# SHI-Labs/Prompt-Free-Diffusion

Hardware: AMD Instinct MI355X
Metric: images/sec @512x512 50-step DDIM, SD-v1.5+SeeCoder (higher is better)
Workload: dtype f16; 1 GPU; [c2] SD-v1.5 UNet + seecoder-v1-0, 512x512, 50-step DDIM (50 real steps), CFG 2.0, fp16, batch=4/GPU, 1 SeeCoder encode(s) + VAE decode per batch; global_batch=4, parallelism=dp1, world_size_reported_by_backend=1, collectives_forced_at_world_1=False

## Files before the change

### include/pfd_hip.h

```cpp
#ifndef PFD_HIP_H
#define PFD_HIP_H

#include <stddef.h>
#include <stdint.h>

#ifdef __cplusplus
extern "C" {
#endif

#define PFD_OK 0
#define PFD_EINVAL (-1)
#define PFD_ESHAPE (-2)
#define PFD_ELAUNCH (-3)

#define PFD_ABI_VERSION 10

typedef void* pfd_stream_t;

#define PFD_ACT_NONE 0
#define PFD_ACT_GELU 1
#define PFD_ACT_RELU 2
#define PFD_ACT_SILU 3
#define PFD_ACT_GEGLU 4

int pfd_abi_version(void);
const char* pfd_last_error(void);

typedef struct PfdGemmDesc {
  const void* A;
  const void* W;
  const void* bias;
  const void* rowvec;
  const void* R;
  void* C;
  int64_t lda, ldw, ldr, ldc, ldrv;
  int32_t M, N, K;
  int32_t rows_per_rv;
  int32_t act;
  int32_t bias_per_row;
  int32_t ksize, stride, pad, ups;
  int32_t B, H, Wd, Cin;
  int32_t Ho, Wo;
  void* ws;
  size_t ws_bytes;
  void* Ct;
  int64_t ldct;
  int32_t n_split;
  int32_t w_tiled;
  const void* gn_table;
  const void* A2;
  int64_t lda2;
  int32_t gn_c1;
  int32_t gn_act;
  const void* ln_stats;
  const void* ln_colsum;
  int32_t ln_parts;
  float ln_eps;
  void* ln_out;
  int32_t k_split;
  int32_t zero_rows;
  void* gn_out;
  const void* gnf_gamma;
  const void* gnf_beta;
  void* gnf_y;
  int64_t gnf_ldy;
  float gnf_eps;
  int32_t gnf_act;
  int32_t gnf_rows;
  int32_t gnf_skip_raw;
  int32_t res_rows;
} PfdGemmDesc;
int pfd_gemm_f16(const PfdGemmDesc* d, pfd_stream_t stream);
int pfd_gemm_f16_ex(const PfdGemmDesc* d, int32_t tile, pfd_stream_t stream);

int32_t pfd_gemm_geglu_group(int32_t N);

typedef struct PfdAttnDesc {
  const void* Q;
  const void* K;
  const void* Vt;
  void* O;
  int64_t ldq, ldk, ldvt, ldo;
  int64_t q_bs, k_bs, vt_bs, o_bs;
  int32_t B, H, Nq, Nk, D;
  float scale;
} PfdAttnDesc;
int pfd_attention_f16(const PfdAttnDesc* d, pfd_stream_t stream);

typedef struct PfdSwinAttnDesc {
  const void* qkv;
  const void* qkv_bias;
  const void* rpb;
  void* out;
  int32_t B, H, W, C, nH, ws, shift;
  float scale;
} PfdSwinAttnDesc;
int pfd_swin_window_attention_f16(const PfdSwinAttnDesc* d, pfd_stream_t stream);

size_t pfd_groupnorm_ws_bytes(int32_t B, int32_t C, int32_t HW);
int32_t pfd_groupnorm_takes_pstats(int32_t B, int32_t C1, int32_t C2, int32_t HW, int32_t G);
int pfd_groupnorm_pstats_f16(const void* x1, int32_t C1, int64_t ldx1, const void* st1, const void* x2, int32_t C2,
                             int64_t ldx2, const void* st2, const void* gamma, const void* beta, void* y, int64_t ldy,
                             int32_t B, int32_t HW, int32_t G, float eps, int32_t act, pfd_stream_t stream);

int pfd_groupnorm_table_f16(const void* x1, int32_t C1, int64_t ldx1, const void* x2, int32_t C2, int64_t ldx2,
                            const void* gamma, const void* beta, void* table, int32_t B, int32_t HW, int32_t G,
                            float eps, void* ws, size_t ws_bytes, pfd_stream_t stream);
int pfd_groupnorm_f16(const void* x1, int32_t C1, int64_t ldx1, const void* x2, int32_t C2,
                      int64_t ldx2, const void* gamma, const void* beta, void* y, int64_t ldy,
                      int32_t B, int32_t HW, int32_t G, float eps, int32_t act ,
                      void* ws, size_t ws_bytes, pfd_stream_t stream);

int pfd_layernorm_f16(const void* x, int64_t ldx, const void* gamma, const void* beta, void* y,
                      int64_t ldy, int32_t M, int32_t C, float eps, int32_t gather4, int32_t B,
                      int32_t H, int32_t W, pfd_stream_t stream);

int pfd_ln_rowstats_f16(const void* x, int64_t ldx, int32_t M, int32_t C, void* out, pfd_stream_t stream);

int pfd_softmax_rows_f16(const void* x, int64_t ldx, void* y, int64_t ldy, int32_t R, int32_t N,
                         float scale, pfd_stream_t stream);

int pfd_nchw_to_nhwc_f16(const void* x, int32_t src_f32, void* y, int32_t B, int32_t C, int32_t H,
                         int32_t W, float mul, float add, int32_t rep, pfd_stream_t stream);
int pfd_nhwc_to_nchw(const void* x, void* y, int32_t dst_f32, int32_t B, int32_t C, int32_t H,
                     int32_t W, float mul, float add, float lo, float hi, pfd_stream_t stream);
int pfd_im2col_f16(const void* x, int64_t ldx, void* col, int32_t B, int32_t H, int32_t W,
                   int32_t Cin, int32_t ksize, int32_t stride, int32_t pad, int32_t Ho, int32_t Wo,
                   int32_t Kpad, pfd_stream_t stream);
int pfd_timestep_embedding_f16(const int64_t* t, void* out, int32_t B, int32_t dim,
                               float max_period, pfd_stream_t stream);
int pfd_cfg_ddim_step(const void* eps, int32_t nb, const float* x, const float* noise,
                      const float* coef, float* x_prev, float* pred_x0, void* xin_next, int32_t rep,
                      int32_t B, int32_t C, int32_t h, int32_t w, pfd_stream_t stream);
int pfd_philox_normal_f32(const int64_t* key, int32_t step, float* out, int32_t B, int64_t n_per_sample,
                          pfd_stream_t stream);
int pfd_cfg_ddim_step_rng(const void* eps, int32_t nb, const float* x, const int64_t* key, int32_t step,
                          float noise_mul, const float* coef, float* x_prev, float* pred_x0, void* xin_next,
                          int32_t rep, int32_t B, int32_t C, int32_t h, int32_t w, pfd_stream_t stream);
int pfd_add_f16(const void* a, const void* b, void* y, int64_t n, pfd_stream_t stream);
int pfd_axpby_f16(const void* a, float alpha, const void* b, float beta, void* y, int64_t n,
                  pfd_stream_t stream);
int pfd_add_rowvec_f16(const void* x, int64_t ldx, const void* v, void* y, int64_t ldy, int32_t R,
                       int32_t C, pfd_stream_t stream);

int pfd_add_rowvec_lnstats_f16(const void* x, int64_t ldx, const void* v, void* y, int64_t ldy, int32_t R, int32_t C,
                               void* stats, pfd_stream_t stream);

int pfd_image_u8_f16(const void* x, void* y, int64_t n, float mul, float add, int32_t f16_image,
                     pfd_stream_t stream);

#define PFD_IMG_PRECISION_BITS 22
#define PFD_IMG_U8 0
#define PFD_IMG_NCHW_F16 1
#define PFD_IMG_NCHW_F32 2
#define PFD_IMG_NHWC_F16 3

int pfd_image_resample_check(int32_t B, int32_t Hin, int32_t Win, int32_t Hout, int32_t Wout, int32_t C);

int pfd_image_resample_h_u8(const void* src, void* dst, int32_t B, int32_t H, int32_t Win, int32_t Wout, int32_t C,
                            const int32_t* kk, const int32_t* xmin, const int32_t* klen, int32_t ktaps,
                            pfd_stream_t stream);

int pfd_image_resample_v_u8(const void* src, void* dst, int32_t out_kind, int32_t B, int32_t Hin, int32_t Hout,
                            int32_t W, int32_t C, const int32_t* kk, const int32_t* ymin, const int32_t* klen,
                            int32_t ktaps, pfd_stream_t stream);

int pfd_act_f16(const void* x, void* y, int64_t n, int32_t act, pfd_stream_t stream);

int pfd_prof_enable(int32_t on);
int pfd_prof_read(int32_t bucket, double* ms, int64_t* launches, double* flops, double* bytes);
const char* pfd_prof_bucket_name(int32_t bucket);
int pfd_prof_num_buckets(void);

#ifdef __cplusplus
}
#endif
#endif
```

### prompt-free-diffusion_amd/csrc/gemm_conv.hip

```cpp
#include "pfd_common.h"

namespace {

__device__ __attribute__((aligned(16))) half_t g_zero_halves[8];
__device__ __forceinline__ const half_t* pfd_zero_halves() { return g_zero_halves; }

constexpr int BK = 64;
constexpr int LDS_LD = BK + 8;

struct GemmParams {
  const half_t* A;
  const half_t* W;
  const half_t* bias;
  const half_t* rowvec;
  const half_t* R;
  half_t* C;
  long lda, ldw, ldr, ldc, ldrv;
  int M, N, K;
  int rows_per_rv, act, bias_per_row;
  int ksize, stride, pad, ups;
  int B, H, Wd, Cin, Ho, Wo;
  int tiles_m, tiles_n;
};

// ... 327 lines not shown
    if (cb + 1 < ncb) store_patch((cb + 1) & 1);
  }
  const int x = x0 + wave * 16 + l15, n0 = 4 * kg;
  if (x < p.Wd && n0 < p.N) {
    const long m = ((long)b * p.H + y) * p.Wd + x;
    const half_t* bsrc = p.bias ? p.bias : pfd_zero_halves();
    half_t bv[4], o[4];
#pragma unroll
    for (int r = 0; r < 4; ++r) bv[r] = bsrc[p.bias ? min(n0 + r, p.N - 1) : r];
#pragma unroll
    for (int r = 0; r < 4; ++r) o[r] = (half_t)(acc[r] + (float)bv[r]);
    half_t* cp = p.C + m * p.ldc + n0;
    if (n0 + 4 <= p.N && (p.ldc & 3) == 0 && (reinterpret_cast<uintptr_t>(p.C) & 7) == 0) {
      Pack8 q;
#pragma unroll
      for (int r = 0; r < 4; ++r) q.e[r] = o[r];
      *reinterpret_cast<uint2*>(cp) = q.u;
    } else {
#pragma unroll
      for (int r = 0; r < 4; ++r)
        if (n0 + r < p.N) cp[r] = o[r];
    }
  }
}

static bool narrow_conv_takes(const GemmParams& p) {
  return p.ksize == 3 && p.stride == 1 && p.pad == 1 && !p.ups && p.Ho == p.H && p.Wo == p.Wd && p.N <= 16 && p.Cin % BK == 0 &&
         !p.rowvec && !p.R && p.act == PFD_ACT_NONE && !p.bias_per_row;
}

static int launch_narrow_conv(const GemmParams& p, hipStream_t s) {
  const bool prof = pfd_prof_on();
  if (prof)
    pfd_prof_begin(20, 2.0 * p.M * p.N * p.K, 2.0 * p.B * p.H * p.Wd * p.Cin + 2.0 * p.N * p.K + 2.0 * p.M * p.N, s);
  const int segs = (p.Wd + NRW_PX - 1) / NRW_PX;
  hipLaunchKernelGGL(conv3x3_narrow_kernel, dim3(segs * p.H * p.B), dim3(256), 0, s, p);
  if (prof) pfd_prof_end(s);
  return pfd_check_launch("pfd_gemm_f16(conv3x3 narrow)");
}

}

int pfd_gemm160_try(const PfdGemmDesc* d, int variant, int splits, hipStream_t s);

extern "C" int32_t pfd_gemm_geglu_group(int32_t N) { return N % 160 == 0 ? 2 : 32; }

extern "C" int pfd_gemm_f16_ex(const PfdGemmDesc* d, int32_t tile, pfd_stream_t stream) {
  if (!d || !d->A || !d->W || !d->C) return PFD_EINVAL;
  if (d->M <= 0 || d->N <= 0 || d->K <= 0) return PFD_EINVAL;
  if ((d->lda & 7) || (d->ldw & 7)) return PFD_EINVAL;
  if ((reinterpret_cast<uintptr_t>(d->A) & 15) || (reinterpret_cast<uintptr_t>(d->W) & 15)) return PFD_EINVAL;
  if (d->K % BK) return PFD_ESHAPE;
  if (d->rowvec && d->rows_per_rv < 1) return PFD_EINVAL;
  if (d->act < PFD_ACT_NONE || d->act > PFD_ACT_GEGLU) return PFD_EINVAL;
  if (d->ksize > 0) {
    if (d->Cin <= 0 || d->K != (d->ups == 2 ? 4 : d->ksize * d->ksize) * d->Cin) return PFD_EINVAL;
    if ((long)d->B * d->Ho * d->Wo != d->M) return PFD_EINVAL;
    if (d->stride < 1) return PFD_EINVAL;
  }
  if (d->Ct && (d->act != PFD_ACT_NONE || d->rowvec || d->R || d->bias_per_row || (tile != 0 && tile < 1000)))
    return PFD_EINVAL;
  if (tile == 0 || tile >= 1000) {
    const int enc = tile >= 1000 ? tile - 1000 : 0;
    const int rc = pfd_gemm160_try(d, enc / 100, enc % 100, (hipStream_t)stream);
    if (rc <= 0) return rc;
    if (tile >= 1000 || d->Ct) return PFD_ESHAPE;
  }
  if (d->ksize > 0 && d->ups == 2) {
    pfd_set_error("pfd_gemm_f16: the phase-folded upsample convolution is served by the 256-row loader-wave kernel only (see PfdGemmDesc.ups)");
    return PFD_ESHAPE;
  }
  if (d->gn_table) {
    pfd_set_error("pfd_gemm_f16: the GroupNorm prologue is served by the 3x3 patch kernel only (see PfdGemmDesc.gn_table)");
    return PFD_ESHAPE;
  }
  if (d->gn_out) {
    pfd_set_error("pfd_gemm_f16: GroupNorm statistics of the output are emitted by the wide-tile kernels only (see PfdGemmDesc.gn_out)");
    return PFD_ESHAPE;
  }
  if (d->res_rows > 0 && d->res_rows != d->M) {
    pfd_set_error("pfd_gemm_f16: a residual stored once for a doubled batch is read by the wide-tile kernels only (see PfdGemmDesc.res_rows)");
    return PFD_ESHAPE;
  }
  if (d->gnf_y) {
    pfd_set_error("pfd_gemm_f16: the fused GroupNorm lives in the split-K reduction of the wide-tile kernels only (see PfdGemmDesc.gnf_y)");
    return PFD_ESHAPE;
  }
  if (d->k_split > 0 || d->zero_rows > 0) {
    pfd_set_error("pfd_gemm_f16: k_split / zero_rows are served by the wide-tile linear kernels only (see PfdGemmDesc.k_split)");
    return PFD_ESHAPE;
  }
  if (d->w_tiled) {
    pfd_set_error("pfd_gemm_f16: K-tile-contiguous weights are read by the wide-tile kernels only (see PfdGemmDesc.w_tiled)");
    return PFD_ESHAPE;
  }
  if (d->ln_stats || d->ln_out) {
    pfd_set_error("pfd_gemm_f16: the LayerNorm fold is served by the wide-tile linear kernels only (see PfdGemmDesc.ln_stats)");
    return PFD_ESHAPE;
  }
  GemmParams p;
  p.A = (const half_t*)d->A;
  p.W = (const half_t*)d->W;
  p.bias = (const half_t*)d->bias;
  p.rowvec = (const half_t*)d->rowvec;
  p.R = (const half_t*)d->R;
  p.C = (half_t*)d->C;
  p.lda = d->lda; p.ldw = d->ldw; p.ldr = d->ldr; p.ldc = d->ldc; p.ldrv = d->ldrv;
  p.M = d->M; p.N = d->N; p.K = d->K;
  p.rows_per_rv = d->rows_per_rv > 0 ? d->rows_per_rv : 1;
  p.act = d->act; p.bias_per_row = d->bias_per_row;
  p.ksize = d->ksize; p.stride = d->stride; p.pad = d->pad; p.ups = d->ups;
  p.B = d->B; p.H = d->H; p.Wd = d->Wd; p.Cin = d->Cin; p.Ho = d->Ho; p.Wo = d->Wo;
  p.tiles_m = p.tiles_n = 0;
  if (p.ksize > 0) {
    if (p.Cin % BK) return PFD_ESHAPE;
    if (p.K != p.ksize * p.ksize * p.Cin) return PFD_EINVAL;
    if ((long)p.B * p.Ho * p.Wo != p.M) return PFD_EINVAL;
    if (p.stride < 1) return PFD_EINVAL;
  }
  if (p.act < PFD_ACT_NONE || p.act > PFD_ACT_GEGLU) return PFD_EINVAL;
  hipStream_t s = (hipStream_t)stream;
  if (tile == 0 && narrow_conv_takes(p)) return launch_narrow_conv(p, s);
  if (p.act == PFD_ACT_GEGLU) {
    if (p.N % 128 || pfd_gemm_geglu_group(p.N) != 32) return PFD_ESHAPE;
    return launch<2, 2>(p, s);
  }
  switch (tile) {
    case 0: break;
    case 22: return launch<2, 2>(p, s);
    case 21: return launch<2, 1>(p, s);
    case 12: return launch<1, 2>(p, s);
    case 11: return launch<1, 1>(p, s);
    default: return PFD_EINVAL;
  }
  auto blocks = [&](int bm, int bn) { return (long)((p.M + bm - 1) / bm) * ((p.N + bn - 1) / bn); };
  auto waste = [&](int bn) { return (double)(((p.N + bn - 1) / bn) * bn) / p.N; };
  if (blocks(128, 128) >= 512 && waste(128) <= 1.13) return launch<2, 2>(p, s);
  if (blocks(128, 64) >= 384 && p.M >= 128) return launch<2, 1>(p, s);
  if (p.N > 64 && blocks(64, 128) >= 384 && waste(128) <= 1.13) return launch<1, 2>(p, s);
  return launch<1, 1>(p, s);
}

extern "C" int pfd_gemm_f16(const PfdGemmDesc* d, pfd_stream_t stream) { return pfd_gemm_f16_ex(d, 0, stream); }
```

### prompt-free-diffusion_amd/csrc/gemm_glds.hip

```cpp
#include <type_traits>

#include <stdlib.h>

#include "pfd_common.h"

int pfd_ln_rowstats_launch(const half_t* x, long ldx, int M, int C, float* out, hipStream_t s, bool prof);

namespace {

constexpr int BK = 64;
constexpr int BN = 160;
constexpr int ROWB = BK * 2;

__device__ __attribute__((aligned(256))) half_t g_zero_page[128];

struct G160Params {
  const half_t* A;
  const half_t* W;
  const half_t* bias;
  const half_t* rowvec;
  const half_t* R;
  half_t* C;
  float* ws;
  half_t* Ct;
  long ldct;
  int n_split;
  long lda, ldw, ldr, ldc, ldrv;
  int M, N, K;
  int rows_per_rv, act;
  int ksize, stride, pad, ups;
  int B, H, Wd, Cin, Ho, Wo;
  int tiles_m, tiles_n, splits, kt_per_split;
  int nmajor;
  int krot;
  int pt_w, pt_sh;
  int w_tu;
  long w_kstep;
  const float2* ln_in;
  const float* ln_cs;
  float2* ln_out;
  int ln_P;
  float ln_eps;
  const float* gn_table;
  const half_t* A2;
  long lda2;
  int gn_c1, gn_act;
  float2* gn_out;
  int k_split;
  int zero_rows;
  int r_wrap;
};

__device__ __forceinline__ long res_row(const G160Params& p, int m) {
  const int mc = min(m, p.M - 1);
  return mc >= p.r_wrap ? mc - p.r_wrap : mc;
}

__device__ __forceinline__ void glds16(const void* src, void* lds_dst) {
  __builtin_amdgcn_global_load_lds((const __attribute__((address_space(1))) void*)src,
                                   (__attribute__((address_space(3))) void*)lds_dst, 16, 0, 0);
}

__device__ __forceinline__ const half_t* w_row_ptr(const G160Params& p, int n, int c8) {
  if (p.w_tu == 0) return p.W + (long)n * p.ldw + c8;
  const int tn = n / p.w_tu;
  return p.W + ((long)tn * (p.K / BK) * p.w_tu + (n - tn * p.w_tu)) * BK + c8;
}

#if !defined(PFD_CPU_EMU)
#define PFD_ARG_BATCH_LIN(p)                                                                                              \
  asm volatile("" ::"s"((p).tiles_m), "s"((p).tiles_n), "s"((p).nmajor), "s"((p).kt_per_split), "s"((p).K), "s"((p).M),      \
               "s"((p).zero_rows), "s"((p).k_split), "s"((p).krot), "s"((p).w_tu), "s"((p).A), "s"((p).A2), "s"((p).W),      \
               "s"((p).lda), "s"((p).lda2), "s"((p).ldw), "s"((p).w_kstep))
#define PFD_ARG_BATCH_CONV(p)                                                                                             \
  asm volatile("" ::"s"((p).tiles_m), "s"((p).tiles_n), "s"((p).nmajor), "s"((p).kt_per_split), "s"((p).K), "s"((p).M),      \
               "s"((p).krot), "s"((p).w_tu), "s"((p).A), "s"((p).W), "s"((p).lda), "s"((p).ldw), "s"((p).w_kstep),           \
               "s"((p).Cin), "s"((p).H), "s"((p).Wd), "s"((p).Ho), "s"((p).Wo), "s"((p).stride), "s"((p).pad), "s"((p).ups), \
               "s"((p).ksize))
#else
#define PFD_ARG_BATCH_LIN(p) ((void)0)
#define PFD_ARG_BATCH_CONV(p) ((void)0)
#endif
template <int BN_>
__device__ __forceinline__ const half_t* w_row_ptr_tile(const G160Params& p, int tile_n, int r, int c8) {
  if (p.w_tu == 0) return p.W + (long)(tile_n * BN_ + r) * p.ldw + c8;
  const int sub = (BN_ > 160 && r >= p.w_tu) ? 1 : 0;
  const int tn = tile_n * (BN_ > 160 ? 2 : 1) + sub;
  return p.W + ((long)tn * (p.K / BK) * p.w_tu + (r - sub * p.w_tu)) * BK + c8;
}
#define PFD_W_ROW_PTR(BN_, p, tile_n, n0, r, c8) w_row_ptr_tile<BN_>(p, tile_n, r, c8)

__device__ __forceinline__ G160Params reload_params() {
  typedef __attribute__((address_space(4))) const unsigned* KArgPtr;
  KArgPtr k = (KArgPtr)__builtin_amdgcn_kernarg_segment_ptr();
  asm volatile("" : "+s"(k)::"memory");
  static_assert(sizeof(G160Params) % 4 == 0, "argument block read as dwords");
  unsigned w[sizeof(G160Params) / 4];
#pragma unroll
  for (unsigned i = 0; i < sizeof(G160Params) / 4; ++i) w[i] = k[i];
  G160Params q;
  __builtin_memcpy(&q, w, sizeof(q));
  return q;
}

template <int BYTES> struct GRaw;
template <> struct GRaw<2>  { typedef unsigned short type; };
template <> struct GRaw<8>  { typedef unsigned int type __attribute__((ext_vector_type(2))); };
template <> struct GRaw<16> { typedef unsigned int type __attribute__((ext_vector_type(4))); };
template <class T>
__device__ __forceinline__ T gld(const void* ptr) {
  typedef typename GRaw<sizeof(T)>::type V;
  const V v = *reinterpret_cast<const __attribute__((address_space(1))) V*>((unsigned long)ptr);
  T out;
  __builtin_memcpy(&out, &v, sizeof(T));
  return out;
}
template <class T>
__device__ __forceinline__ void gst(void* ptr, T val) {
  typedef typename GRaw<sizeof(T)>::type V;
  V v;
  __builtin_memcpy(&v, &val, sizeof(T));
  *reinterpret_cast<__attribute__((address_space(1))) V*>((unsigned long)ptr) = v;
}

template <int PT>
__device__ __forceinline__ int tile_row_m(const G160Params& p, int m0, int row) {
  if constexpr (PT == 2) {
    const int hw = p.H * p.Wd;
    const int bp = m0 / hw;
    const int q = m0 - bp * hw + row;
    const int y = q / p.Wd, x = q - y * p.Wd;
    return ((bp >> 2) * 2 * p.H + 2 * y + ((bp >> 1) & 1)) * (2 * p.Wd) + 2 * x + (bp & 1);
  } else if constexpr (PT == 1) return p.pt_w ? m0 + (row >> p.pt_sh) * p.Wd + (row & (p.pt_w - 1)) : m0 + row;
  else return m0 + row;
}

__device__ __forceinline__ int k_rotation(int krot, int tile_m, int tiles_m, int nsteps) {
  if (!krot || nsteps < 2) return 0;
  const int stride = max(1, nsteps / max(1, tiles_m));
  return (tile_m * stride) % nsteps;
}

__device__ __forceinline__ void lds_store16_opaque(void* lds_dst, uint4 v) {
  typedef unsigned u32x4 __attribute__((ext_vector_type(4)));
  const unsigned addr = (unsigned)(uintptr_t)(__attribute__((address_space(3))) char*)lds_dst;
  const u32x4 d = {v.x, v.y, v.z, v.w};
  asm volatile("ds_write_b128 %0, %1" ::"v"(addr), "v"(d) : "memory");
}

constexpr int stage_row_bytes(int cols) { return cols * 2 + 16; }

template <int WMB, int NT, bool PT = false>
__device__ __forceinline__ bool epilogue_stage(float4_t (&acc)[WMB][NT], const G160Params& p, int lane, int m0,
                                               int n0, int wm, int wn, int split, char* smem,
                                               const float2* lnstat = nullptr) {
  constexpr int BN = 32 * NT;
  const int l15 = lane & 15, g = lane >> 4;
  const int lr0 = wm * WMB * 16 + l15;
  auto mrow = [&](int lr) __attribute__((always_inline)) { return tile_row_m<PT>(p, m0, lr); };
  const int nw = n0 + wn * (16 * NT) + 4 * g;
  constexpr bool GEGLU_ONLY = NT == 10;
  if (lnstat && p.splits == 1) {
    float2 abv[WMB];
#pragma unroll
    for (int i = 0; i < WMB; ++i) abv[i] = lnstat[wm * WMB * 16 + i * 16 + l15];
    asm volatile("s_waitcnt lgkmcnt(0)" ::: "memory");
    __builtin_amdgcn_sched_barrier(0);
    float4_t cs[NT];
#pragma unroll
    for (int j = 0; j < NT; ++j) cs[j] = *reinterpret_cast<const float4_t*>(p.ln_cs + nw + j * 16);
#pragma unroll
    for (int i = 0; i < WMB; ++i) {
      const float2 ab = abv[i];
#pragma unroll
      for (int j = 0; j < NT; ++j)
#pragma unroll
        for (int r = 0; r < 4; ++r) acc[i][j][r] = fmaf(acc[i][j][r], ab.x, ab.y * cs[j][r]);
    }
  }

  const bool slab = !GEGLU_ONLY && p.splits > 1;

  if (!GEGLU_ONLY && !slab && p.Ct && n0 >= p.n_split) {
    float bv[NT][4];
    const half_t* bp = p.bias ? p.bias + nw : g_zero_page;
    const int bstep = p.bias ? 16 : 0;
#pragma unroll
    for (int j = 0; j < NT; ++j) {
      Pack8 b;
      b.u = gld<uint2>(bp + j * bstep);
#pragma unroll
      for (int r = 0; r < 4; ++r) bv[j][r] = (float)b.e[r];
    }
#pragma unroll
    for (int i = 0; i < WMB; ++i) {
      const int m = mrow(lr0 + i * 16);
      if (m >= p.M) continue;
#pragma unroll
      for (int j = 0; j < NT; ++j)
#pragma unroll
        for (int r = 0; r < 4; ++r)
          gst<half_t>(p.Ct + (long)(nw + j * 16 + r - p.n_split) * p.ldct + m, (half_t)(acc[i][j][r] + bv[j][r]));
    }
    return false;
  }

  const bool geglu = GEGLU_ONLY || p.act == PFD_ACT_GEGLU;
  const int lrow = wm * WMB * 16 + l15;
  const bool has_bias = p.bias && !slab;
  const half_t* bp = has_bias ? p.bias + nw : g_zero_page;
  const int bstep = has_bias ? 16 : 0;
  Pack8 bq[NT];
#pragma unroll
  for (int j = 0; j < NT; ++j) bq[j].u = gld<uint2>(bp + j * bstep);
  if (geglu) {
    constexpr int RS = stage_row_bytes(BN / 2);
#pragma unroll
    for (int i = 0; i < WMB; ++i) {
      char* sp = smem + (lrow + i * 16) * RS + (wn * (8 * NT) + 2 * g) * 2;
#pragma unroll
      for (int j = 0; j < NT; ++j) {
        half2_t o;
        o[0] = (half_t)((acc[i][j][0] + (float)bq[j].e[0]) * pfd_gelu(acc[i][j][2] + (float)bq[j].e[2]));
        o[1] = (half_t)((acc[i][j][1] + (float)bq[j].e[1]) * pfd_gelu(acc[i][j][3] + (float)bq[j].e[3]));
        *reinterpret_cast<half2_t*>(sp + j * 16) = o;
      }
    }
  } else if constexpr (!GEGLU_ONLY) {
    constexpr int RS = stage_row_bytes(BN);
    char* sp0 = smem + lrow * RS + (wn * (16 * NT) + 4 * g) * 2;
    auto put_row = [&](auto act, auto itag, const Pack8(&rv)[NT]) __attribute__((always_inline)) {
      constexpr int ACT = decltype(act)::value;
      constexpr int i = decltype(itag)::value;
      char* sp = sp0 + i * 16 * RS;
#pragma unroll
      for (int j = 0; j < NT; ++j) {
        Pack8 o;
#pragma unroll
        for (int r = 0; r < 4; ++r) {
          float v = acc[i][j][r] + (float)bq[j].e[r] + (float)rv[j].e[r];
          if constexpr (ACT == PFD_ACT_GELU) v = pfd_gelu(v);
          else if constexpr (ACT == PFD_ACT_RELU) v = fmaxf(v, 0.f);
          else if constexpr (ACT == PFD_ACT_SILU) v = pfd_silu(v);
          o.e[r] = (half_t)v;
        }
        *reinterpret_cast<uint2*>(sp + j * 32) = o.u;
      }
    };
    auto load_rv = [&](Pack8(&rv)[NT], int m) __attribute__((always_inline)) {
      const half_t* rvp = p.rowvec + (long)(min(m, p.M - 1) / p.rows_per_rv) * p.ldrv + nw;
#pragma unroll
      for (int j = 0; j < NT; ++j) rv[j].u = gld<uint2>(rvp + j * 16);
    };
    auto for_rows = [&](auto&& f) __attribute__((always_inline)) {
      f(std::integral_constant<int, 0>{});
      if constexpr (WMB > 1) f(std::integral_constant<int, 1>{});
      if constexpr (WMB > 2) f(std::integral_constant<int, 2>{});
      if constexpr (WMB > 3) f(std::integral_constant<int, 3>{});
      static_assert(WMB <= 4, "row tiles per wave");
    };
    auto run = [&](auto act) __attribute__((always_inline)) {
      Pack8 cur[NT];
      const int first = mrow(wm * WMB * 16), last = mrow(wm * WMB * 16 + WMB * 16 - 1);
      if (!p.rowvec || slab) {
#pragma unroll
        for (int j = 0; j < NT; ++j) cur[j].u = make_uint2(0, 0);
        for_rows([&](auto it) __attribute__((always_inline)) { put_row(act, it, cur); });
      } else if (PT || min(first, p.M - 1) / p.rows_per_rv == min(last, p.M - 1) / p.rows_per_rv) {
        load_rv(cur, first);
        for_rows([&](auto it) __attribute__((always_inline)) { put_row(act, it, cur); });
      } else if constexpr (!PT) {
        Pack8 nxt[NT];
        load_rv(cur, mrow(lr0));
        for_rows([&](auto it) __attribute__((always_inline)) {
          constexpr int i = decltype(it)::value;
          if constexpr (i + 1 < WMB) load_rv(nxt, mrow(lr0 + (i + 1) * 16));
          put_row(act, it, cur);
          if constexpr (i + 1 < WMB) {
#pragma unroll
            for (int j = 0; j < NT; ++j) cur[j].u = nxt[j].u;
          }
        });
      }
    };
    switch (slab ? PFD_ACT_NONE : p.act) {
      case PFD_ACT_GELU: run(std::integral_constant<int, PFD_ACT_GELU>{}); break;
      case PFD_ACT_RELU: run(std::integral_constant<int, PFD_ACT_RELU>{}); break;
      case PFD_ACT_SILU: run(std::integral_constant<int, PFD_ACT_SILU>{}); break;
      default: run(std::integral_constant<int, PFD_ACT_NONE>{}); break;
    }
// ... 191 lines not shown
    }
  };
  if (geglu) store_pass(std::integral_constant<int, BN / 2>{});
  else if constexpr (!GEGLU_ONLY) store_pass(std::integral_constant<int, BN>{});
}

template <int WMB, int NT, int NTHREADS, bool LNOUT = false, bool PT = false>
__device__ __forceinline__ void epilogue160(float4_t (&acc)[WMB][NT], const G160Params& p, int lane, int m0,
                                            int n0, int wm, int wn, int split, char* smem, int tid,
                                            const float2* lnstat = nullptr, int slab0 = 0) {
  epilogue_stage<WMB, NT, PT>(acc, p, lane, m0, n0, wm, wn, split, smem, lnstat);
  __syncthreads();
  epilogue_store<(NTHREADS / 128) * WMB * 16, NT, NTHREADS, LNOUT, PT>(p, m0, n0, smem, tid, slab0);
}

template <int WAVES_M, int WMB, bool CONV, int NBUF, int NT>
__global__ __launch_bounds__(WAVES_M * 128) void gemm160_kernel(const G160Params p) {
  constexpr int BN = 32 * NT;
  constexpr int NW = WAVES_M * 2;
  constexpr int BM = WAVES_M * WMB * 16;
  constexpr int A_INSTR = BM / 8;
  constexpr int B_INSTR = BN / 8;
  constexpr int A_PER_WAVE = A_INSTR / NW;
  constexpr int B_PER_WAVE = (B_INSTR + NW - 1) / NW;
  constexpr int STAGE = (BM + BN) * ROWB;
  constexpr int MAIN_BYTES = NBUF * STAGE;
  constexpr int DEPTH = NBUF - 1;
  constexpr bool B_DUP = NBUF > 2 && B_INSTR % NW != 0;
  static_assert(MAIN_BYTES <= 160 * 1024, "operand ring exceeds the 160 KiB LDS");
  static_assert(BM * stage_row_bytes(NT == 10 ? BN / 2 : BN) <= MAIN_BYTES, "the epilogue's staging image reuses the operand ring");
  constexpr int SMEM = MAIN_BYTES;
  static_assert(A_INSTR % NW == 0, "A tile must split evenly over the waves");
  static_assert(WAVES_M * 128 >= BM, "one thread per row forms the LayerNorm statistics");
  __shared__ __attribute__((aligned(1024))) char smem[SMEM + (CONV ? 0 : BM * 8)];
  float2* const lnstat = reinterpret_cast<float2*>(smem + SMEM);
  if constexpr (CONV) PFD_ARG_BATCH_CONV(p);
  else PFD_ARG_BATCH_LIN(p);

  const int tid = threadIdx.x;
  const int lane = tid & 63;
  const int wave = __builtin_amdgcn_readfirstlane(tid >> 6);
  const int wm = wave >> 1, wn = wave & 1;
  const int l15 = lane & 15, g = lane >> 4;

  const int nblk = p.tiles_m * p.tiles_n;
  const int t = xcd_remap(blockIdx.x, nblk);
  const int tile_m = p.nmajor ? t % p.tiles_m : t / p.tiles_n;
  const int tile_n = p.nmajor ? t / p.tiles_m : t - tile_m * p.tiles_n;
  const int m0 = tile_m * BM;
  const int n0 = tile_n * BN;
  const int split = blockIdx.z;
  const int kt_begin = split * p.kt_per_split;
  const int nk_total = p.K / BK;
  const int kt_end = min(nk_total, kt_begin + p.kt_per_split);

  const int srow = lane >> 3;
  const int cpos = lane & 7;
  const half_t* a_ptr[A_PER_WAVE];
  const half_t* a2_ptr[A_PER_WAVE];
  int a_oy[A_PER_WAVE], a_ox[A_PER_WAVE];
  long a_img[A_PER_WAVE];
  bool a_ok[A_PER_WAVE];
  int a_chunk[A_PER_WAVE];
#pragma unroll
  for (int j = 0; j < A_PER_WAVE; ++j) {
    const int r = (wave + NW * j) * 8 + srow;
    const int c = cpos ^ ((r >> 1) & 7);
    a_chunk[j] = c * 8;
    const int m = m0 + r;
    a_ok[j] = m < p.M;
    if (CONV) {
      const int hw = p.Ho * p.Wo;
      const int b = m / hw;
      const int rem = m - b * hw;
      const int oy = rem / p.Wo;
      a_oy[j] = oy * p.stride - p.pad;
      a_ox[j] = (rem - oy * p.Wo) * p.stride - p.pad;
      a_img[j] = (long)b * p.H * p.Wd * p.lda;
      a_ptr[j] = a2_ptr[j] = p.A;
    } else {
      const int mz = m - p.zero_rows;
      a_ok[j] = a_ok[j] && mz >= 0;
      a_ptr[j] = a_ok[j] ? p.A + (long)mz * p.lda + c * 8 : g_zero_page;
      a2_ptr[j] = a_ok[j] ? p.A2 + (long)mz * p.lda2 + c * 8 : g_zero_page;
      a_oy[j] = a_ox[j] = 0;
      a_img[j] = 0;
    }
  }
  const half_t* b_ptr[B_PER_WAVE];
#pragma unroll
  for (int j = 0; j < B_PER_WAVE; ++j) {
    int q = wave + NW * j;
    if (q >= B_INSTR) q = B_DUP ? q - NW : 0;
    const int r = q * 8 + srow;
    const int c = cpos ^ ((r >> 1) & 7);
    b_ptr[j] = PFD_W_ROW_PTR(BN, p, tile_n, n0, r, c * 8);
  }
  const int Hin = p.ups ? 2 * p.H : p.H;
  const int Win = p.ups ? 2 * p.Wd : p.Wd;

  const int nsteps = (!CONV && m0 + BM <= p.zero_rows) ? 0 : kt_end - kt_begin;
  int kt_issue = kt_begin + k_rotation(p.krot, tile_m, p.tiles_m, nsteps);
  int tap_ky = 0, tap_kx = 0, ci0 = 0;
  const half_t* a_tap[A_PER_WAVE];
  auto set_tap = [&]() {
#pragma unroll
    for (int j = 0; j < A_PER_WAVE; ++j) {
      int iy = a_oy[j] + tap_ky, ix = a_ox[j] + tap_kx;
      const bool ok = a_ok[j] && iy >= 0 && iy < Hin && ix >= 0 && ix < Win;
      if (p.ups) {
        iy >>= 1;
        ix >>= 1;
      }
      a_tap[j] = ok ? p.A + a_img[j] + ((long)iy * p.Wd + ix) * p.lda + a_chunk[j] : nullptr;
    }
  };
  auto seek = [&](int kt) {
    const int k0 = kt * BK;
    const int tap = k0 / p.Cin;
    ci0 = k0 - tap * p.Cin;
    tap_ky = tap / p.ksize;
    tap_kx = tap - tap_ky * p.ksize;
    set_tap();
  };
  if (CONV) seek(kt_issue);

  auto issue = [&](int stage) {
    char* As = smem + stage * STAGE;
    char* Bs = As + BM * ROWB;
    const int k0 = kt_issue * BK;
    const long kw = kt_issue * p.w_kstep;
    if (CONV) {
#pragma unroll
      for (int j = 0; j < A_PER_WAVE; ++j) {
        const half_t* src = a_tap[j] ? a_tap[j] + ci0 : g_zero_page;
        glds16(src, As + (wave + NW * j) * 1024);
      }
    } else {
      const bool first = k0 < p.k_split;
#pragma unroll
      for (int j = 0; j < A_PER_WAVE; ++j) {
        const half_t* src = first ? a_ptr[j] + k0 : a2_ptr[j] + (k0 - p.k_split);
        glds16(a_ok[j] ? src : a_ptr[j], As + (wave + NW * j) * 1024);
      }
    }
#pragma unroll
    for (int j = 0; j < B_PER_WAVE; ++j) {
      const int q = wave + NW * j;
      if (q < B_INSTR) glds16(b_ptr[j] + kw, Bs + q * 1024);
      else if (B_DUP) glds16(b_ptr[j] + kw, Bs + (q - NW) * 1024);
    }
    if (++kt_issue == kt_end) {
      kt_issue = kt_begin;
      if (CONV) seek(kt_begin);
    } else if (CONV) {
      ci0 += BK;
      if (ci0 >= p.Cin) {
        ci0 = 0;
        if (++tap_kx == p.ksize) {
          tap_kx = 0;
          ++tap_ky;
        }
        set_tap();
      }
    }
  };

// ... 732 lines not shown
                for (int j = 0; j < 5; ++j)
                  acc[i][j] = __builtin_amdgcn_mfma_f32_16x16x32_f16(bf[j], af[i], acc[i][j], 0, 0, 0);
            }
            if constexpr (NWS == 2) stage ^= 1;
            else if (++stage == NWS) stage = 0;
            toff += 1;
          }
          toff += PW - 3;
        }
      }
      block_barrier();
    }
    {
      const G160Params pe = reload_params();
      epilogue_stage<WMB, 5, true>(acc, pe, lane, m0, n0, wm, wn, split, smem);
    }
    asm volatile("s_waitcnt lgkmcnt(0)" ::: "memory");
    block_barrier();
  }
  const G160Params pe = reload_params();
  epilogue_store<256, 5, 768, false, true>(pe, m0, n0, smem, tid, tile_m * (256 / GN_SLAB));
}


__global__ __launch_bounds__(256) void splitk_reduce_kernel(const G160Params p) {
  const int nv = p.N / 8;
  const long nvec = (long)p.M * nv;
  for (long i = (long)blockIdx.x * 256 + threadIdx.x; i < nvec; i += (long)gridDim.x * 256) {
    const int m = (int)(i / nv);
    const int n = (int)(i - (long)m * nv) * 8;
    Pack16 bb, rv, rr;
    bb.u = *reinterpret_cast<const uint4*>(p.bias ? p.bias + n : g_zero_page);
    rv.u = *reinterpret_cast<const uint4*>(p.rowvec ? p.rowvec + (long)(m / p.rows_per_rv) * p.ldrv + n : g_zero_page);
    rr.u = *reinterpret_cast<const uint4*>(p.R ? p.R + res_row(p, m) * p.ldr + n : g_zero_page);
    float v[8] = {0, 0, 0, 0, 0, 0, 0, 0};
    for (int s0 = 0; s0 < p.splits; s0 += 4) {
      Pack16 a[4];
#pragma unroll
      for (int u = 0; u < 4; ++u)
        a[u].u = *reinterpret_cast<const uint4*>(reinterpret_cast<const half_t*>(p.ws) +
                                                 ((long)min(s0 + u, p.splits - 1) * p.M + m) * p.N + n);
#pragma unroll
      for (int u = 0; u < 4; ++u) {
        const float w = s0 + u < p.splits ? 1.f : 0.f;
#pragma unroll
        for (int e = 0; e < 8; ++e) v[e] += (float)a[u].e[e] * w;
      }
    }
    if (p.ln_in) {
      const float2* src = p.ln_in + (long)m * p.ln_P;
      float sum = 0.f, sq = 0.f;
#pragma unroll
      for (int j = 0; j < 8; ++j) {
        const float2 t = src[min(j, p.ln_P - 1)];
        const float w = j < p.ln_P ? 1.f : 0.f;
        sum = fmaf(t.x, w, sum);
        sq = fmaf(t.y, w, sq);
      }
      const float inv_k = 1.0f / (float)p.K;
      const float mean = sum * inv_k;
      const float rstd = rsqrtf(fmaxf(fmaf(-mean, mean, sq * inv_k), 0.f) + p.ln_eps);
      const float4_t c0 = *reinterpret_cast<const float4_t*>(p.ln_cs + n);
      const float4_t c1 = *reinterpret_cast<const float4_t*>(p.ln_cs + n + 4);
#pragma unroll
      for (int e = 0; e < 4; ++e) {
        v[e] = fmaf(v[e], rstd, -rstd * mean * c0[e]);
        v[4 + e] = fmaf(v[4 + e], rstd, -rstd * mean * c1[e]);
      }
    }
    Pack16 o;
#pragma unroll
    for (int e = 0; e < 8; ++e) {
      float x = v[e] + (float)bb.e[e];
      x += (float)rv.e[e];
      if (p.act == PFD_ACT_GELU) x = pfd_gelu(x);
      else if (p.act == PFD_ACT_RELU) x = fmaxf(x, 0.f);
      else if (p.act == PFD_ACT_SILU) x = pfd_silu(x);
      o.e[e] = (half_t)(x + (float)rr.e[e]);
    }
    *reinterpret_cast<uint4*>(p.C + (long)m * p.ldc + n) = o.u;
  }
}

constexpr int RGN_T = 256;
__global__ __launch_bounds__(RGN_T) void splitk_reduce_gn_kernel(const G160Params p) {
  constexpr int RW = RGN_T / 64, ROWS_SW = 3 * RW;
  __shared__ __attribute__((aligned(16))) float red[(RW + 1) * 320];
  const int tid = threadIdx.x, lane = tid & 63, w = tid >> 6;
  const int tiles_n = p.N / 160;
  const int slab = blockIdx.x / tiles_n, tile_n = blockIdx.x - slab * tiles_n;
  const int n = tile_n * 160 + (lane % 20) * 8;
  const bool active = lane < 60;
  const int rsub = lane / 20;
  float cs[8], cq[8];
#pragma unroll
  for (int e = 0; e < 8; ++e) cs[e] = cq[e] = 0.f;
  Pack16 bb;
  bb.u = *reinterpret_cast<const uint4*>(p.bias ? p.bias + n : g_zero_page);
  constexpr int SWEEPS = (GN_SLAB + ROWS_SW - 1) / ROWS_SW, U = SWEEPS < 3 ? SWEEPS : 3;
  static_assert(SWEEPS % U == 0, "sweeps in groups of U");
  for (int it0 = 0; it0 < SWEEPS; it0 += U) {
    int m[U];
    bool ok[U];
    Pack16 rv[U], rr[U];
    float v[U][8];
#pragma unroll
    for (int u = 0; u < U; ++u) {
      const int row_u = w * 3 + rsub + (it0 + u) * ROWS_SW;
      m[u] = min(slab * GN_SLAB + min(row_u, GN_SLAB - 1), p.M - 1);
      ok[u] = active && row_u < GN_SLAB && slab * GN_SLAB + row_u < p.M;
      rv[u].u = *reinterpret_cast<const uint4*>(p.rowvec ? p.rowvec + (long)(m[u] / p.rows_per_rv) * p.ldrv + n : g_zero_page);
      rr[u].u = *reinterpret_cast<const uint4*>(p.R ? p.R + res_row(p, m[u]) * p.ldr + n : g_zero_page);
#pragma unroll
      for (int e = 0; e < 8; ++e) v[u][e] = 0.f;
    }
    for (int s0 = 0; s0 < p.splits; s0 += 4) {
      Pack16 a[U][4];
#pragma unroll
      for (int u = 0; u < U; ++u)
#pragma unroll
        for (int k = 0; k < 4; ++k)
          a[u][k].u = *reinterpret_cast<const uint4*>(reinterpret_cast<const half_t*>(p.ws) +
                                                      ((long)min(s0 + k, p.splits - 1) * p.M + m[u]) * p.N + n);
#pragma unroll
      for (int u = 0; u < U; ++u)
#pragma unroll
        for (int k = 0; k < 4; ++k) {
          const float wgt = s0 + k < p.splits ? 1.f : 0.f;
#pragma unroll
          for (int e = 0; e < 8; ++e) v[u][e] += (float)a[u][k].e[e] * wgt;
        }
    }
#pragma unroll
    for (int u = 0; u < U; ++u) {
      Pack16 o;
      const float mk = ok[u] ? 1.f : 0.f;
#pragma unroll
      for (int e = 0; e < 8; ++e) {
        float x = v[u][e] + (float)bb.e[e];
        x += (float)rv[u].e[e];
        if (p.act == PFD_ACT_GELU) x = pfd_gelu(x);
        else if (p.act == PFD_ACT_RELU) x = fmaxf(x, 0.f);
        else if (p.act == PFD_ACT_SILU) x = pfd_silu(x);
        o.e[e] = (half_t)(x + (float)rr[u].e[e]);
        const float f = (float)o.e[e] * mk;
        cs[e] += f;
        cq[e] = fmaf(f, f, cq[e]);
      }
      if (ok[u]) *reinterpret_cast<uint4*>(p.C + (long)m[u] * p.ldc + n) = o.u;
    }
  }
  gn_slab_reduce<1, RGN_T>(cs, cq, tid, p.N / 32, slab, p.M / GN_SLAB, tiles_n, tile_n, p.gn_out, [&](int) { return red; });
}


struct GnFuse {
  const half_t* gamma;
  const half_t* beta;
  half_t* y;
  long ldy;
  float eps;
  int act, rows, skip_raw;
};
#ifndef PFD_GN_THREADS
#define PFD_GN_THREADS 1024
#endif
// ... 67 lines not shown
        for (int u = 0; u < GNF_U; ++u)
#pragma unroll
          for (int e = 0; e < 4; ++e) acc[u][e] += (float)a[u][q].e[e] * w;
      }
    }
#pragma unroll
    for (int u = 0; u < GNF_U; ++u) {
      Pack8 o;
#pragma unroll
      for (int e = 0; e < 4; ++e) {
        float x = acc[u][e] + (float)bq[u].e[e];
        x += (float)rq[u].e[e];
        if (p.act == PFD_ACT_GELU) x = pfd_gelu(x);
        else if (p.act == PFD_ACT_RELU) x = fmaxf(x, 0.f);
        else if (p.act == PFD_ACT_SILU) x = pfd_silu(x);
        o.e[e] = (half_t)(x + (float)xq[u].e[e]);
      }
      if (on[u] && !f.skip_raw) *reinterpret_cast<uint2*>(p.C + (m_b + ru[u]) * p.ldc + n_g + cu[u] * 4) = o.u;
      v[k0 + u] = on[u] ? o.u : make_uint2(0, 0);
    }
  }
  if (tid < cpg) {
    gam_s[tid] = (float)f.gamma[n_g + tid];
    bet_s[tid] = (float)f.beta[n_g + tid];
  }
  float sm = 0.f, sq = 0.f;
#pragma unroll
  for (int k = 0; k < GNF_MAX; ++k) {
    Pack8 q;
    q.u = v[k];
#pragma unroll
    for (int e = 0; e < 4; ++e) {
      const float x = (float)q.e[e];
      sm += x;
      sq += x * x;
    }
  }
  sm = wave_sum(sm);
  sq = wave_sum(sq);
  constexpr int NWV = GNF_T / 64;
  if (lane == 0) {
    red[wave] = sm;
    red[NWV + wave] = sq;
  }
  __syncthreads();
  const float count = (float)HW * (float)cpg;
  float ts = red[0], tq = red[NWV];
#pragma unroll
  for (int w = 1; w < NWV; ++w) {
    ts += red[w];
    tq += red[NWV + w];
  }
  const float mean = ts / count;
  const float rstd = rsqrtf(fmaxf(tq / count - mean * mean, 0.f) + f.eps);
  half_t* yb = f.y + m_b * f.ldy + n_g;
  r = tid / cpr;
  ch = tid - r * cpr;
  asm volatile("" : "+v"(r), "+v"(ch));
#pragma unroll
  for (int k = 0; k < GNF_MAX; ++k) {
    if (tid + GNF_T * k < total) {
      Pack8 q, o;
      q.u = v[k];
#pragma unroll
      for (int e = 0; e < 4; ++e) {
        const float w = rstd * gam_s[ch * 4 + e];
        float t = (float)q.e[e] * w + (bet_s[ch * 4 + e] - mean * w);
        if (f.act == PFD_ACT_SILU) t = pfd_silu(t);
        o.e[e] = (half_t)t;
      }
      *reinterpret_cast<uint2*>(yb + (long)r * f.ldy + ch * 4) = o.u;
    }
    r += dr;
    ch += dc;
    if (ch >= cpr) {
      ch -= cpr;
      ++r;
    }
  }
}

thread_local GnFuse t_gnf = {nullptr, nullptr, nullptr, 0, 0.f, 0, 0, 0};

inline void launch_splitk_reduce(const G160Params& p, hipStream_t s) {
  if (pfd_prof_on()) {
    pfd_prof_end(s);
    const double mn = (double)p.M * p.N;
    pfd_prof_begin(21, 0.0, 2.0 * p.splits * mn + 2.0 * mn * (1 + (p.R ? 1 : 0) + (t_gnf.y ? 1 : 0)), s);
  }
  if (t_gnf.y) {
    const GnFuse f = t_gnf;
    hipLaunchKernelGGL(splitk_reduce_gnorm_kernel, dim3(32 * (p.M / f.rows)), dim3(GNF_T), 0, s, p, f);
    return;
  }
  if (p.gn_out) {
    hipLaunchKernelGGL(splitk_reduce_gn_kernel, dim3((p.M / GN_SLAB) * (p.N / 160)), dim3(RGN_T), 0, s, p);
  } else {
    const long nvec = (long)p.M * (p.N / 8);
    int g = (int)((nvec + 255) / 256);
    if (g > 2048) g = 2048;
    hipLaunchKernelGGL(splitk_reduce_kernel, dim3(g), dim3(256), 0, s, p);
  }
  if (p.ln_out) pfd_ln_rowstats_launch(p.C, p.ldc, p.M, p.N, reinterpret_cast<float*>(p.ln_out), s, false);
}


inline int pick_nmajor(const G160Params& p) {
  const double a_bytes = p.ksize > 0 ? 2.0 * p.B * p.H * p.Wd * p.Cin : 2.0 * p.M * p.K;
  const double w_bytes = 2.0 * p.N * p.K;
  return (p.tiles_n >= 2 && p.tiles_m >= 2 && w_bytes > a_bytes) ? 1 : 0;
}

template <int WAVES_M, int WMB, int NBUF = 2, int NT = 5>
int launch160(G160Params& p, int bucket, hipStream_t s) {
  constexpr int BM = WAVES_M * WMB * 16;
  p.tiles_m = (p.M + BM - 1) / BM;
  p.tiles_n = p.N / (32 * NT);
  p.nmajor = pick_nmajor(p);
  p.krot = 0;
  const int nk = p.K / BK;
  p.kt_per_split = (nk + p.splits - 1) / p.splits;
  p.splits = (nk + p.kt_per_split - 1) / p.kt_per_split;
  dim3 grid(p.tiles_m * p.tiles_n, 1, p.splits);
  const bool prof = pfd_prof_on();
  if (prof) {
    const double a_bytes = p.ksize > 0 ? 2.0 * p.B * p.H * p.Wd * p.Cin : 2.0 * p.M * p.K;
    const double n_out = p.act == PFD_ACT_GEGLU ? p.N / 2 : p.N;
    pfd_prof_begin(bucket, 2.0 * p.M * p.N * p.K, a_bytes + 2.0 * p.N * p.K + 2.0 * p.M * n_out * (p.R ? 2 : 1), s);
  }
  if (p.ksize > 0)
    hipLaunchKernelGGL((gemm160_kernel<WAVES_M, WMB, true, NBUF, NT>), grid, dim3(WAVES_M * 128), 0, s, p);
  else
    hipLaunchKernelGGL((gemm160_kernel<WAVES_M, WMB, false, NBUF, NT>), grid, dim3(WAVES_M * 128), 0, s, p);
  if (p.splits > 1) launch_splitk_reduce(p, s);
  if (prof) pfd_prof_end(s);
  return pfd_check_launch("pfd_gemm_f16(wide)");
}

template <int NT>
int launch160ws(G160Params& p, int bucket, hipStream_t s, int pp) {
  p.tiles_m = (p.M + 255) / 256;
  p.tiles_n = p.N / (32 * NT);
  p.nmajor = pick_nmajor(p);
  p.krot = 0;
  const int nk = p.K / BK;
  p.kt_per_split = (nk + p.splits - 1) / p.splits;
  p.splits = (nk + p.kt_per_split - 1) / p.kt_per_split;
  dim3 grid(p.tiles_m * p.tiles_n, 1, p.splits);
  const bool prof = pfd_prof_on();
  if (prof) {
    const double a_bytes = p.ksize > 0 ? 2.0 * p.B * p.H * p.Wd * p.Cin : 2.0 * p.M * p.K;
    const double n_out = p.act == PFD_ACT_GEGLU ? p.N / 2 : p.N;
    pfd_prof_begin(bucket, 2.0 * p.M * p.N * p.K, a_bytes + 2.0 * p.N * p.K + 2.0 * p.M * n_out * (p.R ? 2 : 1), s);
  }
  if (p.ksize > 0 && p.ups == 2) {
    if (pp == 2) hipLaunchKernelGGL((gemm160ws_kernel<true, NT, 3, true>), grid, dim3(768), 0, s, p);
    else hipLaunchKernelGGL((gemm160ws_kernel<true, NT, 2, true>), grid, dim3(768), 0, s, p);
  } else if (p.ksize > 0) {
    if (pp == 2) hipLaunchKernelGGL((gemm160ws_kernel<true, NT, 3>), grid, dim3(768), 0, s, p);
    else hipLaunchKernelGGL((gemm160ws_kernel<true, NT>), grid, dim3(768), 0, s, p);
  } else {
    if (pp == 2) hipLaunchKernelGGL((gemm160ws_kernel<false, NT, 3>), grid, dim3(768), 0, s, p);
    else hipLaunchKernelGGL((gemm160ws_kernel<false, NT>), grid, dim3(768), 0, s, p);
  }
  if (p.splits > 1) launch_splitk_reduce(p, s);
  if (prof) pfd_prof_end(s);
  return pfd_check_launch("pfd_gemm_f16(wave-specialised)");
}

int launch_patch(G160Params& p, hipStream_t s, int ws) {
  p.tiles_m = p.M / 256;
  p.tiles_n = p.N / BN;
  p.nmajor = pick_nmajor(p);
  p.krot = 0;
  const int ncb = p.Cin / BK;
  p.kt_per_split = (ncb + p.splits - 1) / p.splits;
  p.splits = (ncb + p.kt_per_split - 1) / p.kt_per_split;
  dim3 grid(p.tiles_m * p.tiles_n, 1, p.splits);
  const bool prof = pfd_prof_on();
  if (prof)
    pfd_prof_begin(19, 2.0 * p.M * p.N * p.K,
                   2.0 * p.B * p.H * p.Wd * p.Cin + 2.0 * p.N * p.K + 2.0 * p.M * p.N * (p.R ? 2 : 1), s);
  if (p.gn_table && p.gn_act == PFD_ACT_SILU) hipLaunchKernelGGL((conv3x3_patch_ws_kernel<2>), grid, dim3(768), 0, s, p);
  else if (p.gn_table) hipLaunchKernelGGL((conv3x3_patch_ws_kernel<1>), grid, dim3(768), 0, s, p);
  else if (ws == 3) hipLaunchKernelGGL((conv3x3_patch_ws_kernel<0, 3>), grid, dim3(768), 0, s, p);
  else if (ws) hipLaunchKernelGGL((conv3x3_patch_ws_kernel<0>), grid, dim3(768), 0, s, p);
  else hipLaunchKernelGGL(conv3x3_patch_kernel, grid, dim3(512), 0, s, p);
  if (p.splits > 1) launch_splitk_reduce(p, s);
  if (prof) pfd_prof_end(s);
  return pfd_check_launch("pfd_gemm_f16(conv3x3 patch)");
}

}

int pfd_gemm160_try(const PfdGemmDesc* d, int variant, int splits, hipStream_t s) {
  const int bn = d->N % 160 == 0 ? 160 : 128;
  if (d->N % bn || d->bias_per_row || d->K % BK) return 1;
  if (bn == 128 && d->act == PFD_ACT_GEGLU) return 1;
  if (d->ksize > 0 && (d->Cin % BK)) return 1;
  if (d->act == PFD_ACT_GEGLU && (d->rowvec || d->R)) return 1;
  if ((d->ldc & 7) || (reinterpret_cast<uintptr_t>(d->C) & 15)) return 1;
  if (d->bias && (reinterpret_cast<uintptr_t>(d->bias) & 15)) return 1;
  if (d->R && ((d->ldr & 7) || (reinterpret_cast<uintptr_t>(d->R) & 15))) return 1;
  if (d->rowvec && ((d->ldrv & 7) || (reinterpret_cast<uintptr_t>(d->rowvec) & 15))) return 1;
  if (d->Ct) {
    if (d->ksize > 0 || d->n_split <= 0 || d->n_split >= d->N || d->n_split % bn || (d->ldct & 7) ||
        (reinterpret_cast<uintptr_t>(d->Ct) & 15))
      return 1;
    splits = 1;
  }
  G160Params p;
  p.Ct = (half_t*)d->Ct; p.ldct = d->ldct; p.n_split = d->n_split;
  p.A = (const half_t*)d->A; p.W = (const half_t*)d->W; p.bias = (const half_t*)d->bias;
  p.rowvec = (const half_t*)d->rowvec; p.R = (const half_t*)d->R; p.C = (half_t*)d->C;
  p.ws = (float*)d->ws;
  p.lda = d->lda; p.ldw = d->ldw; p.ldr = d->ldr; p.ldc = d->ldc; p.ldrv = d->ldrv;
  p.w_tu = d->w_tiled ? bn : 0;
  p.w_kstep = d->w_tiled ? (long)bn * BK : BK;
  p.M = d->M; p.N = d->N; p.K = d->K;
  p.rows_per_rv = d->rows_per_rv > 0 ? d->rows_per_rv : 1;
  p.act = d->act;
  p.ksize = d->ksize; p.stride = d->stride; p.pad = d->pad; p.ups = d->ups;
  p.B = d->B; p.H = d->H; p.Wd = d->Wd; p.Cin = d->Cin; p.Ho = d->Ho; p.Wo = d->Wo;
  p.tiles_m = p.tiles_n = 0;
  p.kt_per_split = 0;
  p.pt_w = p.pt_sh = 0;
  p.gn_table = (const float*)d->gn_table; p.A2 = (const half_t*)d->A2; p.lda2 = d->lda2;
  p.gn_c1 = d->gn_c1; p.gn_act = d->gn_act;
  p.ln_in = (const float2*)d->ln_stats; p.ln_cs = (const float*)d->ln_colsum; p.ln_P = d->ln_parts; p.ln_eps = d->ln_eps;
  p.ln_out = (float2*)d->ln_out;
  p.gn_out = (float2*)d->gn_out;
  if (p.gn_out) {
    if (bn != 160 || (d->N % 32) || d->N / 32 < 8 || (160 % (d->N / 32)) || (d->M % GN_SLAB) || d->act == PFD_ACT_GEGLU || d->Ct ||
        d->ln_out || d->bias_per_row || (reinterpret_cast<uintptr_t>(p.gn_out) & 7))
      return 1;
    if (d->ksize > 0 && ((long)d->Ho * d->Wo) % GN_SLAB) return 1;
  }
  t_gnf.y = nullptr;
  const bool gnf = d->gnf_y != nullptr;
  if (gnf) {
    const int cpg = d->N / 32;
    if (bn != 160 || (d->N % 32) || (cpg % 4) || cpg < 20 || cpg > 256 || d->gnf_rows <= 0 || (d->M % d->gnf_rows) ||
        (long)d->gnf_rows * (cpg / 4) > (long)GNF_T * GNF_MAX || (long)(d->M / d->gnf_rows) * 32 < 128 || !d->gnf_gamma || !d->gnf_beta ||
        (d->gnf_ldy & 3) || (reinterpret_cast<uintptr_t>(d->gnf_y) & 7) || d->act == PFD_ACT_GEGLU || d->Ct || d->ln_stats ||
        d->ln_out || d->gn_out || d->bias_per_row || !d->ws ||
        (d->gnf_act != PFD_ACT_NONE && d->gnf_act != PFD_ACT_SILU))
      return 1;
    const int rpr = d->rows_per_rv > 0 ? d->rows_per_rv : 1;
    if (d->rowvec && (rpr % d->gnf_rows) && rpr < d->M) return 1;
  }
  auto gnf_arm = [&](int nsplits) -> bool {
    if (!gnf) return true;
    if (nsplits <= 1) return false;
    t_gnf = GnFuse{(const half_t*)d->gnf_gamma, (const half_t*)d->gnf_beta, (half_t*)d->gnf_y, (long)d->gnf_ldy, d->gnf_eps,
                   d->gnf_act, d->gnf_rows, d->gnf_skip_raw};
    return true;
  };
  struct GnfDisarm { ~GnfDisarm() { t_gnf.y = nullptr; } } gnf_disarm;
  p.r_wrap = 0x7fffffff;
  if (d->res_rows > 0 && d->res_rows != d->M) {
    if (!d->R || d->res_rows >= d->M || 2L * d->res_rows < d->M || d->gnf_y) return 1;
    p.r_wrap = d->res_rows;
  }
  p.k_split = d->K; p.zero_rows = 0;
  if (d->k_split > 0 || d->zero_rows > 0) {
    if (d->ksize > 0 || d->gn_table || d->bias_per_row || d->Ct) return 1;
    if (d->zero_rows < 0 || d->zero_rows >= d->M || (d->zero_rows > 0 && d->ln_stats)) return 1;
    if (variant == 47 || variant == 48 || variant == 84) return 1;
    if (d->k_split > 0) {
      if (d->k_split >= d->K || (d->k_split % BK) || !d->A2 || (d->lda2 & 7) || (reinterpret_cast<uintptr_t>(d->A2) & 15)) return 1;
      p.k_split = d->k_split;
    }
    p.zero_rows = d->zero_rows;
  }
  if (p.ksize == 0 && p.k_split == d->K) { p.A2 = p.A; p.lda2 = p.lda; }
  if (d->ksize > 0 && d->ups == 2) {
    if (d->ksize != 3 || d->stride != 1 || d->pad != 1 || d->K != 4 * d->Cin || d->Ho != 2 * d->H || d->Wo != 2 * d->Wd ||
        ((long)d->H * d->Wd) % 256 || d->R || d->rowvec || d->Ct || d->gn_table || d->gnf_y || d->ln_stats || d->ln_out ||
        d->k_split > 0 || d->zero_rows > 0 || d->act == PFD_ACT_GEGLU || (variant != 0 && variant != 47 && variant != 48) || splits > 1)
      return 1;
    p.splits = 1;
    const int mode = variant == 48 ? 0 : 2;
    if (bn == 128) return launch160ws<4>(p, 16, s, mode) < 0 ? PFD_ELAUNCH : 0;
    return launch160ws<5>(p, 16, s, mode) < 0 ? PFD_ELAUNCH : 0;
  }
  if (p.ln_in) {
    if (d->ksize > 0 || !p.ln_cs || p.ln_P < 1 || p.ln_P > 8 || p.ln_P * 160 != d->K) return 1;
    if ((reinterpret_cast<uintptr_t>(p.ln_in) & 7) || (reinterpret_cast<uintptr_t>(p.ln_cs) & 15)) return 1;
    if (variant == 47 || variant == 48) return 1;
  }
  if (p.ln_out) {
    if (bn != 160 || d->ksize > 0 || d->act == PFD_ACT_GEGLU || d->Ct || (reinterpret_cast<uintptr_t>(p.ln_out) & 7)) return 1;
    if (variant == 47 || variant == 48) return 1;
  }
  if (p.gn_table) {
    if (bn != 160 || (variant != 0 && variant != 98)) return 1;
    variant = 98;
    if (p.gn_c1 <= 0 || p.gn_c1 > p.Cin || (p.gn_c1 % BK) || (p.gn_c1 < p.Cin && !p.A2)) return 1;
    if ((p.lda2 & 7) || (reinterpret_cast<uintptr_t>(p.A2) & 15) || (reinterpret_cast<uintptr_t>(p.gn_table) & 15))
      return 1;
    if (p.gn_act != PFD_ACT_NONE && p.gn_act != PFD_ACT_SILU) return 1;
    if (p.gn_c1 == p.Cin) { p.A2 = p.A; p.lda2 = p.lda; }
  }
  const int tn = p.N / bn;
  auto tiles = [&](int bm) { return (long)((p.M + bm - 1) / bm) * tn; };
  int pt_w = 0;
  if (p.ksize == 3 && p.Wd != 16 && p.Wd != 32 && p.Wd != 64) {
    if (p.Wd % 32 == 0 && p.H % 8 == 0) pt_w = 32;
    else if (p.Wd % 16 == 0 && p.H % 16 == 0) pt_w = 16;
  }
  const bool patch_w = p.Wd == 16 || p.Wd == 32 || p.Wd == 64 || pt_w != 0;
  if (bn == 160 && (variant == 0 || variant == 99 || variant == 98 || variant == 96) && p.ksize == 3 && p.stride == 1 && p.pad == 1 && !p.ups &&
      patch_w && p.Ho == p.H && p.Wo == p.Wd && (pt_w != 0 || p.H % (256 / p.Wd) == 0) &&
      p.M % 256 == 0 && ((long)p.H * p.Wd) % 256 == 0 && p.act != PFD_ACT_GEGLU) {
    p.pt_w = pt_w;
    p.pt_sh = pt_w == 32 ? 5 : 4;
    const int ncb = p.Cin / BK;
    if (splits == 0) {
      splits = 1;
      const long tl = tiles(256);
      if (d->ws && tl < 200) {
        splits = (int)((256 + tl - 1) / tl);
        if (splits > 8) splits = 8;
        while (splits > 1 && ncb / splits < 2) --splits;
        while (splits > 1 && (size_t)splits * p.M * p.N * 4 > d->ws_bytes) --splits;
      }
    }
    if (splits > 1 && (!d->ws || (size_t)splits * p.M * p.N * 4 > d->ws_bytes)) splits = 1;
    p.splits = splits;
    {
      const int kps = (ncb + splits - 1) / splits;
      if (!gnf_arm((ncb + kps - 1) / kps)) return 1;
    }
    const int ws = variant == 99 ? 0 : variant == 98 ? 1 : 3;
    return launch_patch(p, s, ws) < 0 ? PFD_ELAUNCH : 0;
  }
  if (variant == 99 || variant == 98 || variant == 96 || p.gn_table) return 1;
  const bool auto_variant = variant == 0;
  const int nk_all = p.K / BK;
  if (auto_variant) {
    const long t128 = tiles(128);
    const bool few = nk_all >= 16 ? t128 < 256 : t128 < 384;
    variant = tiles(256) >= 200 ? 44 : (nk_all <= 24 && few) ? 22 : 24;
    if (p.ksize == 0 && variant == 44 && p.M >= 8192 && nk_all <= 40) variant = 24;
    if (bn == 160 && p.ksize == 0 && variant == 24 && t128 <= 256 && nk_all >= 16) variant = 25;
    if (p.ksize == 0 && variant == 24 && nk_all <= 40 && t128 <= 256 && tiles(64) >= 384) variant = 22;
    if (variant == 44 && p.ksize > 0) variant = 47;
// ... 73 lines not shown
```

### prompt-free-diffusion_amd/csrc/norm.hip

```cpp
#include <stdlib.h>

#include "pfd_common.h"

namespace {

constexpr int GN_MAX_CHUNKS = 256;
constexpr int GN_MAX_G = 64;
#ifndef GN_ROWS
#define GN_ROWS 8
#endif

struct GnSrc {
  const half_t* x1;
  const half_t* x2;
  long ld1, ld2;
  int C1, C2;
};

__device__ __forceinline__ uint4 gn_load(const GnSrc& s, long row, int v) {
  const int c = v * 8;
  if (c < s.C1) return *reinterpret_cast<const uint4*>(s.x1 + row * s.ld1 + c);
  return *reinterpret_cast<const uint4*>(s.x2 + row * s.ld2 + (c - s.C1));
}

__global__ __launch_bounds__(256) void gn_stats_kernel(GnSrc s, int HW, int G, int rows_per_chunk,
                                                       float* __restrict__ partial) {
  __shared__ float red[256 * 16];
  __shared__ float chan[4096 * 2];
  const int C = s.C1 + s.C2;
  const int nvec = C / 8;
  const int b = blockIdx.y, chunk = blockIdx.x;
  const int tid = threadIdx.x;
  const int VT = nvec < 256 ? nvec : 256;
  const int RT = 256 / VT;
  const int v0 = tid % VT, rt = tid / VT;
  const int r_beg = chunk * rows_per_chunk;
  const int r_end = min(HW, r_beg + rows_per_chunk);
  const int nslot = (nvec + 255) / 256;
  for (int slot = 0; slot < nslot; ++slot) {
    const int v = v0 + slot * 256;
    float sm[8], sq[8];
#pragma unroll
    for (int e = 0; e < 8; ++e) sm[e] = sq[e] = 0.f;
    if (rt < RT && v < nvec) {
      const int c = v * 8;
      const half_t* src = c < s.C1 ? s.x1 + c : s.x2 + (c - s.C1);
      const long ld = c < s.C1 ? s.ld1 : s.ld2;
      src += (long)b * HW * ld;
      for (int r = r_beg + rt; r < r_end; r += GN_ROWS * RT) {
        Pack16 p[GN_ROWS];
#pragma unroll
        for (int u = 0; u < GN_ROWS; ++u)
          p[u].u = *reinterpret_cast<const uint4*>(src + (long)min(r + u * RT, r_end - 1) * ld);
#pragma unroll
        for (int u = 0; u < GN_ROWS; ++u) {
          const float m = r + u * RT < r_end ? 1.f : 0.f;
#pragma unroll
          for (int e = 0; e < 8; ++e) {
            const float x = (float)p[u].e[e] * m;
            sm[e] += x;
            sq[e] += x * x;
          }
        }
      }
    }
#pragma unroll
    for (int e = 0; e < 8; ++e) {
      red[tid * 16 + e] = sm[e];
      red[tid * 16 + 8 + e] = sq[e];
    }
    __syncthreads();
    if (rt == 0 && v < nvec) {
      for (int e = 0; e < 8; ++e) {
        float a = 0.f, q = 0.f;
        for (int k = 0; k < RT; ++k) {
          a += red[(k * VT + v0) * 16 + e];
          q += red[(k * VT + v0) * 16 + 8 + e];
        }
        chan[(v * 8 + e) * 2] = a;
        chan[(v * 8 + e) * 2 + 1] = q;
      }
    }
    __syncthreads();
  }
  const int cpg = C / G;
  if (tid < G) {
    float a = 0.f, q = 0.f;
    for (int c = tid * cpg; c < (tid + 1) * cpg; ++c) {
      a += chan[c * 2];
      q += chan[c * 2 + 1];
    }
    float* out = partial + (((long)b * gridDim.x + chunk) * G + tid) * 2;
    out[0] = a;
    out[1] = q;
  }
}

__global__ __launch_bounds__(256) void gn_apply_kernel(GnSrc s, const half_t* __restrict__ gamma,
                                                       const half_t* __restrict__ beta,
                                                       const float* __restrict__ partial, half_t* __restrict__ y,
                                                       long ldy, int HW, int G, int rows_per_chunk, int act,
                                                       int nchunks, float count, float eps) {
  __shared__ float sc[4096], sh[4096];
  __shared__ float ra[256], rq[256], gmean[GN_MAX_G], grstd[GN_MAX_G];
  const int C = s.C1 + s.C2;
// ... 19 lines not shown
        a += ra[k * G + tid];
        q += rq[k * G + tid];
      }
      const float mean = a / count;
      gmean[tid] = mean;
      grstd[tid] = rsqrtf(fmaxf(q / count - mean * mean, 0.f) + eps);
    }
    __syncthreads();
  }
  for (int c = tid; c < C; c += 256) {
    const int g = c / cpg;
    const float mean = gmean[g];
    const float rstd = grstd[g];
    const float w = rstd * (float)gamma[c];
    sc[c] = w;
    sh[c] = (float)beta[c] - mean * w;
  }
  __syncthreads();
  const int VT = nvec < 256 ? nvec : 256;
  const int RT = 256 / VT;
  const int v0 = tid % VT, rt = tid / VT;
  if (rt >= RT) return;
  const int r_beg = chunk * rows_per_chunk;
  const int r_end = min(HW, r_beg + rows_per_chunk);
  for (int v = v0; v < nvec; v += 256) {
    float w[8], o[8];
#pragma unroll
    for (int e = 0; e < 8; ++e) {
      w[e] = sc[v * 8 + e];
      o[e] = sh[v * 8 + e];
    }
    for (int r = r_beg + rt; r < r_end; r += 4 * RT) {
      Pack16 p[4];
#pragma unroll
      for (int u = 0; u < 4; ++u)
        if (r + u * RT < r_end) p[u].u = gn_load(s, (long)b * HW + r + u * RT, v);
#pragma unroll
      for (int u = 0; u < 4; ++u) {
        if (r + u * RT >= r_end) break;
        const long row = (long)b * HW + r + u * RT;
        Pack16 q;
#pragma unroll
        for (int e = 0; e < 8; ++e) {
          float t = (float)p[u].e[e] * w[e] + o[e];
          if (act == PFD_ACT_SILU) t = pfd_silu(t);
          q.e[e] = (half_t)t;
        }
        *reinterpret_cast<uint4*>(y + row * ldy + v * 8) = q.u;
      }
    }
  }
}

struct GnPStats {
  const float2* st1;
  const float2* st2;
  int tn1, tn2;
  int cpp1, cpp2;
};

template <bool PAR>
__global__ __launch_bounds__(256) void gn_apply_pstats_kernel(GnSrc s, GnPStats ps, const half_t* __restrict__ gamma,
                                                              const half_t* __restrict__ beta, half_t* __restrict__ y,
                                                              long ldy, int HW, int G, int rows_per_chunk, int act,
                                                              float count, float eps) {
  __shared__ float sc[4096], sh[4096];
  __shared__ float ra[256], rq[256], gmean[GN_MAX_G], grstd[GN_MAX_G];
  const int C = s.C1 + s.C2;
  const int nvec = C / 8;
  const int cpg = C / G;
  const int b = blockIdx.y, chunk = blockIdx.x, tid = threadIdx.x;
  {
    const int nslab = HW / 64;
    const int P = 256 / G;
    const int g = tid % G, part = tid / G;
    float a = 0.f, q = 0.f;
    if (part < P) {
      const int c0 = g * cpg;
      const bool first = c0 < s.C1;
      const float2* st = first ? ps.st1 : ps.st2;
      const int tn = first ? ps.tn1 : ps.tn2, cpp = first ? ps.cpp1 : ps.cpp2;
      const int cl = first ? c0 : c0 - s.C1;
      const int npg = cpg / cpp;
      if constexpr (PAR) {
        const int c1 = cl + (npg > 1 ? cpp : 0);
        const int col0 = (cl / 160) * 16 + (cl % 160) / cpp, col1 = (c1 / 160) * 16 + (c1 % 160) / cpp;
        const float w1 = npg > 1 ? 1.f : 0.f;
        for (int k0 = part; k0 < nslab; k0 += 8 * P) {
          float2 v0[8], v1[8];
#pragma unroll
          for (int u = 0; u < 8; ++u) {
            const int k = min(k0 + u * P, nslab - 1);
            const float2* row = st + ((long)(b * nslab + k) * tn) * 16;
            v0[u] = row[col0];
            v1[u] = row[col1];
          }
#pragma unroll
          for (int u = 0; u < 8; ++u) {
            const float w = k0 + u * P < nslab ? 1.f : 0.f;
            a += v0[u].x * w;
            q += v0[u].y * w;
            a += v1[u].x * (w * w1);
            q += v1[u].y * (w * w1);
          }
        }
      } else {
        for (int k = part; k < nslab; k += P) {
          const float2* row = st + ((long)(b * nslab + k) * tn) * 16;
          for (int j = 0; j < npg; ++j) {
            const int c = cl + j * cpp;
            const float2 v = row[(c / 160) * 16 + (c % 160) / cpp];
            a += v.x;
            q += v.y;
          }
        }
      }
    }
    ra[tid] = a;
    rq[tid] = q;
    __syncthreads();
    if (tid < G) {
      for (int k = 1; k < P; ++k) {
        a += ra[k * G + tid];
        q += rq[k * G + tid];
      }
      const float mean = a / count;
      gmean[tid] = mean;
      grstd[tid] = rsqrtf(fmaxf(q / count - mean * mean, 0.f) + eps);
    }
    __syncthreads();
  }
  for (int c = tid; c < C; c += 256) {
    const int g = c / cpg;
    const float w = grstd[g] * (float)gamma[c];
    sc[c] = w;
    sh[c] = (float)beta[c] - gmean[g] * w;
  }
  __syncthreads();
  const int VT = nvec < 256 ? nvec : 256;
  const int RT = 256 / VT;
  const int v0 = tid % VT, rt = tid / VT;
  if (rt >= RT) return;
  const int r_beg = chunk * rows_per_chunk;
  const int r_end = min(HW, r_beg + rows_per_chunk);
  for (int v = v0; v < nvec; v += 256) {
    float w[8], o[8];
#pragma unroll
    for (int e = 0; e < 8; ++e) {
      w[e] = sc[v * 8 + e];
      o[e] = sh[v * 8 + e];
    }
    constexpr int U = PAR ? 8 : 4;
    for (int r = r_beg + rt; r < r_end; r += U * RT) {
      Pack16 p[U];
#pragma unroll
      for (int u = 0; u < U; ++u)
        if (r + u * RT < r_end) p[u].u = gn_load(s, (long)b * HW + r + u * RT, v);
#pragma unroll
      for (int u = 0; u < U; ++u) {
        if (r + u * RT >= r_end) break;
        const long row = (long)b * HW + r + u * RT;
        Pack16 qv;
#pragma unroll
        for (int e = 0; e < 8; ++e) {
          float t = (float)p[u].e[e] * w[e] + o[e];
          if (act == PFD_ACT_SILU) t = pfd_silu(t);
          qv.e[e] = (half_t)t;
        }
        *reinterpret_cast<uint4*>(y + row * ldy + v * 8) = qv.u;
      }
    }
  }
}

__global__ __launch_bounds__(256) void gn_table_kernel(const half_t* __restrict__ gamma, const half_t* __restrict__ beta,
                                                       const float* __restrict__ partial, float* __restrict__ table,
                                                       int C, int G, int nchunks, float count, float eps) {
  __shared__ float ra[256], rq[256], gmean[GN_MAX_G], grstd[GN_MAX_G];
  const int b = blockIdx.x, tid = threadIdx.x;
  const int cpg = C / G;
  const int P = 256 / G;
  const int g = tid % G, part = tid / G;
  float a = 0.f, q = 0.f;
  if (part < P) {
    for (int k = part; k < nchunks; k += P) {
      const float2 v = *reinterpret_cast<const float2*>(partial + (((long)b * nchunks + k) * G + g) * 2);
      a += v.x;
      q += v.y;
    }
  }
  ra[tid] = a;
// ... 315 lines not shown
  __syncthreads();
  const float inv = 1.f / (red[4] + red[5] + red[6] + red[7]);
  for (int v = tid; v < nvec; v += 256) {
    Pack16 p, o;
    p.u = *reinterpret_cast<const uint4*>(xr + v * 8);
#pragma unroll
    for (int e = 0; e < 8; ++e) o.e[e] = (half_t)(__expf((float)p.e[e] * scale - mx) * inv);
    *reinterpret_cast<uint4*>(y + (long)row * ldy + v * 8) = o.u;
  }
}

}

static void gn_chunks(int B, int C, int HW, int* nchunks_out, int* rpc_out) {
  const int nvec = C / 8;
  const int RT = nvec < 256 ? 256 / nvec : 1;
  constexpr int target_blocks = 512;
  int nchunks = (target_blocks + B - 1) / B;
  const int max_by_rows = (HW + RT * 4 - 1) / (RT * 4);
  if (nchunks > max_by_rows) nchunks = max_by_rows;
  if (nchunks > GN_MAX_CHUNKS) nchunks = GN_MAX_CHUNKS;
  if (nchunks < 1) nchunks = 1;
  const int rpc = (HW + nchunks - 1) / nchunks;
  *nchunks_out = (HW + rpc - 1) / rpc;
  *rpc_out = rpc;
}

static bool gn_is_small(int B, int C, int HW, int G) {
  const int cpg = C / G;
  return cpg % 4 == 0 && cpg >= 32 && (long)HW * (cpg / 4) <= GNS_T * GNS_MAX && (long)B * G >= 128;
}

extern "C" size_t pfd_groupnorm_ws_bytes(int32_t B, int32_t C, int32_t HW) {
  (void)C;
  (void)HW;
  return (size_t)B * (GN_MAX_CHUNKS + 1) * GN_MAX_G * 2 * sizeof(float);
}

extern "C" int pfd_groupnorm_f16(const void* x1, int32_t C1, int64_t ldx1, const void* x2, int32_t C2,
                                 int64_t ldx2, const void* gamma, const void* beta, void* y, int64_t ldy,
                                 int32_t B, int32_t HW, int32_t G, float eps, int32_t act, void* ws,
                                 size_t ws_bytes, pfd_stream_t stream) {
  if (!x1 || !gamma || !beta || !y || !ws) return PFD_EINVAL;
  if (C2 > 0 && !x2) return PFD_EINVAL;
  if (C2 < 0 || C1 <= 0 || B <= 0 || HW <= 0 || G <= 0 || G > GN_MAX_G) return PFD_EINVAL;
  const int C = C1 + C2;
  if ((C1 & 7) || (C2 & 7) || (C % G) || C > 4096) return PFD_ESHAPE;
  if ((ldx1 & 7) || (ldx2 & 7) || (ldy & 7)) return PFD_EINVAL;
  if (act != PFD_ACT_NONE && act != PFD_ACT_SILU) return PFD_EINVAL;
  if (ws_bytes < pfd_groupnorm_ws_bytes(B, C, HW)) return PFD_EINVAL;
  hipStream_t s = (hipStream_t)stream;
  GnSrc src{(const half_t*)x1, (const half_t*)x2, ldx1, ldx2, C1, C2};
  const bool prof = pfd_prof_on();
  if (gn_is_small(B, C, HW, G)) {
    if (prof) pfd_prof_begin(10, 8.0 * B * HW * C, 4.0 * B * HW * C, s);
    hipLaunchKernelGGL(gn_small_kernel, dim3(G, B), dim3(GNS_T), 0, s, src, (const half_t*)gamma, (const half_t*)beta,
                       (half_t*)y, (long)ldy, HW, G, act, eps);
    if (prof) pfd_prof_end(s);
    return pfd_check_launch("pfd_groupnorm_f16(small)");
  }
  int nchunks, rpc;
  gn_chunks(B, C, HW, &nchunks, &rpc);
  float* partial = (float*)ws;
  if (prof) pfd_prof_begin(10, 8.0 * B * HW * C, 6.0 * B * HW * C, s);
  hipLaunchKernelGGL(gn_stats_kernel, dim3(nchunks, B), dim3(256), 0, s, src, HW, G, rpc, partial);
  hipLaunchKernelGGL(gn_apply_kernel, dim3(nchunks, B), dim3(256), 0, s, src, (const half_t*)gamma,
                     (const half_t*)beta, partial, (half_t*)y, (long)ldy, HW, G, rpc, act, nchunks,
                     (float)HW * (float)(C / G), eps);
  if (prof) pfd_prof_end(s);
  return pfd_check_launch("pfd_groupnorm_f16");
}

extern "C" int32_t pfd_groupnorm_takes_pstats(int32_t B, int32_t C1, int32_t C2, int32_t HW, int32_t G) {
  if (B <= 0 || C1 <= 0 || C2 < 0 || HW <= 0 || G <= 0 || G > GN_MAX_G) return 0;
  const int C = C1 + C2;
  if ((C % G) || C > 4096 || (HW % 64) || (C1 % 160) || (C2 % 160) || (C1 % 32) || (C2 % 32)) return 0;
  if (gn_is_small(B, C, HW, G)) return 0;
  const int cpg = C / G, cpp1 = C1 / 32, cpp2 = C2 ? C2 / 32 : cpp1;
  if (cpp1 < 8 || (160 % cpp1) || (cpg % cpp1) || (C1 % cpg)) return 0;
  if (C2 && (cpp2 < 8 || (160 % cpp2) || (cpg % cpp2))) return 0;
  return 1;
}

extern "C" int pfd_groupnorm_pstats_f16(const void* x1, int32_t C1, int64_t ldx1, const void* st1, const void* x2,
                                        int32_t C2, int64_t ldx2, const void* st2, const void* gamma, const void* beta,
                                        void* y, int64_t ldy, int32_t B, int32_t HW, int32_t G, float eps, int32_t act,
                                        pfd_stream_t stream) {
  if (!x1 || !st1 || !gamma || !beta || !y) return PFD_EINVAL;
  if (C2 > 0 && (!x2 || !st2)) return PFD_EINVAL;
  if (act != PFD_ACT_NONE && act != PFD_ACT_SILU) return PFD_EINVAL;
  if ((ldx1 & 7) || (ldx2 & 7) || (ldy & 7) || (reinterpret_cast<uintptr_t>(st1) & 7) || (reinterpret_cast<uintptr_t>(st2) & 7))
    return PFD_EINVAL;
  if (!pfd_groupnorm_takes_pstats(B, C1, C2, HW, G)) return PFD_ESHAPE;
  hipStream_t s = (hipStream_t)stream;
  const int C = C1 + C2;
  GnSrc src{(const half_t*)x1, (const half_t*)x2, ldx1, ldx2, C1, C2};
  GnPStats ps{(const float2*)st1, (const float2*)st2, C1 / 160, C2 ? C2 / 160 : 0, C1 / 32, C2 ? C2 / 32 : C1 / 32};
  int nchunks, rpc;
  gn_chunks(B, C, HW, &nchunks, &rpc);
  PfdProfScope prof_scope(10, 8.0 * B * HW * C, 4.0 * B * HW * C, s);
  const int cpg = C / G;
  const bool par = cpg / ps.cpp1 <= 2 && cpg / ps.cpp2 <= 2;
  if (par)
    hipLaunchKernelGGL(gn_apply_pstats_kernel<true>, dim3(nchunks, B), dim3(256), 0, s, src, ps, (const half_t*)gamma,
                       (const half_t*)beta, (half_t*)y, (long)ldy, HW, G, rpc, act, (float)HW * (float)(C / G), eps);
  else
    hipLaunchKernelGGL(gn_apply_pstats_kernel<false>, dim3(nchunks, B), dim3(256), 0, s, src, ps, (const half_t*)gamma,
                       (const half_t*)beta, (half_t*)y, (long)ldy, HW, G, rpc, act, (float)HW * (float)(C / G), eps);
  return pfd_check_launch("pfd_groupnorm_pstats_f16");
}

extern "C" int pfd_groupnorm_table_f16(const void* x1, int32_t C1, int64_t ldx1, const void* x2, int32_t C2,
                                       int64_t ldx2, const void* gamma, const void* beta, void* table, int32_t B,
                                       int32_t HW, int32_t G, float eps, void* ws, size_t ws_bytes,
                                       pfd_stream_t stream) {
  if (!x1 || !gamma || !beta || !table || !ws) return PFD_EINVAL;
  if (C2 > 0 && !x2) return PFD_EINVAL;
  if (C2 < 0 || C1 <= 0 || B <= 0 || HW <= 0 || G <= 0 || G > GN_MAX_G) return PFD_EINVAL;
  const int C = C1 + C2;
  if ((C1 & 7) || (C2 & 7) || (C % G) || C > 4096) return PFD_ESHAPE;
  if ((ldx1 & 7) || (ldx2 & 7) || (reinterpret_cast<uintptr_t>(table) & 15)) return PFD_EINVAL;
  if (ws_bytes < pfd_groupnorm_ws_bytes(B, C, HW)) return PFD_EINVAL;
  hipStream_t s = (hipStream_t)stream;
  GnSrc src{(const half_t*)x1, (const half_t*)x2, ldx1, ldx2, C1, C2};
  int nchunks, rpc;
  gn_chunks(B, C, HW, &nchunks, &rpc);
  const bool prof = pfd_prof_on();
  if (prof) pfd_prof_begin(10, 4.0 * B * HW * C, 2.0 * B * HW * C, s);
  hipLaunchKernelGGL(gn_stats_kernel, dim3(nchunks, B), dim3(256), 0, s, src, HW, G, rpc, (float*)ws);
  hipLaunchKernelGGL(gn_table_kernel, dim3(B), dim3(256), 0, s, (const half_t*)gamma, (const half_t*)beta,
                     (const float*)ws, (float*)table, C, G, nchunks, (float)HW * (float)(C / G), eps);
  if (prof) pfd_prof_end(s);
  return pfd_check_launch("pfd_groupnorm_table_f16");
}

extern "C" int pfd_layernorm_f16(const void* x, int64_t ldx, const void* gamma, const void* beta, void* y,
                                 int64_t ldy, int32_t M, int32_t C, float eps, int32_t gather4, int32_t B,
                                 int32_t H, int32_t W, pfd_stream_t stream) {
  if (!x || !gamma || !beta || !y || M <= 0 || C <= 0) return PFD_EINVAL;
  if ((C & 7) || C > 64 * 8 * LN_MAXV) return PFD_ESHAPE;
  if ((ldx & 7) || (ldy & 7)) return PFD_EINVAL;
  if (gather4) {
    if ((C % 32) || B <= 0 || H <= 0 || W <= 0) return PFD_EINVAL;
    if ((long)B * ((H + 1) / 2) * ((W + 1) / 2) != M) return PFD_EINVAL;
  }
  PfdProfScope prof_scope(11, 0.0, 4.0 * M * C, (hipStream_t)stream);
  if (!gather4 && C <= 1536 && M >= 8192) {
    constexpr int ROWS = 4;
    const dim3 grid((M + 4 * ROWS - 1) / (4 * ROWS));
    const int nv = (C / 8 + 63) / 64;
#define PFD_LN_ROWS(NV)                                                                                         \
  hipLaunchKernelGGL((layernorm_rows_kernel<NV, ROWS>), grid, dim3(256), 0, (hipStream_t)stream, (const half_t*)x, \
                     (long)ldx, (const half_t*)gamma, (const half_t*)beta, (half_t*)y, (long)ldy, M, C, eps)
    if (nv == 1) PFD_LN_ROWS(1);
    else if (nv == 2) PFD_LN_ROWS(2);
    else PFD_LN_ROWS(3);
#undef PFD_LN_ROWS
    return pfd_check_launch("pfd_layernorm_f16(rows)");
  }
  const int nv = (C / 8 + 63) / 64;
#define PFD_LN(G, NV)                                                                                              \
  hipLaunchKernelGGL((layernorm_kernel<G, NV>), dim3((M + 3) / 4), dim3(256), 0, (hipStream_t)stream,              \
                     (const half_t*)x, (long)ldx, (const half_t*)gamma, (const half_t*)beta, (half_t*)y, (long)ldy, \
                     M, C, eps, B, H, W)
#define PFD_LN_NV(G)                                                                                               \
  do {                                                                                                             \
    if (nv <= 1) PFD_LN(G, 1);                                                                                     \
    else if (nv <= 2) PFD_LN(G, 2);                                                                                \
    else if (nv <= 3) PFD_LN(G, 3);                                                                                \
    else if (nv <= 4) PFD_LN(G, 4);                                                                                \
    else if (nv <= 6) PFD_LN(G, 6);                                                                                \
    else PFD_LN(G, 8);                                                                                             \
  } while (0)
  if (gather4) PFD_LN_NV(true);
  else PFD_LN_NV(false);
#undef PFD_LN_NV
#undef PFD_LN
  return pfd_check_launch("pfd_layernorm_f16");
}

__global__ __launch_bounds__(256) void ln_rowstats_kernel(const half_t* __restrict__ x, long ldx, int M, int P,
                                                          float2* __restrict__ out) {
  const long grp = ((long)blockIdx.x * 256 + threadIdx.x) >> 2;
  const int k = threadIdx.x & 3;
  const long ngrp = (long)M * P;
  const long g = min(grp, ngrp - 1);
  const int m = (int)(g / P), p = (int)(g - (long)m * P);
  const half_t* src = x + (long)m * ldx + p * 160;
  Pack16 v[5];
#pragma unroll
  for (int j = 0; j < 5; ++j) v[j].u = *reinterpret_cast<const uint4*>(src + (k + 4 * j) * 8);
  float s = 0.f, q = 0.f;
// ... 48 lines not shown
```

### prompt-free-diffusion_amd/csrc/selftest.cpp

```cpp
#include <hip/hip_runtime.h>
#include <math.h>
#include <stdio.h>
#include <stdlib.h>
#include <string.h>

#include <algorithm>
#include <functional>
#include <random>
#include <string>
#include <array>
#include <atomic>
#include <thread>
#include <vector>

#include "pfd_hip.h"

typedef _Float16 h16;

#define HIP_OK(x)                                                                 \
  do {                                                                            \
    hipError_t e_ = (x);                                                          \
    if (e_ != hipSuccess) {                                                       \
      fprintf(stderr, "HIP error %s at %s:%d\n", hipGetErrorString(e_), __FILE__, __LINE__); \
      exit(99);                                                                   \
// ... 450 lines not shown
  ++g_total;
  d.C = dC1.p;
  int rc = pfd_gemm_f16_ex(&d, tile_a, nullptr);
  if (rc != 0) { ++g_fail; printf("FAIL %-58s rc=%d (%s)\n", name, rc, pfd_last_error()); return; }
  auto y1 = dC1.get();
  d.C = dC2.p;
  for (int r = 0; r < reps; ++r) {
    HIP_OK(hipMemset(dC2.p, 0xFF, (size_t)M * N * sizeof(h16)));
    rc = pfd_gemm_f16_ex(&d, tile_b, nullptr);
    if (rc != 0) { ++g_fail; printf("FAIL %-58s rc=%d (%s)\n", name, rc, pfd_last_error()); return; }
    auto y2 = dC2.get();
    if (memcmp(y1.data(), y2.data(), y1.size() * sizeof(h16))) {
      size_t nd = 0;
      for (size_t i = 0; i < y1.size(); ++i) nd += memcmp(&y1[i], &y2[i], sizeof(h16)) != 0;
      ++g_fail;
      printf("FAIL %-58s launch %d: %zu of %zu elements differ\n", name, r, nd, y1.size());
      return;
    }
  }
  printf("ok   %-58s\n", name);
}

static void run_lin_same_case(int M, int N, int K, int tile_a, int tile_b, bool res, int k_split = 0, int zero_rows = 0, int reps = 8) {
  auto A = rand_h((size_t)M * K), Wt = rand_h((size_t)N * K, 1.7f / sqrtf((float)K)), Bv = rand_h(N), R = rand_h((size_t)M * N);
  const int K1 = k_split > 0 ? k_split : K, K2 = K - K1, Mz = M - zero_rows;
  std::vector<h16> A1((size_t)Mz * K1), A2((size_t)Mz * (K2 > 0 ? K2 : 1));
  for (int m = 0; m < Mz; ++m) {
    for (int k = 0; k < K1; ++k) A1[(size_t)m * K1 + k] = A[(size_t)(m + zero_rows) * K + k];
    for (int k = 0; k < K2; ++k) A2[(size_t)m * K2 + k] = A[(size_t)(m + zero_rows) * K + K1 + k];
  }
  Dev<h16> dA(A1), dA2(A2), dW(Wt), dB(Bv), dR(R), dC1((size_t)M * N), dC2((size_t)M * N);
  Dev<float> dWS((size_t)8 * M * N);
  PfdGemmDesc d;
  memset(&d, 0, sizeof(d));
  d.M = M; d.N = N; d.K = K; d.A = dA.p; d.W = dW.p; d.bias = dB.p; d.R = res ? dR.p : nullptr;
  d.lda = K1; d.ldw = K; d.ldc = N; d.ldr = N; d.ldrv = N; d.rows_per_rv = 1;
  if (k_split > 0) { d.k_split = k_split; d.A2 = dA2.p; d.lda2 = K2; }
  d.zero_rows = zero_rows;
  d.ws = dWS.p; d.ws_bytes = (size_t)8 * M * N * sizeof(float);
  char name[200];
  snprintf(name, sizeof(name), "linear %dx%dx%d tile %d == tile %d (bitwise, %d launches)%s ks%d zr%d", M, N, K, tile_a, tile_b, reps,
           res ? " +res" : "", k_split, zero_rows);
  ++g_total;
  d.C = dC1.p;
  int rc = pfd_gemm_f16_ex(&d, tile_a, nullptr);
  if (rc != 0) { ++g_fail; printf("FAIL %-58s rc=%d (%s)\n", name, rc, pfd_last_error()); return; }
  auto y1 = dC1.get();
  d.C = dC2.p;
  for (int r = 0; r < reps; ++r) {
    HIP_OK(hipMemset(dC2.p, 0xFF, (size_t)M * N * sizeof(h16)));
    rc = pfd_gemm_f16_ex(&d, tile_b, nullptr);
    if (rc != 0) { ++g_fail; printf("FAIL %-58s rc=%d (%s)\n", name, rc, pfd_last_error()); return; }
    auto y2 = dC2.get();
    if (memcmp(y1.data(), y2.data(), y1.size() * sizeof(h16))) {
      size_t nd = 0;
      for (size_t i = 0; i < y1.size(); ++i) nd += memcmp(&y1[i], &y2[i], sizeof(h16)) != 0;
      ++g_fail;
      printf("FAIL %-58s launch %d: %zu of %zu elements differ\n", name, r, nd, y1.size());
      return;
    }
  }
  printf("ok   %-58s\n", name);
}

static void run_add_rowvec_lnstats_case(int R, int C) {
  auto X = rand_h((size_t)R * C, 3.0f), V = rand_h(C, 1.0f);
  Dev<h16> dX(X), dV(V), dY1((size_t)R * C), dY2((size_t)R * C);
  const int P = C / 160;
  Dev<float> s1((size_t)R * P * 2), s2((size_t)R * P * 2);
  int rc = pfd_add_rowvec_lnstats_f16(dX.p, C, dV.p, dY1.p, C, R, C, s1.p, nullptr);
  if (rc == 0) rc = pfd_add_rowvec_f16(dX.p, C, dV.p, dY2.p, C, R, C, nullptr);
  if (rc == 0) rc = pfd_ln_rowstats_f16(dY2.p, C, R, C, s2.p, nullptr);
  char name[128];
  snprintf(name, sizeof(name), "add_rowvec + row statistics R%d C%d (bitwise vs two launches)", R, C);
  ++g_total;
  if (rc != 0) { ++g_fail; printf("FAIL %-58s rc=%d (%s)\n", name, rc, pfd_last_error()); return; }
  auto y1 = dY1.get(), y2 = dY2.get();
  auto a = s1.get(), b = s2.get();
  const bool same = !memcmp(y1.data(), y2.data(), y1.size() * sizeof(h16)) && !memcmp(a.data(), b.data(), a.size() * sizeof(float));
  if (!same) { ++g_fail; printf("FAIL %-58s outputs differ\n", name); }
  else printf("ok   %-58s\n", name);
}

static void run_ln_fold_suite() {
  run_add_rowvec_lnstats_case(130, 320);
  run_add_rowvec_lnstats_case(77, 1280);
  run_ln_fold_case(300, 320, 960, 0, 0, 0, 640);
  run_ln_fold_case(700, 320, 320, 0, 3400, 3400, 0);
  run_ln_fold_case(520, 640, 640, 0, 9200, 9200, 0);
  run_ln_fold_case(300, 640, 1280, PFD_ACT_GEGLU, 5400, 5400, 0);
  run_ln_fold_case(600, 320, 640, PFD_ACT_GEGLU, 3200, 9400, 0);
  run_ln_fold_case(130, 1280, 320, 0, 3204, 3204, 0);
  run_ln_fold_case(200, 1280, 1280, PFD_ACT_GELU, 5300, 3300, 0);
  run_ln_fold_case(77, 960, 160, 0, 9300, 3500, 0);
}

static void run_attn_case(int B, int H, int Nq, int Nk, int D, bool fused_layout, int spike = 0) {
  const int C = H * D;
  const float scale = 1.0f / sqrtf((float)D);
  const long ldq = fused_layout ? 2 * C : C, ldk = ldq, ldo = C;
  const int Nkp = (Nk + 7) / 8 * 8;
  const long ldvt = (long)B * Nkp;
  auto Qh = rand_h((size_t)B * Nq * ldq, 1.5f), Kh = rand_h((size_t)B * Nk * ldk, 1.5f), Vt = rand_h((size_t)C * ldvt, 1.0f);
  if (spike > 0 && spike < Nk) {
    const int koff0 = fused_layout ? C : 0;
    for (int b = 0; b < B; ++b)
      for (int c = 0; c < C; ++c)
        Kh[(size_t)b * Nk * ldk + (size_t)spike * ldk + koff0 + c] =
            (h16)(4.0f * (float)Qh[(size_t)b * Nq * ldq + (size_t)(spike % Nq) * ldq + c]);
  }
  Dev<h16> dQ(Qh), dK(Kh), dV(Vt), dO((size_t)B * Nq * ldo);
  PfdAttnDesc d;
  memset(&d, 0, sizeof(d));
  d.Q = dQ.p; d.K = fused_layout ? dK.p + C : dK.p; d.Vt = dV.p; d.O = dO.p;
  d.ldq = ldq; d.ldk = ldk; d.ldvt = ldvt; d.ldo = ldo;
  d.q_bs = (long)Nq * ldq; d.k_bs = (long)Nk * ldk; d.vt_bs = Nkp; d.o_bs = (long)Nq * ldo;
  d.B = B; d.H = H; d.Nq = Nq; d.Nk = Nk; d.D = D; d.scale = scale;
  const int rc = pfd_attention_f16(&d, nullptr);
  char name[128];
  snprintf(name, sizeof(name), "attention B%d H%d Nq%d Nk%d D%d fused%d spike%d", B, H, Nq, Nk, D, (int)fused_layout, spike);
  if (rc != 0) { ++g_total; ++g_fail; printf("FAIL %-58s rc=%d (%s)\n", name, rc, pfd_last_error()); return; }
  auto got = dO.get();
  std::vector<double> ref(got.size(), 0.0);
  const int koff = fused_layout ? C : 0;
  std::vector<double> s(Nk);
  for (int b = 0; b < B; ++b)
    for (int h = 0; h < H; ++h)
      for (int i = 0; i < Nq; ++i) {
        double mx = -1e300;
        for (int j = 0; j < Nk; ++j) {
          double a = 0;
          for (int e = 0; e < D; ++e)
            a += (double)Qh[(size_t)b * Nq * ldq + i * ldq + h * D + e] * (double)Kh[(size_t)b * Nk * ldk + j * ldk + koff + h * D + e];
          s[j] = a * scale;
          mx = std::max(mx, s[j]);
        }
        double sum = 0;
        for (int j = 0; j < Nk; ++j) { s[j] = exp(s[j] - mx); sum += s[j]; }
        for (int e = 0; e < D; ++e) {
          double o = 0;
          for (int j = 0; j < Nk; ++j) o += s[j] * (double)Vt[(size_t)(h * D + e) * ldvt + b * Nkp + j];
          ref[(size_t)b * Nq * ldo + i * ldo + h * D + e] = o / sum;
        }
      }
  report(name, got, ref, 3e-3, 5e-3);
}

static void run_swin_case(int B, int H, int W, int nH, int shift) {
  const int C = nH * 32, ws = 12, NT = 144;
  const float scale = 1.0f / sqrtf(32.f);
  auto qkv = rand_h((size_t)B * H * W * 3 * C, 1.5f), qb = rand_h(3 * C, 0.5f), rpb = rand_h(529 * nH, 1.0f);
  Dev<h16> dq(qkv), db(qb), dr(rpb), dout((size_t)B * H * W * C);
  PfdSwinAttnDesc d;
  memset(&d, 0, sizeof(d));
  d.qkv = dq.p; d.qkv_bias = db.p; d.rpb = dr.p; d.out = dout.p;
  d.B = B; d.H = H; d.W = W; d.C = C; d.nH = nH; d.ws = ws; d.shift = shift; d.scale = scale;
  const int rc = pfd_swin_window_attention_f16(&d, nullptr);
  char name[128];
  snprintf(name, sizeof(name), "swin_attn B%d H%d W%d nH%d shift%d", B, H, W, nH, shift);
  if (rc != 0) { ++g_total; ++g_fail; printf("FAIL %-58s rc=%d (%s)\n", name, rc, pfd_last_error()); return; }
  auto got = dout.get();
  std::vector<double> ref(got.size(), 0.0);
  const int Hp = (H + ws - 1) / ws * ws, Wp = (W + ws - 1) / ws * ws;
  auto src = [&](int b, int y, int x, int col) -> double {
    if (y < H && x < W) return (double)qkv[((size_t)(b * H + y) * W + x) * 3 * C + col];
    return (double)qb[col];
  };
// ... 124 lines not shown
           keep_raw ? ", raw too (bitwise)" : ", raw tensor not written");
  }
  std::vector<double> ref(y2.size());
  const int cpg = N / 32;
  for (int b = 0; b < B; ++b)
    for (int g = 0; g < 32; ++g) {
      double sm = 0, q = 0;
      for (int p = 0; p < HW; ++p)
        for (int ch = g * cpg; ch < (g + 1) * cpg; ++ch) { const double v = (double)c2[((size_t)b * HW + p) * N + ch]; sm += v; q += v * v; }
      const double n = (double)HW * cpg, mean = sm / n, rstd = 1.0 / sqrt(q / n - mean * mean + eps);
      for (int p = 0; p < HW; ++p)
        for (int ch = g * cpg; ch < (g + 1) * cpg; ++ch)
          ref[((size_t)b * HW + p) * N + ch] = act_ref(((double)c2[((size_t)b * HW + p) * N + ch] - mean) * rstd * (double)gm[ch] + (double)bt[ch], act_gn);
    }
  report((std::string(name) + " [vs fp64]").c_str(), y, ref, 4e-3, 3e-3);
}

static void run_gnf_decline_case(int B, int H, int W, int Cin, int N) {
  const int HW = H * W, M = B * HW, K = 9 * Cin;
  Dev<h16> dA(rand_h((size_t)M * Cin)), dW(rand_h((size_t)N * K, 0.02f)), dB(rand_h(N, 0.5f)), dG(rand_h(N, 1.f)), dBt(rand_h(N, 0.5f));
  Dev<h16> dC((size_t)M * N), dY((size_t)M * N);
  Dev<float> dWS((size_t)8 * M * N + 64);
  HIP_OK(hipMemset(dC.p, 0x3C, (size_t)M * N * sizeof(h16)));
  HIP_OK(hipMemset(dY.p, 0x3C, (size_t)M * N * sizeof(h16)));
  PfdGemmDesc d;
  memset(&d, 0, sizeof(d));
  d.A = dA.p; d.W = dW.p; d.bias = dB.p; d.C = dC.p; d.lda = Cin; d.ldw = K; d.ldc = N; d.M = M; d.N = N; d.K = K; d.rows_per_rv = HW;
  d.ksize = 3; d.stride = 1; d.pad = 1; d.B = B; d.H = H; d.Wd = W; d.Cin = Cin; d.Ho = H; d.Wo = W;
  d.ws = dWS.p; d.ws_bytes = ((size_t)8 * M * N + 64) * sizeof(float);
  d.gnf_gamma = dG.p; d.gnf_beta = dBt.p; d.gnf_y = dY.p; d.gnf_ldy = N; d.gnf_eps = 1e-5f; d.gnf_act = PFD_ACT_SILU; d.gnf_rows = HW;
  const int rc = pfd_gemm_f16(&d, nullptr);
  HIP_OK(hipDeviceSynchronize());
  auto c = dC.get(), y = dY.get();
  size_t touched = 0;
  const unsigned short one = 0x3C3C;
  for (size_t i = 0; i < c.size(); ++i) touched += (memcmp(&c[i], &one, 2) != 0) + (memcmp(&y[i], &one, 2) != 0);
  ++g_total;
  char name[160];
  snprintf(name, sizeof(name), "conv3x3 B%d %dx%d %d->%d fused GroupNorm request declined", B, H, W, Cin, N);
  if (rc != PFD_ESHAPE || touched) { ++g_fail; printf("FAIL %-58s rc=%d, %zu elements written\n", name, rc, touched); }
  else printf("ok   %-58s PFD_ESHAPE, nothing written\n", name);
}

static void run_gn_pstats_case(int B, int HW, int C1, int C2, int act, float eps) {
  const int C = C1 + C2, G = 32, cpg = C / G;
  auto x1 = rand_h((size_t)B * HW * C1), x2 = rand_h((size_t)B * HW * std::max(C2, 8)), gm = rand_h(C), bt = rand_h(C);
  for (auto& v : x1) v = (h16)((float)v * 1.5f + 0.3f);
  auto mk_stats = [&](const std::vector<h16>& x, int Cs) {
    const int cpp = Cs / 32, tn = Cs / 160;
    std::vector<float> st((size_t)(B * HW / 64) * tn * 32, 0.f);
    for (int sl = 0; sl < B * HW / 64; ++sl)
      for (int c = 0; c < Cs; ++c) {
        double a = 0, q = 0;
        for (int r = 0; r < 64; ++r) { const double v = (double)x[(size_t)(sl * 64 + r) * Cs + c]; a += v; q += v * v; }
        const size_t o = (((size_t)sl * tn + c / 160) * 16 + (c % 160) / cpp) * 2;
        st[o] += (float)a; st[o + 1] += (float)q;
      }
    return st;
  };
  auto s1 = mk_stats(x1, C1);
  std::vector<float> s2 = C2 ? mk_stats(x2, C2) : std::vector<float>(2, 0.f);
  Dev<h16> d1(x1), d2(x2), dg(gm), db(bt), dy((size_t)B * HW * C);
  Dev<float> ds1(s1), ds2(s2);
  char name[160];
  snprintf(name, sizeof(name), "groupnorm pstats B%d HW%d C%d+%d act%d", B, HW, C1, C2, act);
  if (!pfd_groupnorm_takes_pstats(B, C1, C2, HW, G)) { ++g_total; ++g_fail; printf("FAIL %s: shape refused\n", name); return; }
  const int rc = pfd_groupnorm_pstats_f16(d1.p, C1, C1, ds1.p, C2 ? d2.p : nullptr, C2, C2, C2 ? ds2.p : nullptr, dg.p, db.p, dy.p, C,
                                          B, HW, G, eps, act, nullptr);
  if (rc != 0) { ++g_total; ++g_fail; printf("FAIL %s rc=%d (%s)\n", name, rc, pfd_last_error()); return; }
  auto got = dy.get();
  std::vector<double> ref((size_t)B * HW * C);
  auto at = [&](int b, int r, int c) { return c < C1 ? (double)x1[((size_t)b * HW + r) * C1 + c] : (double)x2[((size_t)b * HW + r) * C2 + c - C1]; };
  for (int b = 0; b < B; ++b)
    for (int g = 0; g < G; ++g) {
      double a = 0, q = 0;
      for (int r = 0; r < HW; ++r)
        for (int c = g * cpg; c < (g + 1) * cpg; ++c) { const double v = at(b, r, c); a += v; q += v * v; }
      const double n = (double)HW * cpg, mean = a / n, rstd = 1.0 / sqrt(std::max(q / n - mean * mean, 0.0) + eps);
      for (int r = 0; r < HW; ++r)
        for (int c = g * cpg; c < (g + 1) * cpg; ++c)
          ref[((size_t)b * HW + r) * C + c] = act_ref((at(b, r, c) - mean) * rstd * (double)gm[c] + (double)bt[c], act);
    }
  report(name, got, ref, 6e-3, 4e-3);
}

static void run_gn_conv_case(int B, int H, int W, int C1, int C2, int N, int act, bool with_res) {
  const int C = C1 + C2, HW = H * W, G = 32, M = B * HW, K = 9 * C;
  const float eps = 1e-5f;
  auto x1 = rand_h((size_t)M * C1, 2.f), x2 = rand_h((size_t)M * std::max(C2, 8), 1.f);
  for (auto& v : x1) v = (h16)((float)v + 0.7f);
  auto gm = rand_h(C, 1.f), bt = rand_h(C, 0.5f);
  auto Wt = rand_h((size_t)N * K, 0.05f), bias = rand_h(N, 0.5f), R = rand_h((size_t)M * N, 1.f);
  auto rv = rand_h((size_t)B * N, 0.5f);
  Dev<h16> d1(x1), d2(x2), dg(gm), db(bt), dy((size_t)M * C), dW(Wt), dB(bias), dR(R), dRV(rv);
  Dev<h16> dC0((size_t)M * N), dC1((size_t)M * N);
  Dev<float> dT((size_t)B * C * 2);
  const size_t wsb = pfd_groupnorm_ws_bytes(B, C, HW);
  Dev<char> dws(wsb);
  Dev<float> dWS((size_t)8 * M * N + 64);
  char name[160];
  snprintf(name, sizeof(name), "gn-prologue conv B%d %dx%d C%d+%d N%d act%d res%d", B, H, W, C1, C2, N, act, (int)with_res);
  int rc = pfd_groupnorm_f16(d1.p, C1, C1, C2 ? d2.p : nullptr, C2, C2, dg.p, db.p, dy.p, C, B, HW, G, eps, act, dws.p,
                             wsb, nullptr);
  PfdGemmDesc d;
  memset(&d, 0, sizeof(d));
  d.ws = dWS.p; d.ws_bytes = ((size_t)8 * M * N + 64) * sizeof(float);
  d.A = dy.p; d.W = dW.p; d.bias = dB.p; d.rowvec = dRV.p; d.R = with_res ? dR.p : nullptr; d.C = dC0.p;
  d.lda = C; d.ldw = K; d.ldr = N; d.ldc = N; d.ldrv = N;
  d.M = M; d.N = N; d.K = K; d.rows_per_rv = HW;
  d.ksize = 3; d.stride = 1; d.pad = 1; d.B = B; d.H = H; d.Wd = W; d.Cin = C; d.Ho = H; d.Wo = W;
  if (rc == 0) rc = pfd_gemm_f16_ex(&d, 10800, nullptr);
  if (rc == 0)
    rc = pfd_groupnorm_table_f16(d1.p, C1, C1, C2 ? d2.p : nullptr, C2, C2, dg.p, db.p, dT.p, B, HW, G, eps, dws.p, wsb,
                                 nullptr);
  d.A = d1.p; d.lda = C1; d.A2 = C2 ? d2.p : nullptr; d.lda2 = C2; d.gn_c1 = C1; d.gn_table = dT.p; d.gn_act = act;
  d.C = dC1.p;
  if (rc == 0) rc = pfd_gemm_f16(&d, nullptr);
  ++g_total;
  if (rc != 0) { ++g_fail; printf("FAIL %-58s rc=%d (%s)\n", name, rc, pfd_last_error()); return; }
  auto c0 = dC0.get(), c1 = dC1.get();
  size_t bad = 0;
  double worst = 0, mag = 0;
  for (size_t i = 0; i < c0.size(); ++i) {
    const double a = (double)c0[i], b = (double)c1[i];
    if (!(a == b)) { ++bad; worst = std::max(worst, fabs(a - b)); }
    mag = std::max(mag, fabs(a));
  }
  if (bad) { ++g_fail; printf("FAIL %-58s %zu of %zu differ, max |d| %.4g (max |ref| %.3g)\n", name, bad, c0.size(), worst, mag); }
  else printf("ok   %-58s identical (%zu values, max |ref| %.3g)\n", name, c0.size(), mag);
  d.Wd = 8; d.H = H * W / 8; d.Ho = d.H; d.Wo = 8;
  ++g_total;
  const int rc2 = pfd_gemm_f16(&d, nullptr);
  if (rc2 != PFD_ESHAPE) { ++g_fail; printf("FAIL %-58s W=8 with gn_table: rc=%d, expected PFD_ESHAPE\n", name, rc2); }
}

static void run_ln_case(int M, int C, int gather4, int B, int H, int W) {
  const int Cq = C / 4;
  auto x = rand_h(gather4 ? (size_t)B * H * W * Cq : (size_t)M * C, 2.f);
  for (auto& v : x) v = (h16)((float)v - 0.4f);
  auto gm = rand_h(C, 1.f), bt = rand_h(C, 0.5f);
  Dev<h16> dx(x), dg(gm), db(bt), dy((size_t)M * C);
  const int rc = pfd_layernorm_f16(dx.p, gather4 ? Cq : C, dg.p, db.p, dy.p, C, M, C, 1e-5f, gather4, B, H, W, nullptr);
  char name[128];
  snprintf(name, sizeof(name), "layernorm M%d C%d gather%d", M, C, gather4);
  if (rc != 0) { ++g_total; ++g_fail; printf("FAIL %-58s rc=%d (%s)\n", name, rc, pfd_last_error()); return; }
  auto got = dy.get();
  std::vector<double> ref(got.size());
  const int Ho = (H + 1) / 2, Wo = (W + 1) / 2;
  for (int m = 0; m < M; ++m) {
    std::vector<double> row(C);
    for (int c = 0; c < C; ++c) {
      if (!gather4) row[c] = (double)x[(size_t)m * C + c];
      else {
        const int b = m / (Ho * Wo), oy = (m % (Ho * Wo)) / Wo, ox = m % Wo, part = c / Cq;
        const int iy = 2 * oy + (part & 1), ix = 2 * ox + (part >> 1);
        row[c] = (iy < H && ix < W) ? (double)x[(((size_t)b * H + iy) * W + ix) * Cq + c % Cq] : 0.0;
      }
    }
    double s = 0; for (double v : row) s += v;
    const double mean = s / C;
    double q = 0; for (double v : row) q += (v - mean) * (v - mean);
    const double rstd = 1.0 / sqrt(q / C + 1e-5);
    for (int c = 0; c < C; ++c) ref[(size_t)m * C + c] = (row[c] - mean) * rstd * (double)gm[c] + (double)bt[c];
  }
  report(name, got, ref, 4e-3, 3e-3);
}
// ... 747 lines not shown
      const double M = q[0], N = q[1], K = q[2];
      const double nout = q[3] == PFD_ACT_GEGLU ? N / 2 : N;
      const double Mz = M - q[20];
      const double abytes = q[8] > 0 ? 2.0 * q[12] * q[13] * q[14] * q[15] : 2.0 * Mz * K;
      const double bytes = abytes + 2.0 * N * K + 2.0 * M * nout + (q[6] ? 2.0 * M * nout : 0) + (q[5] ? 2.0 * M * N / std::max<double>(1, std::min<long>(q[18], M)) : 0);
      const double flops = 2.0 * Mz * N * K;
      const double us = a.ms / a.n * 1e3;
      const double ideal = std::max(flops / 2.5e15, bytes / 8e12) * 1e6;
      tot += a.ms; tot_ideal += ideal * a.n * 1e-3;
      printf("%7ld %6ld %6ld %ld %ld %ld %3ld %2ld %ld %4ld %5ld %ld | %3d %9.1f %8.1f %8.1f %8.1f %8.2f\n", q[0], q[1], q[2], q[8], q[9], q[11], q[3], q[5], q[6],
             q[19], q[20], q[21], a.n, us, flops / us * 1e-6, bytes / us * 1e-3, ideal, a.ms);
    }
    printf("total %.2f ms per UNet pass (GEMM/conv only); roofline-ideal %.2f ms\n", tot, tot_ideal);
  }
  return bad;
}

int main(int argc, char** argv) {
  if (argc > 2 && !strcmp(argv[1], "--replay")) return replay(argv[2]);
  if (argc > 1 && !strcmp(argv[1], "--launch-floor")) { bench_launch_floor(); return 0; }
  if (argc > 1 && !strcmp(argv[1], "--winograd")) return winograd_main();
  if (argc > 1 && !strcmp(argv[1], "--bench-patch")) {
    bench_gemm("conv3x3 320->320 @64^2", 0, 320, 0, 3, 8, 64, 320, 0);
    bench_gemm("conv3x3 640->640 @32^2", 0, 640, 0, 3, 8, 32, 640, 0);
    bench_gemm("conv3x3 1280->1280 @16^2", 0, 1280, 0, 3, 8, 16, 1280, 0);
    bench_gemm("conv3x3 320->320 @64^2 implicit GEMM", 0, 320, 0, 3, 8, 64, 320, 5400);
    return 0;
  }
  if (argc > 1 && !strcmp(argv[1], "--bench-gn-conv")) {
    bench_gn_conv("320->320 @64^2", 16, 64, 320, 0, 320);
    bench_gn_conv("640->320 @64^2 (skip concat)", 16, 64, 320, 320, 320);
    bench_gn_conv("960->320 @64^2 (skip concat)", 16, 64, 640, 320, 320);
    bench_gn_conv("640->640 @32^2", 16, 32, 640, 0, 640);
    bench_gn_conv("1280->640 @32^2 (skip concat)", 16, 32, 640, 640, 640);
    bench_gn_conv("1920->640 @32^2 (skip concat)", 16, 32, 1280, 640, 640);
    return 0;
  }
  if (argc > 1 && !strcmp(argv[1], "--gemm-new")) {
    for (int v : {5100, 5300, 9200, 9300}) {
      run_gemm_case({1100, 320, 1024, 0, true, true, true, false, v});
      run_gemm_case({300, 320, 192, PFD_ACT_SILU, true, true, true, false, v});
      run_gemm_case({77, 160, 64, 0, true, false, false, false, v, 8});
      run_gemm_case({0, 160, 0, 0, true, true, false, false, v, 0, 3, 1, 1, 0, 3, 16, 16, 128});
      run_gemm_case({900, 320, 1536, 0, true, false, false, false, v + 3});
      run_gemm_case({200, 320, 128, PFD_ACT_GEGLU, true, false, false, false, v});
    }
    { GemmCase t{520, 480, 128, 0, false, false, false, false, 5100}; t.n_split = 320; run_gemm_case(t); }
    { GemmCase t{520, 480, 128, 0, false, false, false, false, 9200}; t.n_split = 320; run_gemm_case(t); }
    run_gemm_case({600, 640, 320, PFD_ACT_GEGLU, true, false, false, false, 9400});
    run_gemm_case({300, 320, 64, PFD_ACT_GEGLU, false, false, false, false, 9400});
    run_tiled_weight_cases();
    printf("SELFTEST %d/%d passed, %d failed\n", g_total - g_fail, g_total, g_fail);
    return g_fail;
  }
  if (argc > 1 && !strcmp(argv[1], "--r5")) {
    run_gnf_case(8, 16, 16, 1280, 1280, PFD_ACT_SILU, 1e-5f, false, true, false);
    run_gnf_case(8, 8, 8, 1280, 1280, PFD_ACT_SILU, 1e-5f, false, true, false);
    run_gnf_case(8, 8, 8, 2560, 1280, PFD_ACT_SILU, 1e-5f, false, true, false);
    run_gnf_case(8, 16, 16, 640, 1280, PFD_ACT_SILU, 1e-5f, false, true, false);
    run_gnf_case(8, 16, 16, 1280, 1280, PFD_ACT_NONE, 1e-6f, true, false, true);
    run_gnf_case(4, 8, 8, 1280, 1280, PFD_ACT_SILU, 1e-5f, true, true, true);
    run_gnf_case(8, 16, 16, 1280, 1280, PFD_ACT_SILU, 1e-5f, false, true, false, 10802);
    run_gnf_case(8, 8, 8, 1280, 1280, PFD_ACT_SILU, 1e-5f, false, true, false, 3308);
    run_gnf_decline_case(8, 64, 64, 320, 320);
    run_gnf_case(8, 32, 32, 640, 640, PFD_ACT_SILU, 1e-5f, false, true, false);
    run_gnf_case(8, 32, 32, 640, 640, PFD_ACT_SILU, 1e-5f, true, false, true);
    run_gnf_case(8, 32, 32, 1280, 640, PFD_ACT_SILU, 1e-5f, false, true, false);
    run_gnf_case(4, 32, 32, 320, 640, PFD_ACT_SILU, 1e-5f, false, true, false);
    for (int v : {0, 9200, 9300, 3200, 3300, 5400, 5800}) {
      { GemmCase c{1024, 320, 256, 0, true, true, true, false, v}; c.res_rows = 512; run_gemm_case(c); }
      if (v != 5800) { GemmCase c{1024, 320, 256, 0, true, true, false, false, v}; c.res_rows = 512; c.zero_rows = 512; run_gemm_case(c); }
      { GemmCase c{1024, 320, 320, 0, true, true, false, false, v}; c.res_rows = 512; c.gn_out = 1; run_gemm_case(c); }
    }
    { GemmCase c{1024, 320, 2048, 0, true, true, false, false, 3304}; c.res_rows = 512; run_gemm_case(c); }
    { GemmCase c{1024, 320, 2048, 0, true, true, false, false, 3304}; c.res_rows = 512; c.gn_out = 1; run_gemm_case(c); }
    { GemmCase c{512, 1280, 2048, 0, true, true, true, false, 3304}; c.gn_out = 1; run_gemm_case(c); }
    { GemmCase c{0, 320, 0, 0, true, true, true, false, 9302, 0, 3, 1, 1, 0, 2, 16, 16, 128}; c.gn_out = 1; run_gemm_case(c); }
    run_gn_case(8, 64, 1280, 0, 32, PFD_ACT_SILU, 1e-5f);
    run_gn_case(8, 256, 1280, 1280, 32, PFD_ACT_SILU, 1e-5f);
    run_gn_pstats_case(8, 4096, 320, 0, PFD_ACT_SILU, 1e-5f);
    run_gn_pstats_case(8, 4096, 320, 320, PFD_ACT_SILU, 1e-5f);
    run_gn_pstats_case(3, 1024, 640, 0, PFD_ACT_NONE, 1e-6f);
    run_gn_pstats_case(2, 256, 1280, 1280, PFD_ACT_SILU, 1e-5f);
    printf("SELFTEST %d/%d passed, %d failed\n", g_total - g_fail, g_total, g_fail);
    return g_fail;
  }
  if (argc > 1 && !strcmp(argv[1], "--ups-fold")) {
    run_ups_fold_cases();
    if (argc > 2 && !strcmp(argv[2], "full")) {
      { GemmCase c{0, 640, 0, 0, true, false, false, false, 0, 0, 3, 1, 1, 2, 8, 32, 32, 640}; c.gn_out = 1; run_gemm_case(c); }
      { GemmCase c{0, 1280, 0, 0, true, false, false, false, 0, 0, 3, 1, 1, 2, 8, 16, 16, 1280}; c.gn_out = 1; run_gemm_case(c); }
    }
    printf("SELFTEST %d/%d passed, %d failed\n", g_total - g_fail, g_total, g_fail);
    return g_fail;
  }
  if (argc > 1 && !strcmp(argv[1], "--patch-wide")) {
    for (int v : {0, 10800, 10900}) {
      run_gemm_case({0, 160, 0, PFD_ACT_SILU, true, true, true, false, v, 0, 3, 1, 1, 0, 1, 16, 48, 128});
      run_gemm_case({0, 320, 0, 0, true, true, true, false, v, 0, 3, 1, 1, 0, 2, 8, 96, 64});
      run_gemm_case({0, 160, 0, 0, true, false, true, false, v, 0, 3, 1, 1, 0, 1, 32, 96, 128});
      run_gemm_case({0, 160, 0, 0, true, true, false, false, v, 0, 3, 1, 1, 0, 3, 32, 48, 64});
    }
    run_gemm_case({0, 160, 0, 0, true, true, true, false, 10802, 0, 3, 1, 1, 0, 1, 16, 96, 256});
    { GemmCase c{0, 320, 0, 0, true, true, true, false, 0, 0, 3, 1, 1, 0, 2, 16, 96, 128}; c.w_tiled = 1; run_gemm_case(c); }
    run_gemm_case({0, 160, 0, 0, true, true, false, false, 5400, 0, 3, 1, 1, 0, 1, 16, 48, 128});
    printf("SELFTEST %d/%d passed, %d failed\n", g_total - g_fail, g_total, g_fail);
    return g_fail;
  }
  if (argc > 1 && !strcmp(argv[1], "--narrow")) {
    run_narrow_conv_cases();
    bench_gemm("unet head conv 320->4 @64^2 B8", 8 * 4096, 4, 2880, 3, 8, 64, 320, 0);
    bench_gemm("unet head conv 320->4 @96^2 B4", 4 * 9216, 4, 2880, 3, 4, 96, 320, 0);
    bench_gemm("vae conv_out 128->3 @512^2 B4", 4 * 262144, 3, 1152, 3, 4, 512, 128, 0);
    bench_gemm("unet head conv, round-5 kernel", 8 * 4096, 4, 2880, 3, 8, 64, 320, 11);
    bench_gemm("vae conv_out, round-5 kernel", 4 * 262144, 3, 1152, 3, 4, 512, 128, 21);
    printf("SELFTEST %d/%d passed, %d failed\n", g_total - g_fail, g_total, g_fail);
    return g_fail;
  }
  if (argc > 1 && !strcmp(argv[1], "--image")) {
    run_image();
    printf("SELFTEST %d/%d passed, %d failed\n", g_total - g_fail, g_total, g_fail);
    return g_fail;
  }
  if (argc > 1 && !strcmp(argv[1], "--elementwise")) {
    run_elementwise();
    printf("SELFTEST %d/%d passed, %d failed\n", g_total - g_fail, g_total, g_fail);
    return g_fail;
  }
  if (argc > 1 && !strcmp(argv[1], "--ln")) {
    run_ln_fold_suite();
    printf("SELFTEST %d/%d passed, %d failed\n", g_total - g_fail, g_total, g_fail);
    return g_fail;
  }
  if (argc > 1 && !strcmp(argv[1], "--attn")) {
    run_attn_case(2, 2, 128, 128, 40, true);
    run_attn_case(1, 2, 300, 148, 40, false);
    run_attn_case(2, 2, 512, 256, 40, true);
    run_attn_case(1, 1, 256, 40, 40, false);
    run_attn_case(1, 2, 520, 1000, 40, false);
    run_attn_case(1, 2, 77, 64, 40, true);
    run_attn_case(1, 2, 200, 148, 40, false);
    run_attn_case(2, 2, 64, 64, 80, true);
    run_attn_case(1, 2, 144, 256, 96, false);
    run_attn_case(1, 3, 148, 148, 96, false);
    run_attn_case(2, 2, 64, 148, 160, false);
    run_attn_case(1, 1, 256, 320, 160, true);
    run_attn_case(1, 2, 520, 1000, 40, false, 700);
    run_attn_case(2, 2, 512, 256, 40, true, 130);
    run_attn_case(1, 2, 300, 148, 40, false, 140);
    run_attn_case(1, 2, 512, 1024, 40, true, 700);
    run_attn_case(1, 1, 700, 640, 40, false, 333);
    run_attn_case(8, 8, 1024, 1024, 40, true, 500);
    printf("SELFTEST %d/%d passed, %d failed\n", g_total - g_fail, g_total, g_fail);
    return g_fail;
  }
  if (argc > 1 && !strcmp(argv[1], "--attn512")) {
    run_attn_case(2, 1, 256, 256, 512, false);
    run_attn_case(1, 1, 200, 96, 512, false);
    run_attn_case(1, 1, 128, 32, 512, false);
    run_attn_case(2, 1, 128, 512, 512, true);
    run_attn_case(1, 1, 128, 512, 512, false, 300);
    bench_attn("vae mid attention 64^2 d512", 4, 1, 4096, 4096, 512);
    bench_attn("vae mid attention 96^2 d512", 2, 1, 9216, 9216, 512);
    printf("%d checks, %d failed\n", g_total, g_fail);
    return g_fail ? 1 : 0;
  }
  if (argc > 1 && !strcmp(argv[1], "--bench-attn")) {
    bench_attn("self-attn 64^2 d40", 8, 8, 4096, 4096, 40);
    bench_attn("self-attn 64^2 d40 (CFG prefix)", 4, 8, 4096, 4096, 40);
    bench_attn("self-attn 96^2 d40 (C5)", 4, 8, 9216, 9216, 40);
    bench_attn("self-attn 32^2 d80", 8, 8, 1024, 1024, 80);
    bench_attn("self-attn 16^2 d160", 8, 8, 256, 256, 160);
    bench_attn("cross-attn 64^2 d40", 4, 8, 4096, 148, 40);
    bench_attn("seecoder cross d96", 1, 8, 144, 4096, 96);
    bench_attn("cross-attn 64^2 d40, 64 keys", 4, 8, 4096, 64, 40);
    bench_attn("cross-attn 64^2 d40, 8 keys", 4, 8, 4096, 8, 40);
    bench_attn("cross-attn 32^2 d80", 4, 8, 1024, 148, 80);
    bench_attn("cross-attn 32^2 d80, 8 keys", 4, 8, 1024, 8, 80);
    bench_attn("cross-attn 16^2 d160", 4, 8, 256, 148, 160);
    bench_attn("cross-attn 16^2 d160, 8 keys", 4, 8, 256, 8, 160);
    bench_attn("self-attn 16^2 d160, 64 keys", 8, 8, 256, 64, 160);
    return 0;
  }
  if (argc > 1 && !strcmp(argv[1], "--bench-gn")) {
    bench_gn("groupnorm+silu 320 @64^2", 8, 4096, 320);
    bench_gn("groupnorm+silu 640 @64^2", 8, 4096, 640);
    bench_gn("groupnorm+silu 640 @32^2", 8, 1024, 640);
    bench_gn("groupnorm+silu 1280 @32^2", 8, 1024, 1280);
    bench_gn("groupnorm+silu 1280 @16^2", 8, 256, 1280);
    bench_gn("groupnorm+silu 2560 @16^2", 8, 256, 2560);
    bench_gn("groupnorm+silu 1280 @8^2", 8, 64, 1280);
    bench_gn("groupnorm+silu 128 @512^2", 4, 262144, 128);
    bench_ln("layernorm 320 @64^2", 32768, 320);
    bench_ln("layernorm 640 @32^2", 8192, 640);
    bench_ln("layernorm 1280 @16^2", 2048, 1280);
    return 0;
  }
  if (argc > 2 && !strcmp(argv[1], "--replay-time")) return replay(argv[2], true, argc > 3 ? atoi(argv[3]) : 0);
  const bool bench = argc > 1 && !strcmp(argv[1], "--bench");
  const bool only_bench = argc > 1 && !strcmp(argv[1], "--only-bench");
  hipDeviceProp_t prop;
  HIP_OK(hipGetDeviceProperties(&prop, 0));
  printf("device: %s  CUs=%d  abi=%d\n", prop.name, prop.multiProcessorCount, pfd_abi_version());

  if (!only_bench) {
    const int tiles[] = {22, 21, 12, 11};
    for (int t : tiles) {
      run_gemm_case({256, 256, 128, 0, true, false, false, false, t});
// ... 190 lines not shown
```

### prompt-free-diffusion_amd/lib/hip/binding.py

```python
import ctypes as C
import os

_LIB = None
_LIB_PATH = os.path.normpath(os.path.join(os.path.dirname(os.path.abspath(__file__)), "..", "..", "libpfd_hip.so"))

ABI_VERSION = 10

ACT_NONE, ACT_GELU, ACT_RELU, ACT_SILU, ACT_GEGLU = 0, 1, 2, 3, 4

_i32, _i64, _f32, _vp, _sz = C.c_int32, C.c_int64, C.c_float, C.c_void_p, C.c_size_t


class PfdGemmDesc(C.Structure):
    _fields_ = [
        ("A", _vp), ("W", _vp), ("bias", _vp), ("rowvec", _vp), ("R", _vp), ("C", _vp),
        ("lda", _i64), ("ldw", _i64), ("ldr", _i64), ("ldc", _i64), ("ldrv", _i64),
        ("M", _i32), ("N", _i32), ("K", _i32),
        ("rows_per_rv", _i32), ("act", _i32), ("bias_per_row", _i32),
        ("ksize", _i32), ("stride", _i32), ("pad", _i32), ("ups", _i32),
        ("B", _i32), ("H", _i32), ("Wd", _i32), ("Cin", _i32), ("Ho", _i32), ("Wo", _i32),
        ("ws", _vp), ("ws_bytes", _sz),
        ("Ct", _vp), ("ldct", _i64), ("n_split", _i32), ("w_tiled", _i32),
        ("gn_table", _vp), ("A2", _vp), ("lda2", _i64), ("gn_c1", _i32), ("gn_act", _i32),
        ("ln_stats", _vp), ("ln_colsum", _vp), ("ln_parts", _i32), ("ln_eps", _f32), ("ln_out", _vp),
        ("k_split", _i32), ("zero_rows", _i32), ("gn_out", _vp),
        ("gnf_gamma", _vp), ("gnf_beta", _vp), ("gnf_y", _vp), ("gnf_ldy", _i64), ("gnf_eps", _f32), ("gnf_act", _i32),
        ("gnf_rows", _i32), ("gnf_skip_raw", _i32), ("res_rows", _i32),
    ]


class PfdAttnDesc(C.Structure):
    _fields_ = [
        ("Q", _vp), ("K", _vp), ("Vt", _vp), ("O", _vp),
        ("ldq", _i64), ("ldk", _i64), ("ldvt", _i64), ("ldo", _i64),
        ("q_bs", _i64), ("k_bs", _i64), ("vt_bs", _i64), ("o_bs", _i64),
        ("B", _i32), ("H", _i32), ("Nq", _i32), ("Nk", _i32), ("D", _i32),
        ("scale", _f32),
    ]


class PfdSwinAttnDesc(C.Structure):
    _fields_ = [
        ("qkv", _vp), ("qkv_bias", _vp), ("rpb", _vp), ("out", _vp),
        ("B", _i32), ("H", _i32), ("W", _i32), ("C", _i32), ("nH", _i32), ("ws", _i32), ("shift", _i32),
        ("scale", _f32),
    ]


SIGNATURES = {
    "pfd_abi_version": (_i32, []),
    "pfd_last_error": (C.c_char_p, []),
    "pfd_gemm_f16": (_i32, [C.POINTER(PfdGemmDesc), _vp]),
    "pfd_gemm_f16_ex": (_i32, [C.POINTER(PfdGemmDesc), _i32, _vp]),
    "pfd_gemm_geglu_group": (_i32, [_i32]),
    "pfd_attention_f16": (_i32, [C.POINTER(PfdAttnDesc), _vp]),
    "pfd_swin_window_attention_f16": (_i32, [C.POINTER(PfdSwinAttnDesc), _vp]),
    "pfd_groupnorm_ws_bytes": (_sz, [_i32, _i32, _i32]),
    "pfd_groupnorm_table_f16": (_i32, [_vp, _i32, _i64, _vp, _i32, _i64, _vp, _vp, _vp, _i32, _i32, _i32, _f32, _vp, _sz,
                                       _vp]),
    "pfd_groupnorm_f16": (_i32, [_vp, _i32, _i64, _vp, _i32, _i64, _vp, _vp, _vp, _i64, _i32, _i32, _i32, _f32,
                                 _i32, _vp, _sz, _vp]),
    "pfd_groupnorm_takes_pstats": (_i32, [_i32, _i32, _i32, _i32, _i32]),
    "pfd_groupnorm_pstats_f16": (_i32, [_vp, _i32, _i64, _vp, _vp, _i32, _i64, _vp, _vp, _vp, _vp, _i64, _i32, _i32, _i32,
                                        _f32, _i32, _vp]),
    "pfd_layernorm_f16": (_i32, [_vp, _i64, _vp, _vp, _vp, _i64, _i32, _i32, _f32, _i32, _i32, _i32, _i32, _vp]),
    "pfd_ln_rowstats_f16": (_i32, [_vp, _i64, _i32, _i32, _vp, _vp]),
    "pfd_softmax_rows_f16": (_i32, [_vp, _i64, _vp, _i64, _i32, _i32, _f32, _vp]),
    "pfd_nchw_to_nhwc_f16": (_i32, [_vp, _i32, _vp, _i32, _i32, _i32, _i32, _f32, _f32, _i32, _vp]),
    "pfd_nhwc_to_nchw": (_i32, [_vp, _vp, _i32, _i32, _i32, _i32, _i32, _f32, _f32, _f32, _f32, _vp]),
    "pfd_im2col_f16": (_i32, [_vp, _i64, _vp, _i32, _i32, _i32, _i32, _i32, _i32, _i32, _i32, _i32, _i32, _vp]),
    "pfd_timestep_embedding_f16": (_i32, [_vp, _vp, _i32, _i32, _f32, _vp]),
    "pfd_cfg_ddim_step": (_i32, [_vp, _i32, _vp, _vp, _vp, _vp, _vp, _vp, _i32, _i32, _i32, _i32, _i32, _vp]),
    "pfd_philox_normal_f32": (_i32, [_vp, _i32, _vp, _i32, _i64, _vp]),
    "pfd_cfg_ddim_step_rng": (_i32, [_vp, _i32, _vp, _vp, _i32, _f32, _vp, _vp, _vp, _vp, _i32, _i32, _i32, _i32, _i32,
                                     _vp]),
    "pfd_add_f16": (_i32, [_vp, _vp, _vp, _i64, _vp]),
    "pfd_axpby_f16": (_i32, [_vp, _f32, _vp, _f32, _vp, _i64, _vp]),
    "pfd_add_rowvec_f16": (_i32, [_vp, _i64, _vp, _vp, _i64, _i32, _i32, _vp]),
    "pfd_add_rowvec_lnstats_f16": (_i32, [_vp, _i64, _vp, _vp, _i64, _i32, _i32, _vp, _vp]),
    "pfd_act_f16": (_i32, [_vp, _vp, _i64, _i32, _vp]),
    "pfd_image_u8_f16": (_i32, [_vp, _vp, _i64, _f32, _f32, _i32, _vp]),
    "pfd_image_resample_check": (_i32, [_i32, _i32, _i32, _i32, _i32, _i32]),
    "pfd_image_resample_h_u8": (_i32, [_vp, _vp, _i32, _i32, _i32, _i32, _i32, _vp, _vp, _vp, _i32, _vp]),
    "pfd_image_resample_v_u8": (_i32, [_vp, _vp, _i32, _i32, _i32, _i32, _i32, _i32, _vp, _vp, _vp, _i32, _vp]),
    "pfd_prof_enable": (_i32, [_i32]),
    "pfd_prof_read": (_i32, [_i32, C.POINTER(C.c_double), C.POINTER(_i64), C.POINTER(C.c_double),
                             C.POINTER(C.c_double)]),
    "pfd_prof_bucket_name": (C.c_char_p, [_i32]),
    "pfd_prof_num_buckets": (_i32, []),
}


def lib_path():
    return os.environ.get("PFD_HIP_LIB", _LIB_PATH)


def load():
    global _LIB
    if _LIB is not None:
        return _LIB
    path = lib_path()
    if not os.path.exists(path):
        raise RuntimeError(
            f"libpfd_hip.so not found at {path}: build it with `python __graft_entry__.py` "
            "(or `make -C prompt-free-diffusion_amd/csrc`).  There is no CPU/torch fallback.")
    lib = C.CDLL(path)
    for name, (res, args) in SIGNATURES.items():
        fn = getattr(lib, name, None)
        if fn is None:
            raise RuntimeError(f"{path} does not export {name}")
        fn.restype = res
        fn.argtypes = args
    v = lib.pfd_abi_version()
    if v != ABI_VERSION:
        raise RuntimeError(f"libpfd_hip.so ABI {v} != binding ABI {ABI_VERSION}")
    _LIB = lib
    return lib


class PfdError(RuntimeError):
    pass


IMG_U8, IMG_NCHW_F16, IMG_NCHW_F32, IMG_NHWC_F16 = 0, 1, 2, 3

PFD_EINVAL, PFD_ESHAPE, PFD_ELAUNCH = -1, -2, -3
_ERR = {PFD_EINVAL: "PFD_EINVAL", PFD_ESHAPE: "PFD_ESHAPE", PFD_ELAUNCH: "PFD_ELAUNCH"}


def check(rc, what):
    if rc != 0:
        msg = load().pfd_last_error().decode(errors="replace")
        raise PfdError(f"{what} failed: {_ERR.get(rc, rc)} {msg}")


def prof_enable(on=True):
    check(load().pfd_prof_enable(1 if on else 0), "pfd_prof_enable")


def prof_read():
    lib = load()
    out = []
    for b in range(lib.pfd_prof_num_buckets()):
        ms, n, fl, by = C.c_double(), _i64(), C.c_double(), C.c_double()
        check(lib.pfd_prof_read(b, C.byref(ms), C.byref(n), C.byref(fl), C.byref(by)), "pfd_prof_read")
        if n.value:
            out.append(dict(bucket=b, name=lib.pfd_prof_bucket_name(b).decode(), ms=ms.value, launches=n.value,
# ... 3 lines not shown
```

### prompt-free-diffusion_amd/lib/hip/ops.py

```python
import ctypes as C
import functools
import os
import threading

import torch

from . import binding as _b
from .binding import ACT_GEGLU, ACT_GELU, ACT_NONE, ACT_RELU, ACT_SILU

_byref = C.byref


def _lib():
    return _b.load()


def _stream():
    return torch.cuda.current_stream().cuda_stream


def _ptr(t):
    return t.data_ptr() if t is not None else None


# ... 20 lines not shown


_TRACE = os.environ.get("PFD_TRACE_GEMM")
_TRACE_GN = os.environ.get("PFD_TRACE_GN")
LN_FOLD = True


TRACE_FIELDS = ("M", "N", "K", "act", "has_bias", "has_rowvec", "has_res", "bias_per_row",
                "ksize", "stride", "pad", "ups", "B", "H", "W", "Cin", "Ho", "Wo", "rows_per_rv",
                "k_split", "zero_rows", "gn_out", "gnf", "res_rows")
TRACE_FIELDS_ABI7 = 19
TRACE_FIELDS_ABI8 = 22


def trace_record(d):
    return tuple(int(v) for v in (
        d.M, d.N, d.K, d.act, d.bias is not None, d.rowvec is not None, d.R is not None, d.bias_per_row,
        d.ksize, d.stride, d.pad, d.ups, d.B, d.H, d.Wd, d.Cin, d.Ho, d.Wo, d.rows_per_rv,
        d.k_split, d.zero_rows, bool(d.gn_out), (2 if d.gnf_skip_raw else 1) if d.gnf_y else 0, d.res_rows))


def parse_launch_records(path, distinct=True):
    import collections
    Rec = collections.namedtuple("LaunchRecord", TRACE_FIELDS)
    seen, out = set(), []
    for ln, line in enumerate(open(path), 1):
        v = tuple(int(t) for t in line.split())
        if not v:
            continue
        if len(v) in (TRACE_FIELDS_ABI7, TRACE_FIELDS_ABI8):
            v = v + (0,) * (len(TRACE_FIELDS) - len(v))
        if len(v) != len(TRACE_FIELDS):
            raise ValueError(f"{path}:{ln}: {len(v)} fields, expected {len(TRACE_FIELDS)} ({' '.join(TRACE_FIELDS)})")
        if distinct and v in seen:
            continue
        seen.add(v)
        out.append(Rec(*v))
    return out


def _trace(d):
    with open(_TRACE, "a") as f:
        f.write(" ".join(str(v) for v in trace_record(d)) + "\n")


def _chk16(t, what):
    if t.dtype != torch.float16:
        raise TypeError(f"{what}: expected float16, got {t.dtype}")
    if not t.is_cuda:
        raise RuntimeError(f"{what}: tensor is on {t.device}; the HIP path has no CPU fallback")
    if t.stride(-1) != 1:
        raise ValueError(f"{what}: innermost stride must be 1")


def _rows(t):
    cols = t.shape[-1]
    if t.dim() == 1:
        return 1, cols, cols
    ld = t.stride(-2)
    rows = t.numel() // cols
    exp = ld
    for d in range(t.dim() - 2, -1, -1):
        if t.shape[d] != 1 and t.stride(d) != exp:
            raise ValueError(f"tensor of shape {tuple(t.shape)} strides {t.stride()} is not a strided matrix")
        exp *= t.shape[d]
    return rows, cols, ld


def ln_fold_ok(C):
    return LN_FOLD and C % 160 == 0 and C // 160 <= 8 and C % 64 == 0


def ln_rowstats(x, out=None):
    _chk16(x, "ln_rowstats x")
    M, Cc, ld = _rows(x)
    if out is None:
        out = torch.empty((M, Cc // 160, 2), dtype=torch.float32, device=x.device)
    elif out.dtype != torch.float32 or not out.is_contiguous() or out.numel() != M * (Cc // 160) * 2:
        raise ValueError("ln_rowstats: out must be a contiguous float32 [M, C/160, 2]")
    _b.check(_lib().pfd_ln_rowstats_f16(x.data_ptr(), ld, M, Cc, out.data_ptr(), _stream()), "pfd_ln_rowstats_f16")
    return out


GN_PSTATS = True


def gn_stats_wanted(B, HW, N, M=None):
    if not GN_PSTATS or N not in (320, 640, 1280) or HW % 64 or (M is not None and M != B * HW):
        return False
    return bool(_lib().pfd_groupnorm_takes_pstats(B, N, 0, HW, 32))


def _new_gn_stats(M, N, device):
    return torch.empty((M // 64, N // 160, 16, 2), dtype=torch.float32, device=device)


def set_gn_stats(t, stats):
    t._pfd_gn = (stats, t.data_ptr(), tuple(t.shape), t._version)
    return t


def get_gn_stats(t):
    ent = getattr(t, "_pfd_gn", None)
    if ent is None or ent[1] != t.data_ptr() or ent[2] != tuple(t.shape) or ent[3] != t._version:
        return None
    return ent[0]


def _written(out, stats=None):
    if out is not None:
        torch._C._increment_version((out,))
    if stats is not None:
        set_gn_stats(out, stats)
    elif out is not None and getattr(out, "_pfd_gn", None) is not None:
        out._pfd_gn = None
    if out is not None and getattr(out, "_pfd_normed", None) is not None:
        out._pfd_normed = None
    return out


def set_normed(t, key, y):
    t._pfd_normed = (key, t.data_ptr(), tuple(t.shape), y, t._version)
    return t


def get_normed(t, key):
    ent = getattr(t, "_pfd_normed", None)
    if ent is None or ent[0] != key or ent[1] != t.data_ptr() or ent[2] != tuple(t.shape) or ent[4] != t._version:
        return None
    return ent[3]


def cat_pair(t):
    out = torch.cat([t, t])
    st = get_gn_stats(t)
    if st is not None:
        set_gn_stats(out, torch.cat([st, st]))
    return out


GEMM_FUSE = True


def wide_tile_ok(N, K):
    return GEMM_FUSE and (N % 160 == 0 or N % 128 == 0) and K % 64 == 0


def gemm(a, w, *, bias=None, rowvec=None, rows_per_rv=1, res=None, act=ACT_NONE, out=None,
         bias_per_row=False, n=None, k=None, tile=0, out_t=None, n_split=None, ln=None, ln_out=None,
         a2=None, zero_rows=0, gn_out=False, res_rows=None):
    _chk16(a, "gemm A")
    _chk16(w, "gemm W")
    M, Ka, lda = _rows(a)
    Nw, Kw, ldw = _rows(w)
    N = Nw if n is None else n
    K = min(Ka, Kw) if k is None else k
    if a2 is not None:
        _chk16(a2, "gemm A2")
        M2, Ka2, lda2 = _rows(a2)
        if M2 != M or a2.device != a.device:
            raise ValueError(f"gemm: a2 {tuple(a2.shape)} does not pair with a {tuple(a.shape)}")
        if k is None:
            K = Ka + Ka2
        if Ka % 64 or Ka >= K or K - Ka > Ka2:
            raise ValueError(f"gemm: a2 needs a first source of a multiple of 64 columns below K (Ka {Ka}, K {K})")
    if zero_rows:
        if zero_rows < 0 or ln is not None:
            raise ValueError("gemm: zero_rows must be >= 0 and cannot be combined with ln=")
        M += zero_rows
    n_out = N // 2 if act == ACT_GEGLU else N
    if out_t is not None:
        n_out = n_split
    if out is None:
        out = torch.empty((M, n_out), dtype=torch.float16, device=a.device)
    else:
        _chk16(out, "gemm out")
        if out.device != a.device or out.shape[-1] != n_out or out.numel() != M * n_out:
            raise ValueError(f"gemm: out {tuple(out.shape)} on {out.device} cannot hold [{M}, {n_out}] on {a.device}")
    _, _, ldc = _rows(out)
    d = _b.PfdGemmDesc()
    if out_t is not None:
        _chk16(out_t, "gemm out_t")
        if out_t.shape[0] != N - n_split or out_t.shape[1] < M or out_t.stride(1) != 1:
            raise ValueError(f"gemm: out_t {tuple(out_t.shape)} cannot hold [{N - n_split}, {M}]")
        d.Ct, d.ldct, d.n_split = out_t.data_ptr(), out_t.stride(0), n_split
    d.A, d.W, d.C = a.data_ptr(), w.data_ptr(), out.data_ptr()
    d.bias, d.rowvec, d.R = _ptr(bias), _ptr(rowvec), _ptr(res)
    d.lda, d.ldw, d.ldc = lda, ldw, ldc
    d.ldr = _rows(res)[2] if res is not None else 0
    d.ldrv = _rows(rowvec)[2] if rowvec is not None else 0
    d.M, d.N, d.K = M, N, K
    d.rows_per_rv, d.act, d.bias_per_row = rows_per_rv, act, 1 if bias_per_row else 0
    d.ksize = 0
    d.ws, d.ws_bytes = _workspace(a.device).data_ptr(), _WS_BYTES
    if a2 is not None:
        d.A2, d.lda2, d.k_split = a2.data_ptr(), lda2, Ka
    d.zero_rows = zero_rows
    if res_rows is not None:
        if res is None or M != 2 * res_rows or _rows(res)[0] != res_rows:
            raise ValueError(f"gemm: res_rows {res_rows} needs a residual of exactly that many rows and M == 2 * res_rows (M {M})")
        d.res_rows = res_rows
    elif res is not None and _rows(res)[0] != M:
        raise ValueError(f"gemm: residual of {_rows(res)[0]} rows for {M} output rows (res_rows= names a shared one)")
    if ln is not None:
        st, cs, eps = ln
        if st.dtype != torch.float32 or not st.is_contiguous() or st.dim() != 3 or st.shape[0] != M or \
                st.shape[1] * 160 != K or st.shape[2] != 2 or st.device != a.device:
            raise ValueError(f"gemm: ln stats {tuple(st.shape)} {st.dtype} do not describe a [{M}, {K}] operand")
        if cs.dtype != torch.float32 or cs.numel() != N or not cs.is_contiguous() or cs.device != a.device:
            raise ValueError("gemm: ln column sums must be a contiguous float32 [N]")
        d.ln_stats, d.ln_colsum, d.ln_parts, d.ln_eps = st.data_ptr(), cs.data_ptr(), st.shape[1], float(eps)
    stats = None
    if ln_out is not None and ln_out is not False:
        if ln_out is True:
            stats = torch.empty((M, N // 160, 2), dtype=torch.float32, device=a.device)
        else:
            stats = ln_out
            if stats.dtype != torch.float32 or not stats.is_contiguous() or stats.numel() != M * (N // 160) * 2:
                raise ValueError("gemm: ln_out must be a contiguous float32 [M, N/160, 2]")
        d.ln_out = stats.data_ptr()
    gst = None
    if gn_out:
        gst = _new_gn_stats(M, N, a.device)
        d.gn_out = gst.data_ptr()
    if _TRACE:
        _trace(d)
    lib = _lib()
    rc = lib.pfd_gemm_f16_ex(_byref(d), tile, _stream()) if tile else lib.pfd_gemm_f16(_byref(d), _stream())
    _b.check(rc, f"pfd_gemm_f16 M{M} N{N} K{K}")
    _written(out, gst)
    return out if stats is None else (out, stats)


def conv_gn_fusable(B, H, W_, C1, C2, N, ksize=3, stride=1, pad=1):
    return (ksize == 3 and stride == 1 and pad == 1 and W_ in (32, 64) and H % (256 // W_) == 0 and
            (B * H * W_) % 256 == 0 and N % 160 == 0 and C1 % 64 == 0 and C2 % 64 == 0)


_GNF_DECLINED = set()


UPS_FOLD = os.environ.get("PFD_UPS_FOLD", "1") != "0"
_UPS_FOLD_DECLINED = set()


def ups_fold_key(x, N, act, bias, out, gn_out):
    return (tuple(x.shape), int(N), int(act), bias is not None, bool(gn_out), int(x.stride(2)),
            int(N) if out is None else int(_rows(out)[2]), str(x.device))


def ups_fold_declined(key):
    return key in _UPS_FOLD_DECLINED


def conv(x, w, ksize, *, stride=1, pad=None, ups=False, bias=None, rowvec=None, res=None, act=ACT_NONE,
         out=None, tile=0, out_hw=None, rows_per_rv=None, gn=None, gn_out=False, gn_fuse=None):
    _chk16(x, "conv x")
    _chk16(w, "conv W")
    B, H, W_, Cin = x.shape
    x2 = None
    if gn is not None:
        table, x2, gn_silu = gn
        C1 = Cin
        if x2 is not None:
            _chk16(x2, "conv x2")
            if x2.shape[:3] != x.shape[:3] or x2.device != x.device:
                raise ValueError(f"conv: x2 {tuple(x2.shape)} does not match x {tuple(x.shape)}")
            ld2 = x2.stride(2)
            if x2.stride(1) != ld2 * W_ or (B > 1 and x2.stride(0) != ld2 * W_ * H):
                raise ValueError("conv: x2 must be dense over (B, H, W)")
            Cin = C1 + x2.shape[-1]
        if table.dtype != torch.float32 or table.device != x.device or tuple(table.shape) != (B, 2, Cin) or \
                not table.is_contiguous():
            raise ValueError(f"conv: gn table {tuple(table.shape)} {table.dtype} is not a float32 [{B}, 2, {Cin}]")
    if x.stride(2) < x.shape[-1]:
        raise ValueError("conv: bad pixel stride")
    lda = x.stride(2)
    if x.stride(1) != lda * W_ or (B > 1 and x.stride(0) != lda * W_ * H):
        raise ValueError("conv: image must be dense over (B, H, W)")
    if pad is None:
        pad = ksize // 2
    Hin, Win = (2 * H, 2 * W_) if ups else (H, W_)
    Ho = (Hin + 2 * pad - ksize) // stride + 1
    Wo = (Win + 2 * pad - ksize) // stride + 1
    if out_hw is not None:
        Ho, Wo = out_hw
    phase = ups == 2
    if phase:
        if gn is not None or gn_fuse is not None:
            raise ValueError("conv: ups=2 cannot be combined with gn= / gn_fuse=")
        if ksize != 3 or w.dim() != 3 or tuple(w.shape[::2]) != (4, 4 * Cin) or not w.is_contiguous():
            raise ValueError(f"conv: ups=2 takes the folded weight [4, N, {4 * Cin}] of a 3x3 convolution, got {tuple(w.shape)}")
        N, K, ldw = w.shape[1], w.shape[2], w.shape[2]
        fold_key = ups_fold_key(x, N, act, bias, out, gn_out)
        if tile == 0 and fold_key in _UPS_FOLD_DECLINED:
            return None
    else:
        N, K, ldw = _rows(w)
        if K != ksize * ksize * Cin:
            raise ValueError(f"conv: packed weight K {K} != {ksize}*{ksize}*{Cin}")
    M = B * Ho * Wo
    if out is None:
        out = torch.empty((B, Ho, Wo, N), dtype=torch.float16, device=x.device)
# ... 42 lines not shown
        if _TRACE:
            _trace(d)
        return (_written(out) if g_keep else None), y
    if gn_out and gn is None and gn_stats_wanted(B, Ho * Wo, N) and Cin % 64 == 0:
        gst = _new_gn_stats(M, N, x.device)
        d.gn_out = gst.data_ptr()
    if phase:
        lib = _lib()
        rc = lib.pfd_gemm_f16_ex(_byref(d), tile, _stream()) if tile else lib.pfd_gemm_f16(_byref(d), _stream())
        if rc == _b.PFD_ESHAPE:
            if tile == 0:
                _UPS_FOLD_DECLINED.add(fold_key)
            return None
        _b.check(rc, f"pfd_gemm_f16(conv, phase-folded upsample) M{M} N{N} K{K}")
        if _TRACE:
            _trace(d)
        return _written(out, gst)
    if _TRACE:
        _trace(d)
    lib = _lib()
    rc = lib.pfd_gemm_f16_ex(_byref(d), tile, _stream()) if tile else lib.pfd_gemm_f16(_byref(d), _stream())
    _b.check(rc, f"pfd_gemm_f16(conv) M{M} N{N} K{K}" + (" with GroupNorm prologue" if gn is not None else ""))
    return _written(out, gst)


def im2col(x, ksize, stride, pad, kpad, ho=None, wo=None):
    _chk16(x, "im2col x")
    B, H, W_, Cin = x.shape
    Ho = (H + 2 * pad - ksize) // stride + 1 if ho is None else ho
    Wo = (W_ + 2 * pad - ksize) // stride + 1 if wo is None else wo
    col = torch.empty((B * Ho * Wo, kpad), dtype=torch.float16, device=x.device)
    rc = _lib().pfd_im2col_f16(x.data_ptr(), x.stride(2), col.data_ptr(), B, H, W_, Cin, ksize, stride, pad,
                               Ho, Wo, kpad, _stream())
    _b.check(rc, "pfd_im2col_f16")
    return col, Ho, Wo


def conv_narrow(x, w, ksize, *, stride=1, pad=None, bias=None, rowvec=None, res=None, act=ACT_NONE,
                ho=None, wo=None, out=None, gn_out=False):
    if pad is None:
        pad = ksize // 2
    B = x.shape[0]
    col, Ho, Wo = im2col(x, ksize, stride, pad, w.shape[1], ho, wo)
    N = w.shape[0]
    o2 = None if out is None else out.view(-1, out.shape[-1])
    gn_out = bool(gn_out) and gn_stats_wanted(B, Ho * Wo, N) and wide_tile_ok(N, w.shape[1])
    y = gemm(col, w, bias=bias, rowvec=rowvec, rows_per_rv=Ho * Wo, res=res, act=act, out=o2, gn_out=gn_out)
    r = y.view(B, Ho, Wo, N) if out is None else out
    return _written(r, get_gn_stats(y) if gn_out else None)


def attention(q, k, vt, B, H, Nq, Nk, D, scale, *, ldq, ldk, ldvt, q_bs, k_bs, vt_bs, out=None):
    if out is None:
        out = torch.empty((B * Nq, H * D), dtype=torch.float16, device=q.device)
    d = _b.PfdAttnDesc()
    d.Q, d.K, d.Vt, d.O = q.data_ptr(), k.data_ptr(), vt.data_ptr(), out.data_ptr()
    d.ldq, d.ldk, d.ldvt, d.ldo = ldq, ldk, ldvt, out.stride(-2)
    d.q_bs, d.k_bs, d.vt_bs, d.o_bs = q_bs, k_bs, vt_bs, Nq * out.stride(-2)
    d.B, d.H, d.Nq, d.Nk, d.D = B, H, Nq, Nk, D
    d.scale = scale
    _b.check(_lib().pfd_attention_f16(_byref(d), _stream()), f"pfd_attention_f16 B{B} H{H} Nq{Nq} Nk{Nk} D{D}")
    return out


def swin_window_attention(qkv, qkv_bias, rpb, B, H, W_, Cdim, nH, ws, shift, scale):
    _chk16(qkv, "swin qkv")
    out = torch.empty((B * H * W_, Cdim), dtype=torch.float16, device=qkv.device)
    d = _b.PfdSwinAttnDesc()
    d.qkv, d.qkv_bias, d.rpb, d.out = qkv.data_ptr(), qkv_bias.data_ptr(), rpb.data_ptr(), out.data_ptr()
    d.B, d.H, d.W, d.C, d.nH, d.ws, d.shift = B, H, W_, Cdim, nH, ws, shift
    d.scale = scale
    _b.check(_lib().pfd_swin_window_attention_f16(_byref(d), _stream()), "pfd_swin_window_attention_f16")
    return out


def groupnorm(x, gamma, beta, groups, eps, *, x2=None, silu=False, out=None):
    _chk16(x, "groupnorm x")
    B = x.shape[0]
    C1 = x.shape[-1]
    HW = x.numel() // (B * C1)
    C2 = 0 if x2 is None else x2.shape[-1]
    if out is None:
        out = torch.empty(tuple(x.shape[:-1]) + (C1 + C2,), dtype=torch.float16, device=x.device)
    lib = _lib()
    st1 = get_gn_stats(x) if GN_PSTATS else None
    st2 = get_gn_stats(x2) if (GN_PSTATS and x2 is not None) else None
    if _TRACE_GN:
        with open(_TRACE_GN, "a") as f:
            f.write(f"{B} {HW} {C1} {C2} {int(st1 is not None)} {int(x2 is None or st2 is not None)} "
                    f"{int(bool(lib.pfd_groupnorm_takes_pstats(B, C1, C2, HW, groups)))}\n")
    if st1 is not None and (x2 is None or st2 is not None) and groups == 32 and \
            lib.pfd_groupnorm_takes_pstats(B, C1, C2, HW, groups):
        rc = lib.pfd_groupnorm_pstats_f16(x.data_ptr(), C1, x.stride(-2), st1.data_ptr(), _ptr(x2), C2,
                                          0 if x2 is None else x2.stride(-2), _ptr(st2), gamma.data_ptr(), beta.data_ptr(),
                                          out.data_ptr(), out.stride(-2), B, HW, groups, eps,
                                          ACT_SILU if silu else ACT_NONE, _stream())
        _b.check(rc, f"pfd_groupnorm_pstats_f16 B{B} HW{HW} C{C1}+{C2}")
        return _written(out)
    wsb = lib.pfd_groupnorm_ws_bytes(B, C1 + C2, HW)
    ws = torch.empty(wsb, dtype=torch.uint8, device=x.device)
    rc = lib.pfd_groupnorm_f16(x.data_ptr(), C1, x.stride(-2), _ptr(x2), C2, 0 if x2 is None else x2.stride(-2),
                               gamma.data_ptr(), beta.data_ptr(), out.data_ptr(), out.stride(-2), B, HW, groups,
                               eps, ACT_SILU if silu else ACT_NONE, ws.data_ptr(), wsb, _stream())
    _b.check(rc, f"pfd_groupnorm_f16 B{B} HW{HW} C{C1}+{C2}")
    return _written(out)


def groupnorm_table(x, gamma, beta, groups, eps, *, x2=None):
    _chk16(x, "groupnorm_table x")
    B = x.shape[0]
    C1 = x.shape[-1]
    HW = x.numel() // (B * C1)
    C2 = 0 if x2 is None else x2.shape[-1]
    if x2 is not None:
        _chk16(x2, "groupnorm_table x2")
    table = torch.empty((B, 2, C1 + C2), dtype=torch.float32, device=x.device)
    lib = _lib()
    wsb = lib.pfd_groupnorm_ws_bytes(B, C1 + C2, HW)
    ws = torch.empty(wsb, dtype=torch.uint8, device=x.device)
    rc = lib.pfd_groupnorm_table_f16(x.data_ptr(), C1, x.stride(-2), _ptr(x2), C2, 0 if x2 is None else x2.stride(-2),
                                     gamma.data_ptr(), beta.data_ptr(), table.data_ptr(), B, HW, groups, eps,
                                     ws.data_ptr(), wsb, _stream())
    _b.check(rc, f"pfd_groupnorm_table_f16 B{B} HW{HW} C{C1}+{C2}")
    return table


def layernorm(x, gamma, beta, eps=1e-5, out=None):
    _chk16(x, "layernorm x")
    M, Cdim, ldx = _rows(x)
    if out is None:
        out = torch.empty(x.shape, dtype=torch.float16, device=x.device)
    rc = _lib().pfd_layernorm_f16(x.data_ptr(), ldx, gamma.data_ptr(), beta.data_ptr(), out.data_ptr(),
                                  _rows(out)[2], M, Cdim, eps, 0, 0, 0, 0, _stream())
    _b.check(rc, f"pfd_layernorm_f16 M{M} C{Cdim}")
    return _written(out)


def layernorm_patch_merge(x, gamma, beta, eps=1e-5):
    _chk16(x, "layernorm_patch_merge x")
    B, H, W_, Cq = x.shape
    Ho, Wo = (H + 1) // 2, (W_ + 1) // 2
    out = torch.empty((B * Ho * Wo, 4 * Cq), dtype=torch.float16, device=x.device)
    rc = _lib().pfd_layernorm_f16(x.data_ptr(), x.stride(2), gamma.data_ptr(), beta.data_ptr(), out.data_ptr(),
                                  4 * Cq, B * Ho * Wo, 4 * Cq, eps, 1, B, H, W_, _stream())
    _b.check(rc, "pfd_layernorm_f16(gather4)")
    return out


def softmax_rows(x, scale, out=None):
    _chk16(x, "softmax x")
    R, N, ldx = _rows(x)
    if out is None:
        out = torch.empty((R, N), dtype=torch.float16, device=x.device)
    _b.check(_lib().pfd_softmax_rows_f16(x.data_ptr(), ldx, out.data_ptr(), _rows(out)[2], R, N, scale, _stream()),
             "pfd_softmax_rows_f16")
    return out


def to_nhwc(x, mul=1.0, add=0.0, rep=1):
    if not x.is_cuda:
        raise RuntimeError("to_nhwc: input must live on the GPU; the HIP path has no CPU fallback")
    if x.dtype not in (torch.float32, torch.float16):
        x = x.float()
    x = x.contiguous()
    B, Cc, H, W_ = x.shape
    out = torch.empty((rep * B, H, W_, Cc), dtype=torch.float16, device=x.device)
    rc = _lib().pfd_nchw_to_nhwc_f16(x.data_ptr(), 1 if x.dtype == torch.float32 else 0, out.data_ptr(), B, Cc, H,
                                     W_, mul, add, rep, _stream())
    _b.check(rc, "pfd_nchw_to_nhwc_f16")
    return out


def to_nchw(x, dtype=torch.float16, mul=1.0, add=0.0, lo=-65504.0, hi=65504.0):
    _chk16(x, "to_nchw x")
    B, H, W_, Cc = x.shape
    if not x.is_contiguous():
        raise ValueError("to_nchw: dense NHWC expected")
    out = torch.empty((B, Cc, H, W_), dtype=torch.float32 if dtype == torch.float32 else torch.float16,
                      device=x.device)
    rc = _lib().pfd_nhwc_to_nchw(x.data_ptr(), out.data_ptr(), 1 if dtype == torch.float32 else 0, B, Cc, H, W_,
                                 mul, add, lo, hi, _stream())
# ... 168 lines not shown
```

### prompt-free-diffusion_amd/lib/model_zoo/openaimodel.py

```python
import copy
import os
from functools import partial

import torch
import torch.nn as nn

from ..hip import layers as L
from ..hip import ops
from .attention import ContextMix, SpatialTransformer, as_context_kv
from .common.get_model import register

symbol = 'openai'


def normalization(channels):
    return L.GroupNorm(32, channels)


def timestep_embedding(timesteps, dim, max_period=10000, repeat_only=False):
    if repeat_only:
        return timesteps[:, None].to(torch.float16).repeat(1, dim)
    return ops.timestep_embedding(timesteps, dim, float(max_period))


# ... 30 lines not shown

    def forward(self, x, emb, context=None):
        semb = ops.activation(emb.to(torch.float16).contiguous(), ops.ACT_SILU) if emb is not None else None
        y = self.hip(ops.to_nhwc(x), semb, as_context_kv(context))
        return ops.to_nchw(y, x.dtype)


class Upsample(nn.Module):

    def __init__(self, channels, use_conv, dims=2, out_channels=None, padding=1):
        super().__init__()
        assert dims == 2
        self.channels = channels
        self.out_channels = out_channels or channels
        self.use_conv = use_conv
        if use_conv:
            self.conv = L.Conv2d(self.channels, self.out_channels, 3, padding=padding)

    def hip(self, x):
        assert x.shape[-1] == self.channels
        if not self.use_conv:
            raise NotImplementedError("Upsample without conv is not on the hot path")
        return self.conv.hip(x, ups=True, gn_out=True)

    def forward(self, x):
        return ops.to_nchw(self.hip(ops.to_nhwc(x)), x.dtype)


class Downsample(nn.Module):
    def __init__(self, channels, use_conv, dims=2, out_channels=None, padding=1):
        super().__init__()
        assert dims == 2 and use_conv, "only the strided-conv form is on the hot path"
        self.channels = channels
        self.out_channels = out_channels or channels
        self.use_conv = use_conv
        self.op = L.Conv2d(self.channels, self.out_channels, 3, stride=2, padding=padding)

    def hip(self, x):
        assert x.shape[-1] == self.channels
        return self.op.hip(x, gn_out=True)

    def forward(self, x):
        return ops.to_nchw(self.hip(ops.to_nhwc(x)), x.dtype)


class ResBlock(TimestepBlock):
    fuse_groupnorm = False
    fuse_reduce_groupnorm = True

    def __init__(self, channels, emb_channels, dropout, out_channels=None, use_conv=False,
                 use_scale_shift_norm=False, dims=2, use_checkpoint=False, up=False, down=False):
        super().__init__()
        assert dims == 2 and not use_scale_shift_norm and not up and not down, \
            "configuration outside the SD-v1.5 / ControlNet hot path"
        self.channels = channels
        self.emb_channels = emb_channels
        self.dropout = dropout
        self.out_channels = out_channels or channels
        self.use_conv = use_conv
        self.use_checkpoint = use_checkpoint
        self.use_scale_shift_norm = use_scale_shift_norm
        self.updown = False
        self.in_layers = nn.Sequential(
            normalization(channels), nn.SiLU(), L.Conv2d(channels, self.out_channels, 3, padding=1))
        self.h_upd = self.x_upd = nn.Identity()
        self.emb_layers = nn.Sequential(nn.SiLU(), L.Linear(emb_channels, self.out_channels))
        out_conv = L.Conv2d(self.out_channels, self.out_channels, 3, padding=1)
        for p in out_conv.parameters():
            p.detach().zero_()
        self.out_layers = nn.Sequential(
            normalization(self.out_channels), nn.SiLU(), nn.Dropout(p=dropout), out_conv)
        if self.out_channels == channels:
            self.skip_connection = nn.Identity()
        elif use_conv:
            self.skip_connection = L.Conv2d(channels, self.out_channels, 3, padding=1)
        else:
            self.skip_connection = L.Conv2d(channels, self.out_channels, 1)

    def hip(self, x, semb, x2=None, emb=None, next_norm=None):
        C1 = x.shape[-1]
        C2 = 0 if x2 is None else x2.shape[-1]
        assert C1 + C2 == self.channels
        B, H, W_, _ = x.shape
        fuse = self.fuse_groupnorm
        fuse_in = fuse and ops.conv_gn_fusable(B, H, W_, C1, C2, self.out_channels)
        fuse_out = fuse and ops.conv_gn_fusable(B, H, W_, self.out_channels, 0, self.out_channels)
        rows_per_rv = None
        h_norm = None
        if emb is not None:
            table, cols, shared = emb
            c0 = cols[id(self)]
            e = table[:, c0:c0 + self.out_channels]
            if shared:
                rows_per_rv = 1 << 30
        else:
            e = self.emb_layers[1].hip(semb)
        if fuse_in:
            h = self.in_layers[2].hip(x, rowvec=e, rows_per_rv=rows_per_rv,
                                      gn=(self.in_layers[0].hip_table(x, x2), x2, True))
        else:
            hn = self.in_layers[0].hip(x, x2, silu=True)
            fused = None if fuse_out or not self.fuse_reduce_groupnorm else \
                self.in_layers[2].hip_gn(hn, self.out_layers[0], silu=True, rowvec=e, rows_per_rv=rows_per_rv)
            if fused is not None:
                h, h_norm = None, fused[1]
            else:
                h = self.in_layers[2].hip(hn, rowvec=e, rows_per_rv=rows_per_rv, gn_out=not fuse_out)
        skip = self.skip_connection
        if isinstance(skip, nn.Identity):
            assert x2 is None
            sk = x
        elif skip.kernel_size[0] == 1:
            w, b = skip._pk()
            B, H, W_, _ = x.shape
            if x2 is not None and ops.wide_tile_ok(w.shape[0], C1 + C2) and C1 % 64 == 0:
                sk = ops.gemm(x.view(-1, C1), w, bias=b, a2=x2.view(-1, C2), k=C1 + C2)
            else:
                sk = ops.gemm(x.view(-1, C1), w[:, :C1], bias=b, k=C1)
                if x2 is not None:
                    sk = ops.gemm(x2.view(-1, C2), w[:, C1:], res=sk, k=C2, out=sk)
            sk = sk.view(B, H, W_, -1)
        else:
            assert x2 is None
            sk = skip.hip(x)
        if fuse_out:
            return self.out_layers[3].hip(h, res=sk, gn=(self.out_layers[0].hip_table(h), None, True))
        if h_norm is None:
            h_norm = self.out_layers[0].hip(h, silu=True)
        if next_norm is not None and self.fuse_reduce_groupnorm:
            norm, nsilu = next_norm
            fused = self.out_layers[3].hip_gn(h_norm, norm, silu=nsilu, keep_raw=True, res=sk)
            if fused is not None:
                return ops.set_normed(fused[0], norm.fuse_key(nsilu), fused[1])
        return self.out_layers[3].hip(h_norm, res=sk, gn_out=True)

    def forward(self, x, emb):
        semb = ops.activation(emb.to(torch.float16).contiguous(), ops.ACT_SILU)
        return ops.to_nchw(self.hip(ops.to_nhwc(x), semb), x.dtype)


@register('openai_unet_2d_next')
class UNetModel2D_Next(nn.Module, L._Packed):
    def __init__(self, in_channels, model_channels, out_channels, num_res_blocks, attention_resolutions,
                 context_dim, dropout=0, channel_mult=(1, 2, 4, 8), conv_resample=True, use_checkpoint=False,
                 num_heads=8, num_head_channels=None, parts=['global', 'data', 'context']):
        super().__init__()
        self.in_channels = in_channels
        self.model_channels = model_channels
        self.out_channels = out_channels
        if isinstance(num_res_blocks, int):
            num_res_blocks = len(channel_mult) * [num_res_blocks]
        elif len(num_res_blocks) != len(channel_mult):
            raise ValueError("provide num_res_blocks either as an int (globally constant) or "
                             "as a list/tuple (per-level) with the same length as channel_mult")
        self.num_res_blocks = num_res_blocks
        self.attention_resolutions = attention_resolutions
        self.context_dim = context_dim
        self.dropout = dropout
        self.channel_mult = channel_mult
        self.conv_resample = conv_resample
        self.use_checkpoint = use_checkpoint
        self.num_heads = num_heads
        self.num_head_channels = num_head_channels
        assert (num_heads is None) + (num_head_channels is None) == 1, \
            "One of num_heads or num_head_channels need to be set"
        self.parts = parts if isinstance(parts, list) else [parts]
# ... 77 lines not shown
        self.parameter_group = {}
        if self.glayer_included:
            self.parameter_group['global'] = self.time_embed
        if self.dlayer_included:
            self.parameter_group['data'] = self.data_blocks
        if self.clayer_included:
            self.parameter_group['context'] = self.context_blocks

    def get_d_head_n_heads(self, ch):
        if self.num_head_channels is None:
            return ch // self.num_heads, self.num_heads
        return self.num_head_channels, ch // self.num_head_channels

    def add_data_layer(self, layer):
        if self.dlayer_included:
            layers = layer if isinstance(layer, (list, tuple)) else [layer]
            self.data_blocks.append(TimestepEmbedSequential(*layers))
        self._order.append('d')

    def add_context_layer(self, layer):
        if self.clayer_included:
            layers = layer if isinstance(layer, (list, tuple)) else [layer]
            self.context_blocks.append(TimestepEmbedSequential(*layers))
        self._order.append('c')

    def silu_time_embedding(self, timesteps):
        t_emb = timestep_embedding(timesteps, self.model_channels)
        h = self.time_embed[0].hip(t_emb, act=ops.ACT_SILU)
        return self.time_embed[2].hip(h, act=ops.ACT_SILU)

    def _emb_pack(self):
        blocks = [m for seq in self.data_blocks for m in seq if isinstance(m, ResBlock)]
        params = [b.emb_layers[1].weight for b in blocks] + [b.emb_layers[1].bias for b in blocks]

        def build():
            w = torch.cat([L._dev16(b.emb_layers[1].weight) for b in blocks], 0).contiguous()
            bias = torch.cat([L._dev16(b.emb_layers[1].bias) for b in blocks], 0).contiguous()
            cols, off = {}, 0
            for b in blocks:
                cols[id(b)] = off
                off += b.out_channels
            return w, bias, cols
        return self._packed("emb_cat", build, *params)

    def emb_projections(self, timesteps):
        w, bias, cols = self._emb_pack()
        return ops.gemm(self.silu_time_embedding(timesteps), w, bias=bias), cols

    def hip(self, x, timesteps, context, control=None, context_net=None, emb_table=None, cfg_pair=False):
        cnet = self if context_net is None else context_net
        if emb_table is not None:
            emb = (emb_table, self._emb_pack()[2], True)
        else:
            table, cols = self.emb_projections(timesteps)
            emb = (table, cols, False)
        semb = None
        d_iter = iter(self.data_blocks)
        pair = [bool(cfg_pair)]
        if isinstance(context, ContextMix):
            if cfg_pair:
                raise NotImplementedError("cfg_pair with multi-context mixing")
            c_iters = [iter(n.context_blocks) for n in context.nets]
            ctx_layer = lambda hh: context.mix([next(it) for it in c_iters], hh, semb)
        else:
            c_iter = iter(cnet.context_blocks)

            def ctx_layer(hh):
                p, pair[0] = pair[0], False
                return next(c_iter).hip(hh, semb, context, cfg_pair=p)
        ccs = list(control) if control is not None else None
        hs = []
        h = x
        nn_of = self._next_norms(cnet, control is not None) if not isinstance(context, ContextMix) else {}
        step = [0]

        def data_layer(hh, x2=None):
            return next(d_iter).hip(hh, semb, x2=x2, emb=emb, next_norm=nn_of.get(step[0]))
        for ltype in self.i_order:
            if ltype == 'd':
                h = data_layer(h)
            elif ltype == 'c':
                h = ctx_layer(h)
            else:
                hs.append(ops.cat_pair(h) if pair[0] else h)
            step[0] += 1
        if pair[0]:
            raise ValueError("cfg_pair: no context layer in the input half of this UNet")
        for ltype in self.m_order:
            h = data_layer(h) if ltype == 'd' else ctx_layer(h)
            step[0] += 1
        if ccs is not None:
            h = ops.add(h, ccs.pop())
        skip = None
        for ltype in self.o_order:
            if ltype == 'load_hidden_feature':
                skip = hs.pop()
                if ccs is not None:
                    skip = ops.add(skip, ccs.pop())
            elif ltype == 'd':
                h, skip = data_layer(h, x2=skip), None
            else:
                h = ctx_layer(h)
            step[0] += 1
        return h

    def _next_norms(self, cnet, with_control):
        import weakref
        cache = self.__dict__.setdefault("_nn_cache", {})
        key = (bool(with_control), len(cnet.context_blocks), len(self.data_blocks), tuple(self.i_order), tuple(self.m_order),
               tuple(self.o_order))
        ent = cache.get(key)
        if ent is not None and ent[0]() is cnet:
            return ent[1]
        order = list(self.i_order) + list(self.m_order) + list(self.o_order)
        d_list, c_list = list(self.data_blocks), list(cnet.context_blocks)
        di = ci = 0
        seq = []
        for lt in order:
            if lt == 'd':
                seq.append(('d', d_list[di]))
                di += 1
            elif lt == 'c':
                seq.append(('c', c_list[ci]))
                ci += 1
            else:
                seq.append((lt, None))
        n_in, n_mid = len(self.i_order), len(self.m_order)
        out = {}
        for i, (kind, mod) in enumerate(seq):
            if kind != 'd' or not isinstance(mod[len(mod) - 1], ResBlock):
                continue
            j = i + 1
            while j < len(seq) and seq[j][0] not in ('d', 'c', 'load_hidden_feature'):
                j += 1
            if j >= len(seq) or seq[j][0] == 'load_hidden_feature':
                continue
            if with_control and i == n_in + n_mid - 1:
                continue
            fn = seq[j][1].first_norm()
            if fn is not None:
                out[i] = fn
        cache[key] = (weakref.ref(cnet), out)
        return out

    def forward(self, x, timesteps, context):
        y = self.hip(ops.to_nhwc(x), timesteps, as_context_kv(context))
        return ops.to_nchw(y, x.dtype)
```

Baseline: 8.609 images/s.

## Wrap half-batch skip sources instead of duplicating; fuse split-K reduce with LN row stats

Under the CFG pair trick, UNet skip tensors stored before the first context layer were duplicated with cat_pair to double the batch. Now they stay at half batch: the GEMM A2 loader and the GroupNorm pstats apply path wrap row indices for the second source, which removes the concat copies and their memory traffic. A second change adds a split-K reduction kernel that also emits the per-160-column LayerNorm row statistics, so a separate stats pass is no longer needed. Both are on by default behind env switches. They add new wrap constraints and a fallback path that still concatenates when the preconditions are not met.

```diff
diff --git a/include/pfd_hip.h b/include/pfd_hip.h
--- a/include/pfd_hip.h
+++ b/include/pfd_hip.h
@@ -69,11 +69,14 @@
   int32_t gnf_rows;
   int32_t gnf_skip_raw;
   int32_t res_rows;
+  int32_t a2_rows;
 } PfdGemmDesc;
 int pfd_gemm_f16(const PfdGemmDesc* d, pfd_stream_t stream);
 int pfd_gemm_f16_ex(const PfdGemmDesc* d, int32_t tile, pfd_stream_t stream);
 
 int32_t pfd_gemm_geglu_group(int32_t N);
+
+int32_t pfd_gemm_ln_reduce_fused(int32_t on);
 
 typedef struct PfdAttnDesc {
   const void* Q;
@@ -102,6 +105,10 @@
 int pfd_groupnorm_pstats_f16(const void* x1, int32_t C1, int64_t ldx1, const void* st1, const void* x2, int32_t C2,
                              int64_t ldx2, const void* st2, const void* gamma, const void* beta, void* y, int64_t ldy,
                              int32_t B, int32_t HW, int32_t G, float eps, int32_t act, pfd_stream_t stream);
+int pfd_groupnorm_pstats_wrap_f16(const void* x1, int32_t C1, int64_t ldx1, const void* st1, const void* x2, int32_t C2,
+                                  int64_t ldx2, const void* st2, const void* gamma, const void* beta, void* y, int64_t ldy,
+                                  int32_t B, int32_t HW, int32_t G, float eps, int32_t act, int32_t x2_rows,
+                                  pfd_stream_t stream);
 
 int pfd_groupnorm_table_f16(const void* x1, int32_t C1, int64_t ldx1, const void* x2, int32_t C2, int64_t ldx2,
                             const void* gamma, const void* beta, void* table, int32_t B, int32_t HW, int32_t G,
diff --git a/prompt-free-diffusion_amd/csrc/gemm_conv.hip b/prompt-free-diffusion_amd/csrc/gemm_conv.hip
--- a/prompt-free-diffusion_amd/csrc/gemm_conv.hip
+++ b/prompt-free-diffusion_amd/csrc/gemm_conv.hip
@@ -433,6 +433,10 @@
     pfd_set_error("pfd_gemm_f16: a residual stored once for a doubled batch is read by the wide-tile kernels only (see PfdGemmDesc.res_rows)");
     return PFD_ESHAPE;
   }
+  if (d->a2_rows > 0 && d->a2_rows != d->M) {
+    pfd_set_error("pfd_gemm_f16: a second source stored once for a doubled batch needs k_split, no zero_rows and M / 2 <= a2_rows < M (see PfdGemmDesc.a2_rows)");
+    return PFD_ESHAPE;
+  }
   if (d->gnf_y) {
     pfd_set_error("pfd_gemm_f16: the fused GroupNorm lives in the split-K reduction of the wide-tile kernels only (see PfdGemmDesc.gnf_y)");
     return PFD_ESHAPE;
diff --git a/prompt-free-diffusion_amd/csrc/gemm_glds.hip b/prompt-free-diffusion_amd/csrc/gemm_glds.hip
--- a/prompt-free-diffusion_amd/csrc/gemm_glds.hip
+++ b/prompt-free-diffusion_amd/csrc/gemm_glds.hip
@@ -49,6 +49,7 @@
   int k_split;
   int zero_rows;
   int r_wrap;
+  int a2_wrap;
 };
 
 __device__ __forceinline__ long res_row(const G160Params& p, int m) {
@@ -205,7 +206,7 @@
     return false;
   }
 
-  const bool geglu = GEGLU_ONLY || p.act == PFD_ACT_GEGLU;
+  const bool geglu = GEGLU_ONLY || (!slab && p.act == PFD_ACT_GEGLU);
   const int lrow = wm * WMB * 16 + l15;
   const bool has_bias = p.bias && !slab;
   const half_t* bp = has_bias ? p.bias + nw : g_zero_page;
@@ -563,7 +564,8 @@
       const int mz = m - p.zero_rows;
       a_ok[j] = a_ok[j] && mz >= 0;
       a_ptr[j] = a_ok[j] ? p.A + (long)mz * p.lda + c * 8 : g_zero_page;
-      a2_ptr[j] = a_ok[j] ? p.A2 + (long)mz * p.lda2 + c * 8 : g_zero_page;
+      const int mz2 = mz >= p.a2_wrap ? mz - p.a2_wrap : mz;
+      a2_ptr[j] = a_ok[j] ? p.A2 + (long)mz2 * p.lda2 + c * 8 : g_zero_page;
       a_oy[j] = a_ox[j] = 0;
       a_img[j] = 0;
     }
@@ -1462,6 +1464,98 @@
   }
 }
 
+constexpr int RLN_T = 64;
+__global__ __launch_bounds__(RLN_T) void splitk_reduce_ln_kernel(const G160Params p) {
+  const int P = p.N / 160;
+  const long ngrp = (long)p.M * P;
+  const long grp = ((long)blockIdx.x * RLN_T + threadIdx.x) >> 2;
+  const int k = threadIdx.x & 3;
+  const bool ok = grp < ngrp;
+  const long g = min(grp, ngrp - 1);
+  const int m = (int)(g / P);
+  const int n0 = (int)(g - (long)m * P) * 160 + k * 8;
+  const half_t* bp = p.bias ? p.bias + n0 : g_zero_page;
+  const half_t* rvp = p.rowvec ? p.rowvec + (long)(m / p.rows_per_rv) * p.ldrv + n0 : g_zero_page;
+  const half_t* rp = p.R ? p.R + res_row(p, m) * p.ldr + n0 : g_zero_page;
+  const int bstep = p.bias ? 32 : 0, rvstep = p.rowvec ? 32 : 0, rstep = p.R ? 32 : 0;
+  Pack16 bb[5], rv[5], rr[5];
+#pragma unroll
+  for (int j = 0; j < 5; ++j) {
+    bb[j].u = *reinterpret_cast<const uint4*>(bp + j * bstep);
+    rv[j].u = *reinterpret_cast<const uint4*>(rvp + j * rvstep);
+    rr[j].u = *reinterpret_cast<const uint4*>(rp + j * rstep);
+  }
+  float v[5][8];
+#pragma unroll
+  for (int j = 0; j < 5; ++j)
+#pragma unroll
+    for (int e = 0; e < 8; ++e) v[j][e] = 0.f;
+  for (int s0 = 0; s0 < p.splits; s0 += 4) {
+    Pack16 a[5][4];
+#pragma unroll
+    for (int j = 0; j < 5; ++j)
+#pragma unroll
+      for (int u = 0; u < 4; ++u)
+        a[j][u].u = *reinterpret_cast<const uint4*>(reinterpret_cast<const half_t*>(p.ws) +
+                                                    ((long)min(s0 + u, p.splits - 1) * p.M + m) * p.N + n0 + j * 32);
+#pragma unroll
+    for (int j = 0; j < 5; ++j)
+#pragma unroll
+      for (int u = 0; u < 4; ++u) {
+        const float w = s0 + u < p.splits ? 1.f : 0.f;
+#pragma unroll
+        for (int e = 0; e < 8; ++e) v[j][e] += (float)a[j][u].e[e] * w;
+      }
+  }
+  if (p.ln_in) {
+    const float2* src = p.ln_in + (long)m * p.ln_P;
+    float sum = 0.f, sq = 0.f;
+#pragma unroll
+    for (int j = 0; j < 8; ++j) {
+      const float2 t = src[min(j, p.ln_P - 1)];
+      const float w = j < p.ln_P ? 1.f : 0.f;
+      sum = fmaf(t.x, w, sum);
+      sq = fmaf(t.y, w, sq);
+    }
+    const float inv_k = 1.0f / (float)p.K;
+    const float mean = sum * inv_k;
+    const float rstd = rsqrtf(fmaxf(fmaf(-mean, mean, sq * inv_k), 0.f) + p.ln_eps);
+#pragma unroll
+    for (int j = 0; j < 5; ++j) {
+      const float4_t c0 = *reinterpret_cast<const float4_t*>(p.ln_cs + n0 + j * 32);
+      const float4_t c1 = *reinterpret_cast<const float4_t*>(p.ln_cs + n0 + j * 32 + 4);
+#pragma unroll
+      for (int e = 0; e < 4; ++e) {
+        v[j][e] = fmaf(v[j][e], rstd, -rstd * mean * c0[e]);
+        v[j][4 + e] = fmaf(v[j][4 + e], rstd, -rstd * mean * c1[e]);
+      }
+    }
+  }
+  float s = 0.f, q = 0.f;
+#pragma unroll
+  for (int j = 0; j < 5; ++j) {
+    Pack16 o;
+#pragma unroll
+    for (int e = 0; e < 8; ++e) {
+      float x = v[j][e] + (float)bb[j].e[e];
+      x += (float)rv[j].e[e];
+      if (p.act == PFD_ACT_GELU) x = pfd_gelu(x);
+      else if (p.act == PFD_ACT_RELU) x = fmaxf(x, 0.f);
+      else if (p.act == PFD_ACT_SILU) x = pfd_silu(x);
+      o.e[e] = (half_t)(x + (float)rr[j].e[e]);
+      const float f = (float)o.e[e];
+      s += f;
+      q = fmaf(f, f, q);
+    }
+    if (ok) *reinterpret_cast<uint4*>(p.C + (long)m * p.ldc + n0 + j * 32) = o.u;
+  }
+  s += __shfl_xor(s, 1, 64);
+  q += __shfl_xor(q, 1, 64);
+  s += __shfl_xor(s, 2, 64);
+  q += __shfl_xor(q, 2, 64);
+  if (k == 0 && ok) p.ln_out[grp] = make_float2(s, q);
+}
+
 constexpr int RGN_T = 256;
 __global__ __launch_bounds__(RGN_T) void splitk_reduce_gn_kernel(const G160Params p) {
   constexpr int RW = RGN_T / 64, ROWS_SW = 3 * RW;
@@ -1695,6 +1789,8 @@
 
 thread_local GnFuse t_gnf = {nullptr, nullptr, nullptr, 0, 0.f, 0, 0, 0};
 
+int g_ln_reduce_fused = 1;
+
 inline void launch_splitk_reduce(const G160Params& p, hipStream_t s) {
   if (pfd_prof_on()) {
     pfd_prof_end(s);
@@ -1708,6 +1804,10 @@
   }
   if (p.gn_out) {
     hipLaunchKernelGGL(splitk_reduce_gn_kernel, dim3((p.M / GN_SLAB) * (p.N / 160)), dim3(RGN_T), 0, s, p);
+  } else if (p.ln_out && g_ln_reduce_fused) {
+    const long nthr = (long)p.M * (p.N / 160) * 4;
+    hipLaunchKernelGGL(splitk_reduce_ln_kernel, dim3((unsigned)((nthr + RLN_T - 1) / RLN_T)), dim3(RLN_T), 0, s, p);
+    return;
   } else {
     const long nvec = (long)p.M * (p.N / 8);
     int g = (int)((nvec + 255) / 256);
@@ -1804,6 +1904,12 @@
   return pfd_check_launch("pfd_gemm_f16(conv3x3 patch)");
 }
 
+}
+
+extern "C" int32_t pfd_gemm_ln_reduce_fused(int32_t on) {
+  const int was = g_ln_reduce_fused;
+  if (on >= 0) g_ln_reduce_fused = on ? 1 : 0;
+  return was;
 }
 
 int pfd_gemm160_try(const PfdGemmDesc* d, int variant, int splits, hipStream_t s) {
@@ -1875,7 +1981,11 @@
     if (!d->R || d->res_rows >= d->M || 2L * d->res_rows < d->M || d->gnf_y) return 1;
     p.r_wrap = d->res_rows;
   }
-  p.k_split = d->K; p.zero_rows = 0;
+  p.k_split = d->K; p.zero_rows = 0; p.a2_wrap = 0x7fffffff;
+  if (d->a2_rows > 0 && d->a2_rows != d->M) {
+    if (d->k_split <= 0 || d->zero_rows != 0 || d->a2_rows >= d->M || 2L * d->a2_rows < d->M) return 1;
+    p.a2_wrap = d->a2_rows;
+  }
   if (d->k_split > 0 || d->zero_rows > 0) {
     if (d->ksize > 0 || d->gn_table || d->bias_per_row || d->Ct) return 1;
     if (d->zero_rows < 0 || d->zero_rows >= d->M || (d->zero_rows > 0 && d->ln_stats)) return 1;
diff --git a/prompt-free-diffusion_amd/csrc/norm.hip b/prompt-free-diffusion_amd/csrc/norm.hip
--- a/prompt-free-diffusion_amd/csrc/norm.hip
+++ b/prompt-free-diffusion_amd/csrc/norm.hip
@@ -15,12 +15,14 @@
   const half_t* x2;
   long ld1, ld2;
   int C1, C2;
+  long rows2;
 };
 
 __device__ __forceinline__ uint4 gn_load(const GnSrc& s, long row, int v) {
   const int c = v * 8;
   if (c < s.C1) return *reinterpret_cast<const uint4*>(s.x1 + row * s.ld1 + c);
-  return *reinterpret_cast<const uint4*>(s.x2 + row * s.ld2 + (c - s.C1));
+  const long row2 = row >= s.rows2 ? row - s.rows2 : row;
+  return *reinterpret_cast<const uint4*>(s.x2 + row2 * s.ld2 + (c - s.C1));
 }
 
 __global__ __launch_bounds__(256) void gn_stats_kernel(GnSrc s, int HW, int G, int rows_per_chunk,
@@ -206,6 +208,8 @@
       const int tn = first ? ps.tn1 : ps.tn2, cpp = first ? ps.cpp1 : ps.cpp2;
       const int cl = first ? c0 : c0 - s.C1;
       const int npg = cpg / cpp;
+      const long sl2 = s.rows2 / 64;
+      const long sl0 = !first && (long)b * nslab >= sl2 ? (long)b * nslab - sl2 : (long)b * nslab;
       if constexpr (PAR) {
         const int c1 = cl + (npg > 1 ? cpp : 0);
         const int col0 = (cl / 160) * 16 + (cl % 160) / cpp, col1 = (c1 / 160) * 16 + (c1 % 160) / cpp;
@@ -215,7 +219,7 @@
 #pragma unroll
           for (int u = 0; u < 8; ++u) {
             const int k = min(k0 + u * P, nslab - 1);
-            const float2* row = st + ((long)(b * nslab + k) * tn) * 16;
+            const float2* row = st + ((sl0 + k) * tn) * 16;
             v0[u] = row[col0];
             v1[u] = row[col1];
           }
@@ -230,7 +234,7 @@
         }
       } else {
         for (int k = part; k < nslab; k += P) {
-          const float2* row = st + ((long)(b * nslab + k) * tn) * 16;
+          const float2* row = st + ((sl0 + k) * tn) * 16;
           for (int j = 0; j < npg; ++j) {
             const int c = cl + j * cpp;
             const float2 v = row[(c / 160) * 16 + (c % 160) / cpp];
@@ -712,19 +716,22 @@
   return 1;
 }
 
-extern "C" int pfd_groupnorm_pstats_f16(const void* x1, int32_t C1, int64_t ldx1, const void* st1, const void* x2,
-                                        int32_t C2, int64_t ldx2, const void* st2, const void* gamma, const void* beta,
-                                        void* y, int64_t ldy, int32_t B, int32_t HW, int32_t G, float eps, int32_t act,
-                                        pfd_stream_t stream) {
+extern "C" int pfd_groupnorm_pstats_wrap_f16(const void* x1, int32_t C1, int64_t ldx1, const void* st1, const void* x2,
+                                             int32_t C2, int64_t ldx2, const void* st2, const void* gamma, const void* beta,
+                                             void* y, int64_t ldy, int32_t B, int32_t HW, int32_t G, float eps, int32_t act,
+                                             int32_t x2_rows, pfd_stream_t stream) {
   if (!x1 || !st1 || !gamma || !beta || !y) return PFD_EINVAL;
   if (C2 > 0 && (!x2 || !st2)) return PFD_EINVAL;
   if (act != PFD_ACT_NONE && act != PFD_ACT_SILU) return PFD_EINVAL;
   if ((ldx1 & 7) || (ldx2 & 7) || (ldy & 7) || (reinterpret_cast<uintptr_t>(st1) & 7) || (reinterpret_cast<uintptr_t>(st2) & 7))
     return PFD_EINVAL;
   if (!pfd_groupnorm_takes_pstats(B, C1, C2, HW, G)) return PFD_ESHAPE;
+  const long rows = (long)B * HW;
+  if (x2_rows < 0) return PFD_EINVAL;
+  if (x2_rows > 0 && x2_rows != rows && (C2 <= 0 || x2_rows >= rows || 2L * x2_rows < rows || (x2_rows % HW))) return PFD_ESHAPE;
   hipStream_t s = (hipStream_t)stream;
   const int C = C1 + C2;
-  GnSrc src{(const half_t*)x1, (const half_t*)x2, ldx1, ldx2, C1, C2};
+  GnSrc src{(const half_t*)x1, (const half_t*)x2, ldx1, ldx2, C1, C2, x2_rows > 0 && x2_rows != rows ? (long)x2_rows : 0L};
   GnPStats ps{(const float2*)st1, (const float2*)st2, C1 / 160, C2 ? C2 / 160 : 0, C1 / 32, C2 ? C2 / 32 : C1 / 32};
   int nchunks, rpc;
   gn_chunks(B, C, HW, &nchunks, &rpc);
@@ -738,6 +745,13 @@
     hipLaunchKernelGGL(gn_apply_pstats_kernel<false>, dim3(nchunks, B), dim3(256), 0, s, src, ps, (const half_t*)gamma,
                        (const half_t*)beta, (half_t*)y, (long)ldy, HW, G, rpc, act, (float)HW * (float)(C / G), eps);
   return pfd_check_launch("pfd_groupnorm_pstats_f16");
+}
+
+extern "C" int pfd_groupnorm_pstats_f16(const void* x1, int32_t C1, int64_t ldx1, const void* st1, const void* x2,
+                                        int32_t C2, int64_t ldx2, const void* st2, const void* gamma, const void* beta,
+                                        void* y, int64_t ldy, int32_t B, int32_t HW, int32_t G, float eps, int32_t act,
+                                        pfd_stream_t stream) {
+  return pfd_groupnorm_pstats_wrap_f16(x1, C1, ldx1, st1, x2, C2, ldx2, st2, gamma, beta, y, ldy, B, HW, G, eps, act, 0, stream);
 }
 
 extern "C" int pfd_groupnorm_table_f16(const void* x1, int32_t C1, int64_t ldx1, const void* x2, int32_t C2,
diff --git a/prompt-free-diffusion_amd/csrc/selftest.cpp b/prompt-free-diffusion_amd/csrc/selftest.cpp
--- a/prompt-free-diffusion_amd/csrc/selftest.cpp
+++ b/prompt-free-diffusion_amd/csrc/selftest.cpp
@@ -556,7 +556,49 @@
   else printf("ok   %-58s\n", name);
 }
 
+static void run_ln_reduce_case(int M, int N, int K, int tile, int act, bool rowvec, bool ln_in = false) {
+  auto A = rand_h((size_t)M * K), Wt = rand_h((size_t)N * K, 1.7f / sqrtf((float)K)), Bv = rand_h(N), R = rand_h((size_t)M * N, 2.0f);
+  auto V = rand_h((size_t)2 * N);
+  const int P = N / 160, Pk = K / 160, rpr = (M + 1) / 2;
+  auto sti = rand_f((size_t)M * (Pk > 0 ? Pk : 1) * 2, 1.0f), cs = rand_f(N, 0.5f);
+  for (size_t i = 1; i < sti.size(); i += 2) sti[i] = fabsf(sti[i]) * (float)K / (float)(Pk > 0 ? Pk : 1) + 4.0f;
+  Dev<h16> dA(A), dW(Wt), dB(Bv), dR(R), dV(V), dC1((size_t)M * N), dC2((size_t)M * N);
+  Dev<float> dSti(sti), dCs(cs), s1((size_t)M * P * 2), s2((size_t)M * P * 2), s3((size_t)M * P * 2), dWS((size_t)8 * M * N);
+  PfdGemmDesc d;
+  memset(&d, 0, sizeof(d));
+  d.M = M; d.N = N; d.K = K; d.A = dA.p; d.W = dW.p; d.bias = dB.p; d.R = dR.p; d.act = act;
+  d.lda = K; d.ldw = K; d.ldc = N; d.ldr = N; d.ldrv = N; d.rows_per_rv = 1;
+  if (rowvec) { d.rowvec = dV.p; d.rows_per_rv = rpr; }
+  if (ln_in) { d.ln_stats = dSti.p; d.ln_colsum = dCs.p; d.ln_parts = Pk; d.ln_eps = 1e-5f; }
+  d.ws = dWS.p; d.ws_bytes = (size_t)8 * M * N * sizeof(float);
+  char name[200];
+  snprintf(name, sizeof(name), "split-K reduction + row statistics %dx%dx%d tile %d act%d%s%s (bitwise)", M, N, K, tile, act,
+           rowvec ? " +rv" : "", ln_in ? " +ln" : "");
+  ++g_total;
+  HIP_OK(hipMemset(s1.p, 0xFF, (size_t)M * P * 2 * sizeof(float)));
+  HIP_OK(hipMemset(s2.p, 0xFF, (size_t)M * P * 2 * sizeof(float)));
+  const int was = pfd_gemm_ln_reduce_fused(1);
+  d.C = dC1.p; d.ln_out = s1.p;
+  int rc = pfd_gemm_f16_ex(&d, tile, nullptr);
+  pfd_gemm_ln_reduce_fused(0);
+  d.C = dC2.p; d.ln_out = s2.p;
+  if (rc == 0) rc = pfd_gemm_f16_ex(&d, tile, nullptr);
+  pfd_gemm_ln_reduce_fused(was);
+  if (rc == 0) rc = pfd_ln_rowstats_f16(dC1.p, N, M, N, s3.p, nullptr);
+  if (rc != 0) { ++g_fail; printf("FAIL %-58s rc=%d (%s)\n", name, rc, pfd_last_error()); return; }
+  auto y1 = dC1.get(), y2 = dC2.get();
+  auto a = s1.get(), b = s2.get(), c = s3.get();
+  const bool same_y = !memcmp(y1.data(), y2.data(), y1.size() * sizeof(h16));
+  const bool same_s = !memcmp(a.data(), b.data(), a.size() * sizeof(float)) && !memcmp(a.data(), c.data(), a.size() * sizeof(float));
+  if (!same_y || !same_s) { ++g_fail; printf("FAIL %-58s %s differ\n", name, same_y ? "statistics" : "stored results"); }
+  else printf("ok   %-58s\n", name);
+}
+
 static void run_ln_fold_suite() {
+  for (int s : {2, 4}) run_ln_reduce_case(512, 1280, 1280, 3300 + s, PFD_ACT_NONE, false);
+  run_ln_reduce_case(200, 320, 1280, 3304, PFD_ACT_GELU, true);
+  run_ln_reduce_case(203, 640, 640, 3302, PFD_ACT_NONE, false, true);
+  run_ln_reduce_case(512, 320, 2048, 3308, PFD_ACT_SILU, true);
   run_add_rowvec_lnstats_case(130, 320);
   run_add_rowvec_lnstats_case(77, 1280);
   run_ln_fold_case(300, 320, 960, 0, 0, 0, 640);
@@ -847,6 +889,94 @@
           ref[((size_t)b * HW + r) * C + c] = act_ref((at(b, r, c) - mean) * rstd * (double)gm[c] + (double)bt[c], act);
     }
   report(name, got, ref, 6e-3, 4e-3);
+}
+
+static void run_a2_wrap_case(int B, int B2, int HW, int C1, int C2, int N, int tile) {
+  const int M = B * HW, M2 = B2 * HW, C = C1 + C2, G = 32;
+  auto x1 = rand_h((size_t)M * C1, 1.5f), x2 = rand_h((size_t)M2 * C2, 1.5f), gm = rand_h(C), bt = rand_h(C);
+  for (auto& v : x2) v = (h16)((float)v + 0.4f);
+  std::vector<h16> x2d((size_t)M * C2);
+  for (int m = 0; m < M; ++m)
+    for (int c = 0; c < C2; ++c) x2d[(size_t)m * C2 + c] = x2[(size_t)(m >= M2 ? m - M2 : m) * C2 + c];
+  auto mk_stats = [&](const std::vector<h16>& x, int rows, int Cs) {
+    const int cpp = Cs / 32, tn = Cs / 160;
+    std::vector<float> st((size_t)(rows / 64) * tn * 32, 0.f);
+    for (int sl = 0; sl < rows / 64; ++sl)
+      for (int c = 0; c < Cs; ++c) {
+        float a = 0, q = 0;
+        for (int r = 0; r < 64; ++r) { const float v = (float)x[(size_t)(sl * 64 + r) * Cs + c]; a += v; q += v * v; }
+        const size_t o = (((size_t)sl * tn + c / 160) * 16 + (c % 160) / cpp) * 2;
+        st[o] += a; st[o + 1] += q;
+      }
+    return st;
+  };
+  auto s1 = mk_stats(x1, M, C1), s2 = mk_stats(x2, M2, C2), s2d = mk_stats(x2d, M, C2);
+  Dev<h16> d1(x1), d2(x2), d2d(x2d), dg(gm), db(bt), dy1((size_t)M * C), dy2((size_t)M * C);
+  Dev<float> ds1(s1), ds2(s2), ds2d(s2d);
+  char name[200];
+  snprintf(name, sizeof(name), "second source of %d of %d samples read with one wrap: HW%d C%d+%d N%d tile %d (bitwise)", B2, B, HW, C1, C2, N, tile);
+  ++g_total;
+  auto fail = [&](const char* what, int rc) { ++g_fail; printf("FAIL %-58s %s rc=%d (%s)\n", name, what, rc, pfd_last_error()); };
+  int rc = pfd_groupnorm_pstats_wrap_f16(d1.p, C1, C1, ds1.p, d2.p, C2, C2, ds2.p, dg.p, db.p, dy1.p, C, B, HW, G, 1e-5f, PFD_ACT_SILU, M2, nullptr);
+  if (rc == 0) rc = pfd_groupnorm_pstats_f16(d1.p, C1, C1, ds1.p, d2d.p, C2, C2, ds2d.p, dg.p, db.p, dy2.p, C, B, HW, G, 1e-5f, PFD_ACT_SILU, nullptr);
+  if (rc != 0) return fail("groupnorm", rc);
+  {
+    auto a = dy1.get(), b = dy2.get();
+    if (memcmp(a.data(), b.data(), a.size() * sizeof(h16))) return fail("groupnorm: results differ", 0);
+  }
+  HIP_OK(hipMemset(dy1.p, 0x5A, (size_t)M * C * sizeof(h16)));
+  for (int bad : {M2 - HW, M - 1, M2 + 64}) {
+    if (bad <= 0 || 2 * bad >= M && bad % HW == 0) continue;
+    rc = pfd_groupnorm_pstats_wrap_f16(d1.p, C1, C1, ds1.p, d2.p, C2, C2, ds2.p, dg.p, db.p, dy1.p, C, B, HW, G, 1e-5f, PFD_ACT_SILU, bad, nullptr);
+    if (rc != PFD_ESHAPE) return fail("groupnorm: bad x2_rows not declined", rc);
+  }
+  {
+    auto a = dy1.get();
+    for (auto& v : a) { unsigned short u; memcpy(&u, &v, 2); if (u != 0x5A5A) return fail("groupnorm: a declined call wrote", 0); }
+  }
+  auto Wt = rand_h((size_t)N * C, 1.7f / sqrtf((float)C)), Bv = rand_h(N);
+  Dev<h16> dW(Wt), dB(Bv), dC1((size_t)M * N), dC2((size_t)M * N);
+  Dev<float> dWS((size_t)8 * M * N);
+  PfdGemmDesc d;
+  memset(&d, 0, sizeof(d));
+  d.M = M; d.N = N; d.K = C; d.A = d1.p; d.W = dW.p; d.bias = dB.p; d.lda = C1; d.ldw = C; d.ldc = N; d.rows_per_rv = 1;
+  d.k_split = C1; d.lda2 = C2;
+  d.ws = dWS.p; d.ws_bytes = (size_t)8 * M * N * sizeof(float);
+  d.A2 = d2.p; d.a2_rows = M2; d.C = dC1.p;
+  rc = pfd_gemm_f16_ex(&d, tile, nullptr);
+  d.A2 = d2d.p; d.a2_rows = 0; d.C = dC2.p;
+  if (rc == 0) rc = pfd_gemm_f16_ex(&d, tile, nullptr);
+  if (rc != 0) return fail("gemm", rc);
+  {
+    auto a = dC1.get(), b = dC2.get();
+    if (memcmp(a.data(), b.data(), a.size() * sizeof(h16))) return fail("gemm: results differ", 0);
+  }
+  HIP_OK(hipMemset(dC1.p, 0x5A, (size_t)M * N * sizeof(h16)));
+  d.A2 = d2.p; d.C = dC1.p;
+  if (M2 - HW > 0 && 2 * (M2 - HW) < M) {
+    d.a2_rows = M2 - HW;
+    rc = pfd_gemm_f16_ex(&d, tile, nullptr);
+    if (rc != PFD_ESHAPE) return fail("gemm: a2_rows below M / 2 not declined", rc);
+  }
+  d.a2_rows = M2; d.zero_rows = 64;
+  rc = pfd_gemm_f16_ex(&d, tile, nullptr);
+  if (rc != PFD_ESHAPE) return fail("gemm: a2_rows with zero_rows not declined", rc);
+  d.zero_rows = 0; d.k_split = 0; d.K = C1;
+  rc = pfd_gemm_f16_ex(&d, tile, nullptr);
+  if (rc != PFD_ESHAPE) return fail("gemm: a2_rows without k_split not declined", rc);
+  {
+    auto a = dC1.get();
+    for (auto& v : a) { unsigned short u; memcpy(&u, &v, 2); if (u != 0x5A5A) return fail("gemm: a declined call wrote", 0); }
+  }
+  printf("ok   %-58s\n", name);
+}
+
+static void run_a2_wrap_cases() {
+  run_a2_wrap_case(2, 1, 256, 320, 320, 320, 0);
+  for (int v : {9200, 9300, 3200, 3300, 5400})
+    run_a2_wrap_case(4, 2, 128, 320, 320, 320, v);
+  run_a2_wrap_case(3, 2, 64, 640, 640, 640, 0);
+  run_a2_wrap_case(2, 1, 256, 320, 320, 320, 3302);
 }
 
 static void run_gn_conv_case(int B, int H, int W, int C1, int C2, int N, int act, bool with_res) {
@@ -1760,6 +1890,7 @@
     run_gn_pstats_case(8, 4096, 320, 320, PFD_ACT_SILU, 1e-5f);
     run_gn_pstats_case(3, 1024, 640, 0, PFD_ACT_NONE, 1e-6f);
     run_gn_pstats_case(2, 256, 1280, 1280, PFD_ACT_SILU, 1e-5f);
+    run_a2_wrap_cases();
     printf("SELFTEST %d/%d passed, %d failed\n", g_total - g_fail, g_total, g_fail);
     return g_fail;
   }
@@ -1802,6 +1933,13 @@
   }
   if (argc > 1 && !strcmp(argv[1], "--elementwise")) {
     run_elementwise();
+    printf("SELFTEST %d/%d passed, %d failed\n", g_total - g_fail, g_total, g_fail);
+    return g_fail;
+  }
+  if (argc > 1 && !strcmp(argv[1], "--glue")) {
+    for (int sp : {2, 4}) run_ln_reduce_case(512, 1280, 1280, 3300 + sp, PFD_ACT_NONE, false);
+    run_ln_reduce_case(203, 640, 640, 3302, PFD_ACT_NONE, false, true);
+    run_a2_wrap_cases();
     printf("SELFTEST %d/%d passed, %d failed\n", g_total - g_fail, g_total, g_fail);
     return g_fail;
   }
diff --git a/prompt-free-diffusion_amd/lib/hip/binding.py b/prompt-free-diffusion_amd/lib/hip/binding.py
--- a/prompt-free-diffusion_amd/lib/hip/binding.py
+++ b/prompt-free-diffusion_amd/lib/hip/binding.py
@@ -25,7 +25,7 @@
         ("ln_stats", _vp), ("ln_colsum", _vp), ("ln_parts", _i32), ("ln_eps", _f32), ("ln_out", _vp),
         ("k_split", _i32), ("zero_rows", _i32), ("gn_out", _vp),
         ("gnf_gamma", _vp), ("gnf_beta", _vp), ("gnf_y", _vp), ("gnf_ldy", _i64), ("gnf_eps", _f32), ("gnf_act", _i32),
-        ("gnf_rows", _i32), ("gnf_skip_raw", _i32), ("res_rows", _i32),
+        ("gnf_rows", _i32), ("gnf_skip_raw", _i32), ("res_rows", _i32), ("a2_rows", _i32),
     ]
 
 
@@ -53,6 +53,7 @@
     "pfd_gemm_f16": (_i32, [C.POINTER(PfdGemmDesc), _vp]),
     "pfd_gemm_f16_ex": (_i32, [C.POINTER(PfdGemmDesc), _i32, _vp]),
     "pfd_gemm_geglu_group": (_i32, [_i32]),
+    "pfd_gemm_ln_reduce_fused": (_i32, [_i32]),
     "pfd_attention_f16": (_i32, [C.POINTER(PfdAttnDesc), _vp]),
     "pfd_swin_window_attention_f16": (_i32, [C.POINTER(PfdSwinAttnDesc), _vp]),
     "pfd_groupnorm_ws_bytes": (_sz, [_i32, _i32, _i32]),
@@ -63,6 +64,8 @@
     "pfd_groupnorm_takes_pstats": (_i32, [_i32, _i32, _i32, _i32, _i32]),
     "pfd_groupnorm_pstats_f16": (_i32, [_vp, _i32, _i64, _vp, _vp, _i32, _i64, _vp, _vp, _vp, _vp, _i64, _i32, _i32, _i32,
                                         _f32, _i32, _vp]),
+    "pfd_groupnorm_pstats_wrap_f16": (_i32, [_vp, _i32, _i64, _vp, _vp, _i32, _i64, _vp, _vp, _vp, _vp, _i64, _i32, _i32,
+                                             _i32, _f32, _i32, _i32, _vp]),
     "pfd_layernorm_f16": (_i32, [_vp, _i64, _vp, _vp, _vp, _i64, _i32, _i32, _f32, _i32, _i32, _i32, _i32, _vp]),
     "pfd_ln_rowstats_f16": (_i32, [_vp, _i64, _i32, _i32, _vp, _vp]),
     "pfd_softmax_rows_f16": (_i32, [_vp, _i64, _vp, _i64, _i32, _i32, _f32, _vp]),
diff --git a/prompt-free-diffusion_amd/lib/hip/ops.py b/prompt-free-diffusion_amd/lib/hip/ops.py
--- a/prompt-free-diffusion_amd/lib/hip/ops.py
+++ b/prompt-free-diffusion_amd/lib/hip/ops.py
@@ -126,6 +126,17 @@
     return out
 
 
+LN_REDUCE = os.environ.get("PFD_LN_REDUCE", "1") != "0"
+_LN_REDUCE_SENT = None
+
+
+def _sync_ln_reduce():
+    global _LN_REDUCE_SENT
+    if _LN_REDUCE_SENT != LN_REDUCE:
+        _lib().pfd_gemm_ln_reduce_fused(1 if LN_REDUCE else 0)
+        _LN_REDUCE_SENT = LN_REDUCE
+
+
 GN_PSTATS = True
 
 
@@ -181,6 +192,18 @@
     if st is not None:
         set_gn_stats(out, torch.cat([st, st]))
     return out
+
+
+SKIP_WRAP = os.environ.get("PFD_SKIP_WRAP", "1") != "0"
+
+
+def pair_skip_wraps(x, x2, groups, n_out):
+    B, C1, C2 = x.shape[0], x.shape[-1], x2.shape[-1]
+    if 2 * x2.shape[0] != B or tuple(x2.shape[1:-1]) != tuple(x.shape[1:-1]) or not GN_PSTATS or groups != 32:
+        return False
+    if get_gn_stats(x) is None or get_gn_stats(x2) is None or not wide_tile_ok(n_out, C1 + C2) or C1 % 64:
+        return False
+    return bool(_lib().pfd_groupnorm_takes_pstats(B, C1, C2, x.numel() // (B * C1), groups))
 
 
 GEMM_FUSE = True
@@ -202,7 +225,7 @@
     if a2 is not None:
         _chk16(a2, "gemm A2")
         M2, Ka2, lda2 = _rows(a2)
-        if M2 != M or a2.device != a.device:
+        if not (M2 == M or (not zero_rows and M2 < M <= 2 * M2)) or a2.device != a.device:
             raise ValueError(f"gemm: a2 {tuple(a2.shape)} does not pair with a {tuple(a.shape)}")
         if k is None:
             K = Ka + Ka2
@@ -239,6 +262,8 @@
     d.ws, d.ws_bytes = _workspace(a.device).data_ptr(), _WS_BYTES
     if a2 is not None:
         d.A2, d.lda2, d.k_split = a2.data_ptr(), lda2, Ka
+        if M2 != M:
+            d.a2_rows = M2
     d.zero_rows = zero_rows
     if res_rows is not None:
         if res is None or M != 2 * res_rows or _rows(res)[0] != res_rows:
@@ -263,6 +288,7 @@
             if stats.dtype != torch.float32 or not stats.is_contiguous() or stats.numel() != M * (N // 160) * 2:
                 raise ValueError("gemm: ln_out must be a contiguous float32 [M, N/160, 2]")
         d.ln_out = stats.data_ptr()
+        _sync_ln_reduce()
     gst = None
     if gn_out:
         gst = _new_gn_stats(M, N, a.device)
@@ -471,6 +497,11 @@
     C2 = 0 if x2 is None else x2.shape[-1]
     if out is None:
         out = torch.empty(tuple(x.shape[:-1]) + (C1 + C2,), dtype=torch.float16, device=x.device)
+    x2_rows = 0
+    if x2 is not None and x2.shape[0] != B:
+        if 2 * x2.shape[0] != B or tuple(x2.shape[1:-1]) != tuple(x.shape[1:-1]):
+            raise ValueError(f"groupnorm: x2 {tuple(x2.shape)} does not pair with x {tuple(x.shape)}")
+        x2_rows = x2.shape[0] * HW
     lib = _lib()
     st1 = get_gn_stats(x) if GN_PSTATS else None
     st2 = get_gn_stats(x2) if (GN_PSTATS and x2 is not None) else None
@@ -480,12 +511,15 @@
                     f"{int(bool(lib.pfd_groupnorm_takes_pstats(B, C1, C2, HW, groups)))}\n")
     if st1 is not None and (x2 is None or st2 is not None) and groups == 32 and \
             lib.pfd_groupnorm_takes_pstats(B, C1, C2, HW, groups):
-        rc = lib.pfd_groupnorm_pstats_f16(x.data_ptr(), C1, x.stride(-2), st1.data_ptr(), _ptr(x2), C2,
-                                          0 if x2 is None else x2.stride(-2), _ptr(st2), gamma.data_ptr(), beta.data_ptr(),
-                                          out.data_ptr(), out.stride(-2), B, HW, groups, eps,
-                                          ACT_SILU if silu else ACT_NONE, _stream())
+        rc = lib.pfd_groupnorm_pstats_wrap_f16(x.data_ptr(), C1, x.stride(-2), st1.data_ptr(), _ptr(x2), C2,
+                                               0 if x2 is None else x2.stride(-2), _ptr(st2), gamma.data_ptr(), beta.data_ptr(),
+                                               out.data_ptr(), out.stride(-2), B, HW, groups, eps,
+                                               ACT_SILU if silu else ACT_NONE, x2_rows, _stream())
         _b.check(rc, f"pfd_groupnorm_pstats_f16 B{B} HW{HW} C{C1}+{C2}")
         return _written(out)
+    if x2_rows:
+        raise ValueError("groupnorm: an x2 of half the samples needs the producers' statistics of both sources "
+                         "(ops.pair_skip_wraps says whether a skip concat qualifies)")
     wsb = lib.pfd_groupnorm_ws_bytes(B, C1 + C2, HW)
     ws = torch.empty(wsb, dtype=torch.uint8, device=x.device)
     rc = lib.pfd_groupnorm_f16(x.data_ptr(), C1, x.stride(-2), _ptr(x2), C2, 0 if x2 is None else x2.stride(-2),
diff --git a/prompt-free-diffusion_amd/lib/model_zoo/openaimodel.py b/prompt-free-diffusion_amd/lib/model_zoo/openaimodel.py
--- a/prompt-free-diffusion_amd/lib/model_zoo/openaimodel.py
+++ b/prompt-free-diffusion_amd/lib/model_zoo/openaimodel.py
@@ -136,6 +136,11 @@
         C2 = 0 if x2 is None else x2.shape[-1]
         assert C1 + C2 == self.channels
         B, H, W_, _ = x.shape
+        if x2 is not None and x2.shape[0] != B:
+            sc = self.skip_connection
+            if self.fuse_groupnorm or not isinstance(sc, L.Conv2d) or sc.kernel_size[0] != 1 or \
+                    not ops.pair_skip_wraps(x, x2, self.in_layers[0].num_groups, self.out_channels):
+                x2 = ops.cat_pair(x2)
         fuse = self.fuse_groupnorm
         fuse_in = fuse and ops.conv_gn_fusable(B, H, W_, C1, C2, self.out_channels)
         fuse_out = fuse and ops.conv_gn_fusable(B, H, W_, self.out_channels, 0, self.out_channels)
@@ -379,7 +384,7 @@
             elif ltype == 'c':
                 h = ctx_layer(h)
             else:
-                hs.append(ops.cat_pair(h) if pair[0] else h)
+                hs.append(ops.cat_pair(h) if pair[0] and (ccs is not None or not ops.SKIP_WRAP) else h)
             step[0] += 1
         if pair[0]:
             raise ValueError("cfg_pair: no context layer in the input half of this UNet")
```

Result: no change. 8.629 images/s, median of 6 (+0.2%).
